# CasualGANPapers/Make-A-Scene

Measured on NVIDIA B200. Metric: VQ-IMG 256^2 images/sec (enc+VQ+dec fwd+bwd), higher is better.
Workload: dtype fp16 (3x3 convolutions) / tf32 (1x1) tcgen05 operands (11-bit significand), fp32 accumulate / storage; 3xTF32 for the attention contractions; fp32 FFMA for VQ argmin and edge layers

## Files before the change

include/mas_b200.h:

```cpp
#ifndef MAS_B200_H_
#define MAS_B200_H_

#include <stddef.h>
#include <stdint.h>

#ifdef __cplusplus
extern "C" {
#endif

#define MAS_OK 0
#define MAS_ERR_INVALID_ARG (-1)
#define MAS_ERR_UNSUPPORTED (-2)
#define MAS_ERR_LAUNCH (-3)
#define MAS_ERR_WORKSPACE (-4)

#define MAS_CONV_S1 0
#define MAS_CONV_S2 1
#define MAS_CONV_UP 2
#define MAS_CONV_ZS 3

#define MAS_IMPL_AUTO 0
#define MAS_IMPL_SIMT 1
#define MAS_IMPL_TC 2
#define MAS_IMPL_TC3 3

typedef struct mas_tensor4 {
  int64_t n, h, w, c;
  int64_t sn, sh, sw, sc;
} mas_tensor4;

int mas_version(void);
const char* mas_last_error(void);
int64_t mas_launch_count(void);
int64_t mas_tc_launch_count(void);

int mas_ffma_probe(float* scratch, int iters, double* flops_out_host, void* stream);

int mas_copy_strided(const float* x, mas_tensor4 xs, float* y, mas_tensor4 ys, void* stream);

int mas_nchw_to_nhwc_pad(const float* x_nchw, float* y_nhwc, int N, int C, int CP, int H, int W, void* stream);
int mas_scale_by(const float* x, const float* g, float* y, int64_t n, void* stream);

size_t mas_gn_ws_bytes(int N, int HW, int C, int G);
int mas_gn_stats(const float* x, int N, int HW, int C, int G, float eps, float* mean, float* rstd,
                 void* ws, size_t ws_bytes, void* stream);
int mas_gn_apply(const float* x, const float* mean, const float* rstd, const float* gamma,
                 const float* beta, float* y, int N, int HW, int C, int G, int silu, int round_tf32,
                 void* stream);
int mas_gn_backward(const float* dy, const float* x, const float* mean, const float* rstd,
                    const float* gamma, const float* beta, const float* dx_add, float* dx, float* dgamma,
                    float* dbeta, void* act_out, int act_f16, float* dx_amax, const float* add_amax, void* dx_f16,
                    float* dx_bound, int N, int HW, int C, int G, int silu, void* ws, size_t ws_bytes, void* stream);
int mas_add(const float* a, const float* b, float* out, int64_t n, void* stream);
int mas_silu_forward(const float* x, float* y, int64_t n, void* stream);
int mas_silu_backward(const float* dy, const float* x, float* dx, int64_t n, void* stream);

int mas_pack_conv3x3(const float* w_oihw, float* w_packed, int Cout, int Cin, int flip_transpose,
                     int round_tf32, void* stream);
int mas_conv3x3_fprop(const float* x, mas_tensor4 xs, const float* w_packed, const float* bias,
                      const float* residual, float* y, mas_tensor4 ys, int mode, int impl, void* stream);
int mas_conv3x3_tc_eligible(mas_tensor4 xs, mas_tensor4 ys, int mode);
int mas_pack_conv3x3_tc(const float* w_oihw, float* w_tc, int Cout, int Cin, int transpose, void* stream);
int mas_conv3x3_fprop_tc(const float* x, mas_tensor4 xs, const float* w_tc, const float* bias,
                         const float* residual, float* y, mas_tensor4 ys, int mode, const float* gn_table,
                         int gn_silu, float* stats_part, void* stream);
int mas_amax(const float* x, int64_t n, float* out, void* stream);
int mas_pack_conv3x3_tc16(const float* w_oihw, void* w_tc16, void* w_tc16_dgrad, int Cout, int Cin, int transpose,
                          void* stream);
int mas_conv3x3_fprop_tc16(const float* x, mas_tensor4 xs, const void* w_tc16, const float* bias,
                           const float* residual, float* y, mas_tensor4 ys, int mode, const float* gn_table,
                           int gn_silu, float* stats_part, const float* x_amax, void* stream);
int mas_conv3x3_tc16h_eligible(mas_tensor4 xs, mas_tensor4 ys);
int mas_conv3x3_fprop_tc16h(const void* x_f16, mas_tensor4 xs, const void* w_tc16, const float* bias,
                            const float* residual, float* y, mas_tensor4 ys, float* stats_part,
                            const float* x_amax, void* stream);
int mas_to_half(const float* x, void* y_f16, int64_t n, const float* amax, void* stream);
int mas_pack_conv3x3_tc_pair(const float* w_oihw, float* w_tc_fwd, float* w_tc_dgrad, int Cout, int Cin, void* stream);
int mas_gn_finalize_partials(const float* part, int tiles_per_image, int N, int C, int G, int64_t hw, float eps,
                             float* mean, float* rstd, void* stream);
int mas_gn_table(const float* mean, const float* rstd, const float* gamma, const float* beta, int N, int C, int G,
                 float* table, void* stream);
int mas_pack_gemm_tc(const float* w_nk, float* w_tc, int N, int K, int transpose, void* stream);
int mas_gemm_rows_packed(const float* A, int64_t lda, const float* w_tc, float* C, int64_t ldc, int64_t M, int N,
                         int K, float alpha, const float* bias, const float* residual, float* stats_part,
                         void* stream);
int mas_pack_gemm_tc16(const float* w_nk, void* w_tc16, int N, int K, int transpose, void* stream);
int mas_gemm_rows_f16(const void* x_f16, int64_t M, int K, const void* w_tc16, float* y, int64_t ldy, int N, const float* bias,
                      const float* residual, const float* x_amax, float alpha, void* stream);
size_t mas_wgrad_rows_f16_ws_bytes(int64_t M, int N, int K);
int mas_wgrad_rows_f16(const void* x_f16, const void* dy_f16, int64_t M, int N, int K, float* dw, float* dbias,
                       const float* x_amax, const float* dy_amax, void* ws, size_t ws_bytes, void* stream);
int mas_tc_probe(const float* A, const float* B, float* D, int a_src, int b_layout, uint64_t raw_desc,
                 uint32_t raw_idesc, int raw_off, void* stream);
int mas_tc_probe16(float* D, uint64_t raw_desc, uint32_t raw_idesc, int raw_off, void* stream);
size_t mas_conv3x3_wgrad_ws_bytes(mas_tensor4 xs, mas_tensor4 dys, int mode);
int mas_conv3x3_wgrad(const float* x, mas_tensor4 xs, const float* dy, mas_tensor4 dys, float* dw_oihw,
                      float* dbias, int mode, int impl, const float* gn_table, int gn_silu, void* ws,
                      size_t ws_bytes, void* stream);
int mas_conv3x3_wgrad_tc_eligible(mas_tensor4 xs, mas_tensor4 dys, int mode);
int mas_conv3x3_wgrad_tc16(const void* x, int x_is_f16, mas_tensor4 xs, const float* dy, mas_tensor4 dys, float* dw_oihw,
                           float* dbias, int mode, const float* gn_table, int gn_silu, const float* dy_amax, int cout_rows,
                           void* ws, size_t ws_bytes, void* stream);
size_t mas_conv1x1_wgrad_ws_bytes(int64_t M, int Cin, int Cout);
int mas_conv1x1_wgrad(const float* x, int64_t ldx, const float* dy, int64_t ldy, int64_t M, int Cin, int Cout,
                      float* dw, float* dbias, int impl, void* ws, size_t ws_bytes, void* stream);
int mas_edge_small_cin_fprop(const float* xs, mas_tensor4 xst, const float* w, const float* bias, float* y,
                             mas_tensor4 yst, int flip_transpose, void* stream);
int mas_edge_small_cout_fprop(const float* a, mas_tensor4 at, const float* w, const float* bias, float* ys,
                              mas_tensor4 yst, void* stream);
size_t mas_edge_wgrad_ws_bytes(int Cbig);
int mas_edge_small_cin_wgrad(const float* xs, mas_tensor4 xst, const float* dy, mas_tensor4 dyt, float* dw,
                             float* dbias, void* ws, size_t ws_bytes, void* stream);
int mas_edge_small_cout_wgrad(const float* a, mas_tensor4 at, const float* dys, mas_tensor4 dyt, float* dw,
                              float* dbias, void* ws, size_t ws_bytes, void* stream);
int mas_space_to_depth(const float* x, float* y, int N, int H, int W, int C, void* stream);
int mas_s2d_pack_weights(const float* w, float* w9, int Cout, int C, void* stream);
int mas_s2d_unpack_wgrad(const float* dw9, float* dw, int Cout, int C, void* stream);
int mas_sumpool2x2(const float* x, float* y, int N, int H, int W, int C, void* stream);

int mas_gemm(const float* A, const float* B, float* C, int M, int N, int K, int batch, int64_t lda,
             int64_t ldb, int64_t ldc, int64_t stride_a, int64_t stride_b, int64_t stride_c, int trans_a,
             int trans_b, float alpha, const float* bias, const float* residual, int impl, void* stream);
int mas_gemm_batched2(const float* A, const float* B, float* C, int M, int N, int K, int outer, int batch, int64_t lda,
                      int64_t ldb, int64_t ldc, int64_t outer_stride_a, int64_t outer_stride_b, int64_t outer_stride_c,
                      int64_t stride_a, int64_t stride_b, int64_t stride_c, int trans_a, int trans_b, float alpha, int impl,
                      int causal, void* stream);
size_t mas_colsum_ws_bytes(mas_tensor4 t);
int mas_colsum(const float* x, mas_tensor4 t, float* out, void* ws, size_t ws_bytes, void* stream);

int mas_softmax_forward(const float* s, float* p, int64_t rows, int cols, void* stream);
int mas_softmax_backward(const float* p, const float* dp, float* ds, int64_t rows, int cols, float scale,
                         void* stream);

size_t mas_attnblock_ws_bytes(int N, int HW, int C, int G);
int mas_attnblock_forward(const float* x, int N, int HW, int C, int G, const float* mean, const float* rstd,
                          const float* norm_w, const float* norm_b, const float* q_w, const float* q_b,
                          const float* k_w, const float* k_b, const float* v_w, const float* v_b,
                          const float* proj_w, const float* proj_b, float* hn, float* qkv, float* P, float* O,
                          float* out, float* stats_part, int impl, void* ws, size_t ws_bytes, void* stream);
int mas_attnblock_backward(const float* dout, const float* x, int N, int HW, int C, int G, const float* mean,
                           const float* rstd, const float* norm_w, const float* norm_b, const float* q_w,
                           const float* k_w, const float* v_w, const float* proj_w, const float* hn,
                           const float* qkv, const float* P, const float* O, float* dx, float* dnorm_w,
                           float* dnorm_b, float* dqkv_w, float* dqkv_b, float* dproj_w, float* dproj_b,
                           float* dx_amax , int impl, void* ws,
                           size_t ws_bytes, void* stream);

int mas_bn_stats(const float* x, int64_t R, int C, double* stats_out, void* stream);
int mas_bn_finalize(const double* stats, double count, int C, float eps, float momentum, float* mean,
                    float* invstd, float* running_mean, float* running_var, void* stream);
int mas_bn_invstd(const float* running_var, float eps, float* invstd, int C, void* stream);
int mas_bn_apply(const float* x, const float* mean, const float* invstd, const float* gamma,
                 const float* beta, float* y, int64_t R, int C, void* stream);
int mas_bn_backward_reduce(const float* dy, const float* x, const float* mean, const float* invstd,
                           int64_t R, int C, double* sums_out, void* stream);
int mas_bn_backward_apply(const float* dy, const float* x, const float* mean, const float* invstd,
                          const float* gamma, const double* sums_global, const double* sums_local,
                          double inv_count, float* dx, float* dgamma, float* dbeta, int64_t R, int C,
                          void* stream);

int mas_vq_select_path(int use_tensor_core_filter);
size_t mas_vq_ws_bytes(int64_t R, int K, int D);
int mas_vq_forward(const float* z, const float* E, int64_t R, int K, int D, float beta, int64_t* idx_out,
                   float* zq_out, float* loss_out, void* ws, size_t ws_bytes, void* stream);
int mas_vq_forward_given(const float* z, const float* E, const int64_t* idx_in, int64_t R, int K, int D, float beta,
                         float* zq_out, float* loss_out, void* ws, size_t ws_bytes, void* stream);
size_t mas_kmeans_ws_bytes(int K, int D);
int mas_kmeans_update(const float* x, const int64_t* idx, int64_t n, int K, int D, const float* centres_old,
                      float* centres_new, float* shift_out, void* ws, size_t ws_bytes, void* stream);
int mas_vq_backward(const float* g_zq, const float* g_loss, const float* z, const float* E,
                    const int64_t* idx, int64_t R, int K, int D, float beta, float* grad_z, float* grad_E,
                    void* stream);
int mas_vq_gather(const float* E, const int64_t* idx, int64_t R, int K, int D, float* out, void* stream);

int mas_layernorm_forward(const float* x, const float* gamma, const float* beta, const float* residual, float* y,
                          float* mean, float* rstd, int64_t R, int H, float eps, void* stream);
int mas_layernorm2_forward(const float* x, const float* gamma1, const float* beta1, const float* residual, float* y1,
                           const float* gamma2, const float* beta2, float* y2, int64_t R, int H, float eps1, float eps2,
                           void* stream);
size_t mas_layernorm_ws_bytes(int64_t R, int H);
int mas_layernorm_backward(const float* dy, const float* x, const float* mean, const float* rstd,
                           const float* gamma, float* dx, float* dgamma, float* dbeta, int64_t R, int H, void* ws,
                           size_t ws_bytes, void* stream);
int mas_gelu_forward(const float* x, float* y, int64_t n, void* stream);
int mas_gelu_backward(const float* dy, const float* x, float* dx, int64_t n, void* stream);
int mas_softmax_causal_forward(const float* s, float* p, int64_t mats, int rows, int cols, void* stream);
int mas_softmax_causal_backward(const float* p, const float* dp, float* ds, int64_t mats, int rows, int cols, float scale,
                                void* stream);
int mas_embed3_forward(const float* t0, const int64_t* id0, const float* t1, const int64_t* id1, const float* t2,
                       const int64_t* id2, float* out, int64_t R, int H, int seg, int total, int off, void* stream);
int mas_embed3_backward(const float* dout, const int64_t* id0, float* d0, const int64_t* id1, float* d1,
                        const int64_t* id2, float* d2, int64_t R, int H, int seg, int total, int off, void* stream);
int mas_attn_causal_forward(const float* qkv, const float* amax, float* P, float* ctx, int B, int S, int heads, int hd,
                            float scale, void* stream);
int mas_ce_forward(const float* logits, int64_t ld, const int64_t* target, float* loss_rows, float* lse, float* out,
                   int64_t R, int V, void* stream);
int mas_ce_backward(const float* logits, int64_t ld, const int64_t* target, const float* lse, const float* stat,
                    const float* dloss, float* dlogits, int64_t ldd, int64_t R, int V, void* stream);

int mas_linear_small(const float* x, int64_t ldx, const float* W, const float* bias, float* y, int64_t ldy, int R, int N,
                     int K, int act, void* stream);
int mas_kv_append(const float* qkv, int R, int T, int heads, int hd, float* kcache, float* vcache, int Tmax, int pos0,
                  void* stream);
int mas_attn_decode(const float* qkv, const float* kcache, const float* vcache, float* ctx, int R, int heads, int hd,
                    int Tmax, int len, void* stream);
int mas_attn_decode_append(const float* qkv, float* kcache, float* vcache, float* ctx, int R, int heads, int hd, int Tmax,
                           int pos, void* stream);
int mas_cfg_mix(const float* cond, const float* uncond, float* out, int64_t n, float scale, void* stream);
int mas_sample_topk(const float* logits, int64_t ld, int R, int V, float temperature, int top_k, const float* u,
                    int64_t* tokens, void* stream);

int mas_bce_logits(const float* logits, mas_tensor4 ls, const float* target, mas_tensor4 ts,
                   const float* pos_weight, float* loss_out, float* grad, mas_tensor4 gs, float grad_scale,
                   void* ws, size_t ws_bytes, void* stream);
size_t mas_bce_ws_bytes(mas_tensor4 ls);
size_t mas_bce_cl_ws_bytes(int N, int H, int W);
int mas_bce_cl_forward(const float* logits, const float* target_nchw, const float* pos_weight, int N, int C, int CP, int H,
                       int W, float* loss_out, void* ws, size_t ws_bytes, void* stream);
int mas_bce_cl_backward(const float* logits, const float* target_nchw, const float* pos_weight, const float* g, int N, int C,
                        int CP, int H, int W, float* grad, void* stream);

#ifdef __cplusplus
}
#endif
#endif
```

make-a-scene_b200/csrc/contract_tc.cu:

```cuda
#include <cuda.h>
#include <cudaTypedefs.h>
#include <cuda_fp16.h>
#include <stdlib.h>

#include "mas_common.cuh"
#include "tc_ptx.cuh"

namespace mas {
namespace tc {

constexpr int TILES_MAX = 4;
constexpr int NPROD = 256;
constexpr int NTHREADS = 320;
constexpr int STAGES_CONV = 3;

enum { MAP_S1 = 0, MAP_UP = 2, MAP_ZS = 3, MAP_ROWS = 4 };

struct Params {
  const float* x;
  const float* wpk;
  const float* bias;
  const float* res;
  float* y;
  int N, Hin, Win, Cin, Hout, Wout, Cout;
  int map;
  int64_t ldx, ldy;
  int tiles_x, tiles_y;
  int64_t total_tiles;
  float alpha;
  const float* gn_table;
  int gn_silu;
  float* stats_part;
  const float* x_amax;
  int Cstore;
};

template <int TAPS, int KC, int STAGES, int TILES, bool F16>
__global__ void __launch_bounds__(NTHREADS, (TILES == 2) ? 2 : 1) shift_gemm_tc(const Params p) {
  constexpr int EPC = F16 ? 8 : 4;
  constexpr int SLOTS = (TAPS == 9) ? 180 : 132;
  constexpr int ROWP = (TAPS == 9) ? 10 : 8;
  constexpr int LBO_A = SLOTS * 16;
  constexpr int SBO_A = ROWP * 16;
  constexpr int A_TILE = (KC / EPC) * LBO_A;
  constexpr int A_STAGE = TILES * A_TILE;
  constexpr int LBO_B = BN * 16;
  constexpr int B_TAP = (KC / EPC) * LBO_B;
  constexpr int B_STAGE = TAPS * B_TAP;
  constexpr int STAGE = A_STAGE + B_STAGE;
  constexpr int QUADS = KC / EPC;
  constexpr int ITEMS = TILES * SLOTS * QUADS;
  constexpr int LPI = F16 ? 2 : 1;
  constexpr int PER_THREAD = (ITEMS + NPROD - 1) / NPROD;
  static_assert((SLOTS % 8) == 4, "A plane pitch must be 64 mod 128 bytes for conflict-free producer stores");

  extern __shared__ __align__(1024) uint8_t smem[];
  uint64_t* bars = reinterpret_cast<uint64_t*>(smem + (size_t)STAGES * STAGE);
  uint32_t* tmem_slot = reinterpret_cast<uint32_t*>(bars + 2 * STAGES + 1);
  const uint32_t smem_base = smem_u32(smem);
  const uint32_t bar_base = smem_u32(bars);
  auto full_bar = [&](int s) { return bar_base + 8u * s; };
  auto empty_bar = [&](int s) { return bar_base + 8u * (STAGES + s); };
  const uint32_t accum_bar = bar_base + 8u * (2 * STAGES);

  const int tid = threadIdx.x, warp = tid >> 5, lane = tid & 31;
  const int64_t tile0 = (int64_t)blockIdx.x * TILES;
  const int n0 = blockIdx.y * BN;
  const int nchunks = p.Cin / KC;

  if (tid == 0) {
    for (int s = 0; s < STAGES; ++s) {
      mbar_init(full_bar(s), NPROD + 1);
      mbar_init(empty_bar(s), 1);
    }
    mbar_init(accum_bar, 1);
    fence_barrier_init();
  }
  if (warp == 8) tmem_alloc(smem_u32(tmem_slot), TILES * BN);
  tc_fence_before();
  __syncthreads();
  tc_fence_after();
  const uint32_t tmem_base = *tmem_slot;

  if (warp < 8) {
    const float* src[PER_THREAD];
    const float* tab[(TAPS == 9) ? PER_THREAD : 1];
    uint32_t dst[PER_THREAD];
#pragma unroll
    for (int i = 0; i < PER_THREAD; ++i) {
      const int item = tid + i * NPROD;
      src[i] = nullptr;
      if (TAPS == 9) tab[i] = nullptr;
      dst[i] = 0xFFFFFFFFu;
      if (item < ITEMS) {
        const int q = item % QUADS, rest = item / QUADS, slot = rest % SLOTS, tl = rest / SLOTS;
        dst[i] = (uint32_t)(tl * A_TILE + q * LBO_A + slot * 16);
        const int64_t tile = tile0 + tl;
        if (tile < p.total_tiles) {
          if (TAPS == 9) {
            const int tx_ = (int)(tile % p.tiles_x), ty_ = (int)((tile / p.tiles_x) % p.tiles_y);
            const int n = (int)(tile / ((int64_t)p.tiles_x * p.tiles_y));
            const int r = slot / 10, c = slot % 10;
            const int vy = ty_ * 16 - 1 + r, vx = tx_ * 8 - 1 + c;
            int iy = vy, ix = vx;
            bool ok;
            if (p.map == MAP_S1) {
              ok = (unsigned)vy < (unsigned)p.Hin && (unsigned)vx < (unsigned)p.Win;
            } else if (p.map == MAP_UP) {
              ok = (unsigned)vy < (unsigned)(2 * p.Hin) && (unsigned)vx < (unsigned)(2 * p.Win);
              iy = vy >> 1; ix = vx >> 1;
            } else {
              ok = vy >= 0 && vx >= 0 && (vy & 1) && (vx & 1) && (vy >> 1) < p.Hin && (vx >> 1) < p.Win;
              iy = vy >> 1; ix = vx >> 1;
            }
            if (ok) {
              src[i] = p.x + ((int64_t)(n * p.Hin + iy) * p.Win + ix) * p.ldx + q * EPC;
              if (p.gn_table) tab[i] = p.gn_table + ((size_t)n * p.Cin + q * EPC) * 2;
            }
          } else {
            const int64_t row = tile * BM + slot;
            if (slot >= BM) dst[i] = 0xFFFFFFFFu;
            else if (row < (int64_t)p.N * p.Hout * p.Wout) src[i] = p.x + row * p.ldx + q * EPC;
          }
        }
      }
    }
    int stage = 0;
    uint32_t phase = 0;
    float inv_scale = 1.f;
    const float in_scale = F16 ? operand_scale(p.x_amax, &inv_scale) : 1.f;
    float4 va[PER_THREAD][LPI], vb[PER_THREAD][LPI];
    auto gload = [&](int kc, float4 (*v)[LPI]) {
#pragma unroll
      for (int i = 0; i < PER_THREAD; ++i) {
#pragma unroll
        for (int h = 0; h < LPI; ++h) {
          v[i][h] = make_float4(0.f, 0.f, 0.f, 0.f);
          if (src[i]) v[i][h] = ldg_l2pf(reinterpret_cast<const float4*>(src[i] + (size_t)kc * KC) + h);
        }
      }
    };
    auto consume = [&](int kc, float4 (*v)[LPI]) {
      if (TAPS == 9) {
        if (p.gn_table) {
#pragma unroll
          for (int i = 0; i < PER_THREAD; ++i) {
            if (tab[i]) {
#pragma unroll
              for (int h = 0; h < LPI; ++h) {
                const float4* tp = reinterpret_cast<const float4*>(tab[i] + (size_t)kc * KC * 2) + 2 * h;
                const float4 t0 = __ldg(tp);
                const float4 t1 = __ldg(tp + 1);
                float a0 = fmaf(v[i][h].x, t0.x, t0.y), a1 = fmaf(v[i][h].y, t0.z, t0.w);
                float a2 = fmaf(v[i][h].z, t1.x, t1.y), a3 = fmaf(v[i][h].w, t1.z, t1.w);
                if (p.gn_silu) { a0 = silu_f(a0); a1 = silu_f(a1); a2 = silu_f(a2); a3 = silu_f(a3); }
                v[i][h] = make_float4(a0, a1, a2, a3);
              }
            }
          }
        }
      }
      mbar_wait(empty_bar(stage), phase ^ 1);
      uint8_t* a_st = smem + (size_t)stage * STAGE;
#pragma unroll
      for (int i = 0; i < PER_THREAD; ++i) {
        if (dst[i] != 0xFFFFFFFFu) {
          if (F16) {
            const float4 lo = v[i][0], hi = v[i][LPI - 1];
            *reinterpret_cast<uint4*>(a_st + dst[i]) =
                make_uint4(pack_h2(lo.x * in_scale, lo.y * in_scale), pack_h2(lo.z * in_scale, lo.w * in_scale),
                           pack_h2(hi.x * in_scale, hi.y * in_scale), pack_h2(hi.z * in_scale, hi.w * in_scale));
          } else {
            *reinterpret_cast<float4*>(a_st + dst[i]) = v[i][0];
          }
        }
      }
      fence_proxy_async();
      mbar_arrive(full_bar(stage));
      if (++stage == STAGES) { stage = 0; phase ^= 1; }
    };
    gload(0, va);
    if (nchunks > 1) gload(1, vb);
    for (int kc = 0; kc < nchunks; kc += 2) {
      consume(kc, va);
      if (kc + 2 < nchunks) gload(kc + 2, va);
      if (kc + 1 < nchunks) {
        consume(kc + 1, vb);
        if (kc + 3 < nchunks) gload(kc + 3, vb);
      }
    }
    const float alpha = p.alpha * inv_scale;

    mbar_wait(accum_bar, 0);
    tc_fence_after();
    const int lane_grp = warp & 3;
    const int chalf = warp >> 2;
    constexpr int EP_LD = 36;
    float* patch = reinterpret_cast<float*>(smem) + warp * (32 * EP_LD);
    const int sub_r = lane >> 3, sub_c = lane & 7;
#pragma unroll 1
    for (int tl = 0; tl < TILES; ++tl) {
      const int64_t tile = tile0 + tl;
      if (tile >= p.total_tiles) break;
      int64_t pix_base = 0;
      int tx_ = 0, ty_ = 0, n_img = 0;
      if (TAPS == 9) {
        tx_ = (int)(tile % p.tiles_x); ty_ = (int)((tile / p.tiles_x) % p.tiles_y);
        n_img = (int)(tile / ((int64_t)p.tiles_x * p.tiles_y));
      } else {
        pix_base = tile * BM;
      }
#pragma unroll 1
      for (int cc = 0; cc < 2; ++cc) {
        const int col = chalf * 64 + cc * 32;
        float v[32];
        tmem_ld32(tmem_base + ((uint32_t)(lane_grp * 32) << 16) + (uint32_t)(tl * BN + col), v);
        __syncwarp();
#pragma unroll
        for (int j = 0; j < 32; j += 4)
          *reinterpret_cast<float4*>(patch + lane * EP_LD + j) =
              make_float4(v[j] * alpha, v[j + 1] * alpha, v[j + 2] * alpha, v[j + 3] * alpha);
        __syncwarp();
        float4 bq = make_float4(0.f, 0.f, 0.f, 0.f);
        if (p.bias) bq = __ldg(reinterpret_cast<const float4*>(p.bias + n0 + col + sub_c * 4));
        float st_s = 0.f, st_q = 0.f;
#pragma unroll
        for (int i = 0; i < 8; ++i) {
          const int row = i * 4 + sub_r;
          const int m = lane_grp * 32 + row;
          int64_t pix;
          if (TAPS == 9) pix = ((int64_t)n_img * p.Hout + ty_ * 16 + (m >> 3)) * p.Wout + tx_ * 8 + (m & 7);
          else pix = pix_base + m;
          if (TAPS == 9 || pix < (int64_t)p.N * p.Hout * p.Wout) {
            float4 o = *reinterpret_cast<const float4*>(patch + row * EP_LD + sub_c * 4);
            o.x += bq.x; o.y += bq.y; o.z += bq.z; o.w += bq.w;
            const int64_t off = pix * p.ldy + n0 + col + sub_c * 4;
            if (n0 + col + sub_c * 4 >= p.Cstore) continue;
            if (p.res) {
              const float4 r4 = __ldg(reinterpret_cast<const float4*>(p.res + off));
              o.x += r4.x; o.y += r4.y; o.z += r4.z; o.w += r4.w;
            }
            *reinterpret_cast<float4*>(p.y + off) = o;
            st_s += (o.x + o.y) + (o.z + o.w);
            st_q = fmaf(o.x, o.x, fmaf(o.y, o.y, fmaf(o.z, o.z, fmaf(o.w, o.w, st_q))));
          }
        }
        if (p.stats_part) {
          st_s += __shfl_xor_sync(0xffffffffu, st_s, 8);
          st_q += __shfl_xor_sync(0xffffffffu, st_q, 8);
          st_s += __shfl_xor_sync(0xffffffffu, st_s, 16);
          st_q += __shfl_xor_sync(0xffffffffu, st_q, 16);
          if (lane < 8) {
            float* sp = p.stats_part + (((size_t)tile * 4 + lane_grp) * (p.Cout >> 2) + ((n0 + col) >> 2) + sub_c) * 2;
            sp[0] = st_s;
            sp[1] = st_q;
          }
        }
      }
    }
    tc_fence_before();
  } else if (warp == 8) {
    {
      constexpr uint32_t idesc = F16 ? make_idesc_f16(BN) : make_idesc(BN);
      int stage = 0;
      uint32_t phase = 0;
      for (int kc = 0; kc < nchunks; ++kc) {
        mbar_wait(full_bar(stage), phase);
        tc_fence_after();
        const uint32_t a_st = smem_base + (uint32_t)stage * STAGE;
        const uint64_t a_base = make_desc(a_st, LBO_A, SBO_A);
        const uint64_t b_base = make_desc(a_st + A_STAGE, LBO_B, 128);
        const uint32_t acc0 = (kc > 0) ? 1u : 0u;
        if (elect_one()) {
#pragma unroll
          for (int tl = 0; tl < TILES; ++tl) {
#pragma unroll
            for (int t = 0; t < TAPS; ++t) {
              const uint32_t tapoff = (TAPS == 9) ? (uint32_t)(((t / 3) * 10 + (t % 3)) * 16) : 0u;
#pragma unroll
              for (int k8 = 0; k8 < KC / (2 * EPC); ++k8) {
                const uint64_t ad = a_base + (uint64_t)((tl * A_TILE + tapoff + k8 * 2 * LBO_A) >> 4);
                const uint64_t bd = b_base + (uint64_t)((t * B_TAP + k8 * 2 * LBO_B) >> 4);
                if (F16) mma_f16_ss(tmem_base + (uint32_t)(tl * BN), ad, bd, idesc, (t > 0 || k8 > 0) ? 1u : acc0);
                else mma_tf32_ss(tmem_base + (uint32_t)(tl * BN), ad, bd, idesc, (t > 0 || k8 > 0) ? 1u : acc0);
              }
            }
          }
          mma_commit(empty_bar(stage));
          if (kc == nchunks - 1) mma_commit(accum_bar);
        }
        __syncwarp();
        if (++stage == STAGES) { stage = 0; phase ^= 1; }
      }
    }
  } else {
    if (lane == 0) {
      int stage = 0;
      uint32_t phase = 0;
      const float* wsrc = p.wpk + (size_t)blockIdx.y * nchunks * (B_STAGE / 4);
      for (int kc = 0; kc < nchunks; ++kc) {
        mbar_wait(empty_bar(stage), phase ^ 1);
        mbar_expect_tx(full_bar(stage), B_STAGE);
        bulk_g2s(smem_base + (uint32_t)stage * STAGE + A_STAGE, wsrc + (size_t)kc * (B_STAGE / 4), B_STAGE, full_bar(stage));
        if (++stage == STAGES) { stage = 0; phase ^= 1; }
      }
    }
    __syncwarp();
  }
  __syncthreads();
  if (warp == 8) {
    tc_fence_after();
    tmem_dealloc(tmem_base, TILES * BN);
  }
}

constexpr int P_STAGES = 4;
constexpr int P_NTHREADS = 14 * 32;
constexpr int P_EPI0 = 8;

__global__ void __launch_bounds__(P_NTHREADS, 1) shift_gemm_p16(const Params p) {
  constexpr int KC = 16, EPC = 8, TILES = 2, TAPS = 9;
  constexpr int SLOTS = 180, ROWP = 10;
  constexpr int LBO_A = SLOTS * 16, SBO_A = ROWP * 16;
  constexpr int A_TILE = (KC / EPC) * LBO_A, A_STAGE = TILES * A_TILE;
  constexpr int LBO_B = BN * 16, B_TAP = (KC / EPC) * LBO_B, B_STAGE = TAPS * B_TAP;
  constexpr int STAGE = A_STAGE + B_STAGE;
  constexpr int QUADS = KC / EPC;
  constexpr int ITEMS = TILES * SLOTS * QUADS;
  constexpr int PER_THREAD = (ITEMS + NPROD - 1) / NPROD;
  constexpr int EP_LD = 36;

  extern __shared__ __align__(1024) uint8_t smem[];
  float* patches = reinterpret_cast<float*>(smem + (size_t)P_STAGES * STAGE);
  uint64_t* bars = reinterpret_cast<uint64_t*>(patches + 4 * 32 * EP_LD);
  uint32_t* tmem_slot = reinterpret_cast<uint32_t*>(bars + 2 * P_STAGES + 4);
  const uint32_t smem_base = smem_u32(smem), bar_base = smem_u32(bars);
  auto full_bar = [&](int s) { return bar_base + 8u * s; };
  auto empty_bar = [&](int s) { return bar_base + 8u * (P_STAGES + s); };
  auto accf_bar = [&](int b) { return bar_base + 8u * (2 * P_STAGES + b); };
  auto acce_bar = [&](int b) { return bar_base + 8u * (2 * P_STAGES + 2 + b); };

  const int tid = threadIdx.x, warp = tid >> 5, lane = tid & 31;
  const int nchunks = p.Cin / KC;
  const int n_tiles = p.Cout / BN;
  const int64_t ngroups = (p.total_tiles + TILES - 1) / TILES;
  const int64_t nitems = ngroups * n_tiles;

  if (tid == 0) {
    for (int s = 0; s < P_STAGES; ++s) {
      mbar_init(full_bar(s), NPROD + 1);
      mbar_init(empty_bar(s), 1);
    }
    for (int b = 0; b < 2; ++b) {
      mbar_init(accf_bar(b), 1);
      mbar_init(acce_bar(b), 128);
    }
    fence_barrier_init();
  }
  if (warp == 12) tmem_alloc(smem_u32(tmem_slot), 512);
  tc_fence_before();
  __syncthreads();
  tc_fence_after();
  const uint32_t tmem_base = *tmem_slot;

  if (warp < 8) {
    float inv_scale = 1.f;
    const float in_scale = operand_scale(p.x_amax, &inv_scale);
    int stage = 0;
    uint32_t phase = 0;
    for (int64_t item = blockIdx.x; item < nitems; item += gridDim.x) {
      const int64_t tile0 = (item / n_tiles) * TILES;
      const float* src[PER_THREAD];
      const float* tab[PER_THREAD];
      uint32_t dst[PER_THREAD];
#pragma unroll
      for (int i = 0; i < PER_THREAD; ++i) {
        const int it = tid + i * NPROD;
        src[i] = nullptr;
        tab[i] = nullptr;
        dst[i] = 0xFFFFFFFFu;
        if (it < ITEMS) {
          const int q = it % QUADS, rest = it / QUADS, slot = rest % SLOTS, tl = rest / SLOTS;
          dst[i] = (uint32_t)(tl * A_TILE + q * LBO_A + slot * 16);
          const int64_t tile = tile0 + tl;
          if (tile < p.total_tiles) {
            const int tx_ = (int)(tile % p.tiles_x), ty_ = (int)((tile / p.tiles_x) % p.tiles_y);
            const int n = (int)(tile / ((int64_t)p.tiles_x * p.tiles_y));
            const int r = slot / 10, c = slot % 10;
            const int vy = ty_ * 16 - 1 + r, vx = tx_ * 8 - 1 + c;
            int iy = vy, ix = vx;
            bool ok;
            if (p.map == MAP_S1) {
              ok = (unsigned)vy < (unsigned)p.Hin && (unsigned)vx < (unsigned)p.Win;
            } else if (p.map == MAP_UP) {
              ok = (unsigned)vy < (unsigned)(2 * p.Hin) && (unsigned)vx < (unsigned)(2 * p.Win);
              iy = vy >> 1; ix = vx >> 1;
            } else {
              ok = vy >= 0 && vx >= 0 && (vy & 1) && (vx & 1) && (vy >> 1) < p.Hin && (vx >> 1) < p.Win;
              iy = vy >> 1; ix = vx >> 1;
            }
            if (ok) {
              src[i] = p.x + ((int64_t)(n * p.Hin + iy) * p.Win + ix) * p.ldx + q * EPC;
              if (p.gn_table) tab[i] = p.gn_table + ((size_t)n * p.Cin + q * EPC) * 2;
            }
          }
        }
      }
      float4 va[PER_THREAD][2], vb[PER_THREAD][2];
      auto gload = [&](int kc, float4 (*v)[2]) {
#pragma unroll
        for (int i = 0; i < PER_THREAD; ++i) {
#pragma unroll
          for (int h = 0; h < 2; ++h) {
            v[i][h] = make_float4(0.f, 0.f, 0.f, 0.f);
            if (src[i]) v[i][h] = ldg_l2pf(reinterpret_cast<const float4*>(src[i] + (size_t)kc * KC) + h);
          }
        }
      };
      auto consume = [&](int kc, float4 (*v)[2]) {
        if (p.gn_table) {
#pragma unroll
          for (int i = 0; i < PER_THREAD; ++i) {
            if (tab[i]) {
#pragma unroll
              for (int h = 0; h < 2; ++h) {
                const float4* tp = reinterpret_cast<const float4*>(tab[i] + (size_t)kc * KC * 2) + 2 * h;
                const float4 t0 = __ldg(tp);
                const float4 t1 = __ldg(tp + 1);
                float a0 = fmaf(v[i][h].x, t0.x, t0.y), a1 = fmaf(v[i][h].y, t0.z, t0.w);
                float a2 = fmaf(v[i][h].z, t1.x, t1.y), a3 = fmaf(v[i][h].w, t1.z, t1.w);
                if (p.gn_silu) { a0 = silu_f(a0); a1 = silu_f(a1); a2 = silu_f(a2); a3 = silu_f(a3); }
                v[i][h] = make_float4(a0, a1, a2, a3);
              }
            }
          }
        }
        mbar_wait(empty_bar(stage), phase ^ 1);
        uint8_t* a_st = smem + (size_t)stage * STAGE;
#pragma unroll
        for (int i = 0; i < PER_THREAD; ++i) {
          if (dst[i] != 0xFFFFFFFFu) {
            const float4 lo = v[i][0], hi = v[i][1];
            *reinterpret_cast<uint4*>(a_st + dst[i]) =
                make_uint4(pack_h2(lo.x * in_scale, lo.y * in_scale), pack_h2(lo.z * in_scale, lo.w * in_scale),
                           pack_h2(hi.x * in_scale, hi.y * in_scale), pack_h2(hi.z * in_scale, hi.w * in_scale));
          }
        }
        fence_proxy_async();
        mbar_arrive(full_bar(stage));
        if (++stage == P_STAGES) { stage = 0; phase ^= 1; }
      };
      gload(0, va);
      if (nchunks > 1) gload(1, vb);
      for (int kc = 0; kc < nchunks; kc += 2) {
        consume(kc, va);
        if (kc + 2 < nchunks) gload(kc + 2, va);
        if (kc + 1 < nchunks) {
          consume(kc + 1, vb);
          if (kc + 3 < nchunks) gload(kc + 3, vb);
        }
      }
    }
  } else if (warp < 12) {
    float inv_scale = 1.f;
    operand_scale(p.x_amax, &inv_scale);
    const float alpha = p.alpha * inv_scale;
    const int lane_grp = warp & 3;
    float* patch = patches + lane_grp * (32 * EP_LD);
    const int sub_r = lane >> 3, sub_c = lane & 7;
    int buf = 0;
    uint32_t ph[2] = {0u, 0u};
    for (int64_t item = blockIdx.x; item < nitems; item += gridDim.x) {
      const int64_t tile0 = (item / n_tiles) * TILES;
      const int n0 = (int)(item % n_tiles) * BN;
      mbar_wait(accf_bar(buf), ph[buf]);
      ph[buf] ^= 1u;
      tc_fence_after();
#pragma unroll 1
      for (int tl = 0; tl < TILES; ++tl) {
        const int64_t tile = tile0 + tl;
        const bool live = tile < p.total_tiles;
        const int tx_ = (int)(tile % p.tiles_x), ty_ = (int)((tile / p.tiles_x) % p.tiles_y);
        const int n_img = (int)(tile / ((int64_t)p.tiles_x * p.tiles_y));
#pragma unroll 1
        for (int cb = 0; cb < BN / 32; ++cb) {
          const int col = cb * 32;
          float v[32];
          tmem_ld32(tmem_base + ((uint32_t)(lane_grp * 32) << 16) + (uint32_t)(buf * TILES * BN + tl * BN + col), v);
          if (tl == TILES - 1 && cb == BN / 32 - 1) {
            tc_fence_before();
            mbar_arrive(acce_bar(buf));
          }
          if (!live) continue;
          __syncwarp();
#pragma unroll
          for (int j = 0; j < 32; j += 4)
            *reinterpret_cast<float4*>(patch + lane * EP_LD + j) =
                make_float4(v[j] * alpha, v[j + 1] * alpha, v[j + 2] * alpha, v[j + 3] * alpha);
          __syncwarp();
          float4 bq = make_float4(0.f, 0.f, 0.f, 0.f);
          if (p.bias) bq = __ldg(reinterpret_cast<const float4*>(p.bias + n0 + col + sub_c * 4));
          float st_s = 0.f, st_q = 0.f;
#pragma unroll
          for (int i = 0; i < 8; ++i) {
            const int row = i * 4 + sub_r;
            const int m = lane_grp * 32 + row;
            const int64_t pix = ((int64_t)n_img * p.Hout + ty_ * 16 + (m >> 3)) * p.Wout + tx_ * 8 + (m & 7);
            float4 o = *reinterpret_cast<const float4*>(patch + row * EP_LD + sub_c * 4);
            o.x += bq.x; o.y += bq.y; o.z += bq.z; o.w += bq.w;
            const int64_t off = pix * p.ldy + n0 + col + sub_c * 4;
            if (n0 + col + sub_c * 4 >= p.Cstore) continue;
            if (p.res) {
              const float4 r4 = __ldg(reinterpret_cast<const float4*>(p.res + off));
              o.x += r4.x; o.y += r4.y; o.z += r4.z; o.w += r4.w;
            }
            *reinterpret_cast<float4*>(p.y + off) = o;
            st_s += (o.x + o.y) + (o.z + o.w);
            st_q = fmaf(o.x, o.x, fmaf(o.y, o.y, fmaf(o.z, o.z, fmaf(o.w, o.w, st_q))));
          }
          if (p.stats_part) {
            st_s += __shfl_xor_sync(0xffffffffu, st_s, 8);
            st_q += __shfl_xor_sync(0xffffffffu, st_q, 8);
            st_s += __shfl_xor_sync(0xffffffffu, st_s, 16);
            st_q += __shfl_xor_sync(0xffffffffu, st_q, 16);
            if (lane < 8) {
              float* sp = p.stats_part + (((size_t)tile * 4 + lane_grp) * (p.Cout >> 2) + ((n0 + col) >> 2) + sub_c) * 2;
              sp[0] = st_s;
              sp[1] = st_q;
            }
          }
        }
      }
      buf ^= 1;
    }
  } else if (warp == 12) {
    {
      constexpr uint32_t idesc = make_idesc_f16(BN);
      int stage = 0, buf = 0;
      uint32_t phase = 0, eph[2] = {0u, 0u};
      for (int64_t item = blockIdx.x; item < nitems; item += gridDim.x) {
        mbar_wait(acce_bar(buf), eph[buf] ^ 1);
        eph[buf] ^= 1u;
        tc_fence_after();
        const uint32_t acc = tmem_base + (uint32_t)(buf * TILES * BN);
        for (int kc = 0; kc < nchunks; ++kc) {
          mbar_wait(full_bar(stage), phase);
          tc_fence_after();
          const uint32_t a_st = smem_base + (uint32_t)stage * STAGE;
          const uint64_t a_base = make_desc(a_st, LBO_A, SBO_A);
          const uint64_t b_base = make_desc(a_st + A_STAGE, LBO_B, 128);
          const uint32_t acc0 = (kc > 0) ? 1u : 0u;
          if (elect_one()) {
#pragma unroll
            for (int tl = 0; tl < TILES; ++tl) {
#pragma unroll
              for (int t = 0; t < TAPS; ++t) {
                const uint32_t tapoff = (uint32_t)(((t / 3) * 10 + (t % 3)) * 16);
                const uint64_t ad = a_base + (uint64_t)((tl * A_TILE + tapoff) >> 4);
                const uint64_t bd = b_base + (uint64_t)((t * B_TAP) >> 4);
                mma_f16_ss(acc + (uint32_t)(tl * BN), ad, bd, idesc, t > 0 ? 1u : acc0);
              }
            }
            mma_commit(empty_bar(stage));
            if (kc == nchunks - 1) mma_commit(accf_bar(buf));
          }
          __syncwarp();
          if (++stage == P_STAGES) { stage = 0; phase ^= 1; }
        }
        buf ^= 1;
      }
    }
  } else {
    if (lane == 0) {
      int stage = 0;
      uint32_t phase = 0;
      for (int64_t item = blockIdx.x; item < nitems; item += gridDim.x) {
        const float* wsrc = p.wpk + (size_t)(item % n_tiles) * nchunks * (B_STAGE / 4);
        for (int kc = 0; kc < nchunks; ++kc) {
          mbar_wait(empty_bar(stage), phase ^ 1);
          mbar_expect_tx(full_bar(stage), B_STAGE);
          bulk_g2s(smem_base + (uint32_t)stage * STAGE + A_STAGE, wsrc + (size_t)kc * (B_STAGE / 4), B_STAGE, full_bar(stage));
          if (++stage == P_STAGES) { stage = 0; phase ^= 1; }
        }
      }
    }
    __syncwarp();
  }
  tc_fence_before();
  __syncthreads();
  if (warp == 12) {
    tc_fence_after();
    tmem_dealloc(tmem_base, 512);
  }
}
constexpr size_t p16_smem_bytes() {
  return (size_t)P_STAGES * (2 * 2 * 180 * 16 + 9 * 2 * BN * 16) + 4 * 32 * 36 * 4 + (2 * P_STAGES + 4) * 8 + 16;
}

template <int TAPS, int KC, int STAGES, int TILES, bool F16>
constexpr size_t smem_bytes() {
  constexpr int SLOTS = (TAPS == 9) ? 180 : 132, EPC = F16 ? 8 : 4;
  return (size_t)STAGES * (TILES * (KC / EPC) * SLOTS * 16 + TAPS * (KC / EPC) * BN * 16) + (2 * STAGES + 1) * 8 + 16;
}

__global__ void pack_weights_tc(const float* __restrict__ w, float* __restrict__ out, int Cout, int Cin, int taps, int KC, int transpose) {
  const int N = transpose ? Cin : Cout, K = transpose ? Cout : Cin;
  const int64_t total = (int64_t)N * K * taps;
  const int nchunks = K / KC, quads = KC / 4;
  for (int64_t i = (int64_t)blockIdx.x * blockDim.x + threadIdx.x; i < total; i += (int64_t)gridDim.x * blockDim.x) {
    int64_t r = i;
    const int e = (int)(r % 4); r /= 4;
    const int nn = (int)(r % BN); r /= BN;
    const int q = (int)(r % quads); r /= quads;
    const int t = (int)(r % taps); r /= taps;
    const int kc = (int)(r % nchunks); r /= nchunks;
    const int nt = (int)r;
    const int n = nt * BN + nn, k = kc * KC + q * 4 + e;
    float v;
    if (!transpose) v = w[((size_t)n * Cin + k) * taps + t];
    else v = w[((size_t)k * Cin + n) * taps + (taps - 1 - t)];
    out[i] = round_tf32(v);
  }
}

__global__ void pack_weights_tc16(const float* __restrict__ w, __half* __restrict__ out_f, __half* __restrict__ out_d, int Cout, int Cin,
                                  int taps, int KC, int transpose, int both) {
  const int64_t total = (int64_t)Cout * Cin * taps;
  for (int64_t i = (int64_t)blockIdx.x * blockDim.x + threadIdx.x; i < total; i += (int64_t)gridDim.x * blockDim.x) {
    const int t = (int)(i % taps);
    const int ci = (int)((i / taps) % Cin), co = (int)(i / ((int64_t)taps * Cin));
    const __half v = __float2half_rn(w[i]);
    auto put = [&](__half* out, int n, int k, int tt, int K) {
      const int nchunks = K / KC, octs = KC / 8;
      const int64_t j = (((((int64_t)(n / BN) * nchunks + k / KC) * taps + tt) * octs + (k % KC) / 8) * BN + (n % BN)) * 8 + (k % 8);
      out[j] = v;
    };
    if (both) {
      put(out_f, co, ci, t, Cin);
      put(out_d, ci, co, taps - 1 - t, Cout);
    } else if (!transpose) {
      put(out_f, co, ci, t, Cin);
    } else {
      put(out_f, ci, co, taps - 1 - t, Cout);
    }
  }
}

__global__ void pack_weights_tc_pair(const float* __restrict__ w, float* __restrict__ out_f, float* __restrict__ out_d, int Cout, int Cin) {
  constexpr int taps = 9, KC = 8, quads = KC / 4;
  const int64_t total = (int64_t)Cout * Cin * taps;
  const int nchunks = Cin / KC, nchunks_d = Cout / KC;
  for (int64_t i = (int64_t)blockIdx.x * blockDim.x + threadIdx.x; i < total; i += (int64_t)gridDim.x * blockDim.x) {
    int64_t r = i;
    const int e = (int)(r % 4); r /= 4;
    const int nn = (int)(r % BN); r /= BN;
    const int q = (int)(r % quads); r /= quads;
    const int t = (int)(r % taps); r /= taps;
    const int kc = (int)(r % nchunks); r /= nchunks;
    const int nt = (int)r;
    const int n = nt * BN + nn, k = kc * KC + q * 4 + e;
    const float v = round_tf32(w[((size_t)n * Cin + k) * taps + t]);
    out_f[i] = v;
    const int td = taps - 1 - t;
    const int64_t j = ((((int64_t)(k / BN) * nchunks_d + n / KC) * taps + td) * quads + (n % KC) / 4) * BN * 4 + (int64_t)(k % BN) * 4 + (n % 4);
    out_d[j] = v;
  }
}


constexpr int WG_NT = 32;
constexpr int WG_STAGES = 3;
constexpr int WG_SLOTS = 100;
constexpr int WG_THREADS = 14 * 32;
constexpr int WG_DY_STAGE = 64 * 128 * 4;

struct WParams {
  const float* x;
  const float* dy;
  float* part;
  float* bpart;
  int N, Hin, Win, Cin, H, W, Cout, map;
  int units_x, units_y;
  int64_t total_units, units_per_split, rows, ldx, ldy;
  const float* gn_table;
  int gn_silu;
  const float* dy_amax;
  int Cout_real;
  int x_f16;
  int dy_f16;
};

template <int TAPS, bool PRO, bool F16>
__global__ void __launch_bounds__(WG_THREADS, 1) wgrad_tc(const WParams p, const __grid_constant__ CUtensorMap dy_map) {
  static_assert(!F16 || TAPS == 9, "the fp16-operand weight-gradient kernel is the 3x3 one");
  constexpr int NT = (TAPS == 9) ? WG_NT : 128, QUADS = NT / 4;
  constexpr int SLOTS = (TAPS == 9) ? WG_SLOTS : 64;
  constexpr int COPIES = (TAPS == 9) ? 3 : 1;
  constexpr int LBO_B = COPIES * NT * 16;
  constexpr int P16 = SLOTS * 16 + 32;
  constexpr int B_STAGE = F16 ? 12 * P16 : ((TAPS == 9) ? 20 : 16) * LBO_B;
  constexpr int A_COLS = F16 ? 32 : 64;
  constexpr int ITEMS = SLOTS * QUADS, PER_THREAD = (ITEMS + NPROD - 1) / NPROD;
  constexpr uint32_t ACC_COLS = TAPS * NT;
  constexpr int NMMA = COPIES * NT;
  constexpr uint32_t idesc = F16 ? (make_idesc_f16(NMMA) | (1u << 16))
                                 : ((1u << 4) | (2u << 7) | (2u << 10) | ((uint32_t)(NMMA >> 3) << 17) | ((uint32_t)(BM >> 4) << 24));

  extern __shared__ __align__(1024) uint8_t smem[];
  uint8_t* dy_smem = smem + (size_t)WG_STAGES * B_STAGE;
  uint64_t* bars = reinterpret_cast<uint64_t*>(dy_smem + (size_t)WG_STAGES * WG_DY_STAGE);
  uint32_t* tmem_slot = reinterpret_cast<uint32_t*>(bars + 4 * WG_STAGES + 1);
  const uint32_t smem_base = smem_u32(smem), bar_base = smem_u32(bars);
  auto fullB = [&](int s) { return bar_base + 8u * s; };
  auto fullA = [&](int s) { return bar_base + 8u * (WG_STAGES + s); };
  auto empty = [&](int s) { return bar_base + 8u * (2 * WG_STAGES + s); };
  auto fullD = [&](int s) { return bar_base + 8u * (3 * WG_STAGES + s); };
  const uint32_t accum_bar = bar_base + 8u * (4 * WG_STAGES);

  const int tid = threadIdx.x, warp = tid >> 5, lane = tid & 31;
  const int ci0 = blockIdx.x * NT, co0 = blockIdx.y * BM, split = blockIdx.z;
  const int64_t u0 = (int64_t)split * p.units_per_split;
  const int64_t u1 = min(p.total_units, u0 + p.units_per_split);

  if (tid == 0) {
    for (int s = 0; s < WG_STAGES; ++s) {
      mbar_init(fullB(s), NPROD);
      mbar_init(fullA(s), 128);
      mbar_init(empty(s), 1);
      mbar_init(fullD(s), 1);
    }
    mbar_init(accum_bar, 1);
    fence_barrier_init();
  }
  if (warp == 12) tmem_alloc(smem_u32(tmem_slot), 512);
  tc_fence_before();
  __syncthreads();
  tc_fence_after();
  const uint32_t tmem_base = *tmem_slot;

  if (warp < 8 && F16) {
    constexpr int OCTS = NT / 8, ITEMS16 = SLOTS * OCTS, PT16 = (ITEMS16 + NPROD - 1) / NPROD;
    int sl_r[PT16], sl_c[PT16], sl_o[PT16];
#pragma unroll
    for (int i = 0; i < PT16; ++i) {
      const int item = tid + i * NPROD, slot = item / OCTS;
      sl_o[i] = item % OCTS;
      sl_r[i] = slot / 10;
      sl_c[i] = item < ITEMS16 ? slot % 10 : -100;
    }
    int pux = (int)(u0 % p.units_x), puy = (int)((u0 / p.units_x) % p.units_y), pn = (int)(u0 / ((int64_t)p.units_x * p.units_y));
    int cux = 0, cuy = 0, cn = 0;
    auto gload16 = [&](float4 (*v)[2]) {
      const int ux = pux, uy = puy, n = pn;
      if (++pux == p.units_x) { pux = 0; if (++puy == p.units_y) { puy = 0; ++pn; } }
#pragma unroll
      for (int i = 0; i < PT16; ++i) {
        v[i][0] = make_float4(0.f, 0.f, 0.f, 0.f);
        v[i][1] = v[i][0];
        if (sl_c[i] >= 0) {
          const int vy = uy * 8 - 1 + sl_r[i], vx = ux * 8 - 1 + sl_c[i];
          int iy = vy, ix = vx;
          bool ok;
          if (p.map == MAP_S1) {
            ok = (unsigned)vy < (unsigned)p.Hin && (unsigned)vx < (unsigned)p.Win;
          } else {
            ok = (unsigned)vy < (unsigned)(2 * p.Hin) && (unsigned)vx < (unsigned)(2 * p.Win);
            iy = vy >> 1; ix = vx >> 1;
          }
          if (ok) {
            const int64_t e = ((int64_t)(n * p.Hin + iy) * p.Win + ix) * p.Cin + ci0 + sl_o[i] * 8;
            if (p.x_f16) {
              v[i][0] = __ldg(reinterpret_cast<const float4*>(reinterpret_cast<const __half*>(p.x) + e));
            } else {
              const float4* src = reinterpret_cast<const float4*>(p.x + e);
              v[i][0] = __ldg(src);
              v[i][1] = __ldg(src + 1);
            }
          }
        }
      }
    };
    int stage = 0;
    uint32_t phase = 0;
    float4 vn[PT16][2];
    if (u0 < u1) gload16(vn);
    for (int64_t u = u0; u < u1; ++u) {
      float4 v[PT16][2];
#pragma unroll
      for (int i = 0; i < PT16; ++i) { v[i][0] = vn[i][0]; v[i][1] = vn[i][1]; }
      if (PRO) {
        cux = (int)(u % p.units_x); cuy = (int)((u / p.units_x) % p.units_y); cn = (int)(u / ((int64_t)p.units_x * p.units_y));
      }
      if (u + 1 < u1) gload16(vn);
      if (PRO && p.gn_table) {
#pragma unroll
        for (int i = 0; i < PT16; ++i) {
          if (sl_c[i] >= 0) {
            const int vy = cuy * 8 - 1 + sl_r[i], vx = cux * 8 - 1 + sl_c[i];
            const bool ok = (p.map == MAP_S1) ? ((unsigned)vy < (unsigned)p.Hin && (unsigned)vx < (unsigned)p.Win)
                                              : ((unsigned)vy < (unsigned)(2 * p.Hin) && (unsigned)vx < (unsigned)(2 * p.Win));
            if (ok) {
#pragma unroll
              for (int h = 0; h < 2; ++h) {
                const float4* tp = reinterpret_cast<const float4*>(p.gn_table + ((size_t)cn * p.Cin + ci0 + sl_o[i] * 8 + h * 4) * 2);
                const float4 t0 = __ldg(tp), t1 = __ldg(tp + 1);
                float a0 = fmaf(v[i][h].x, t0.x, t0.y), a1 = fmaf(v[i][h].y, t0.z, t0.w);
                float a2 = fmaf(v[i][h].z, t1.x, t1.y), a3 = fmaf(v[i][h].w, t1.z, t1.w);
                if (p.gn_silu) { a0 = silu_f(a0); a1 = silu_f(a1); a2 = silu_f(a2); a3 = silu_f(a3); }
                v[i][h] = make_float4(a0, a1, a2, a3);
              }
            }
          }
        }
      }
      mbar_wait(empty(stage), phase ^ 1);
      uint8_t* b_st = smem + (size_t)stage * B_STAGE;
#pragma unroll
      for (int i = 0; i < PT16; ++i) {
        if (sl_c[i] >= 0) {
          const uint4 h = p.x_f16 ? make_uint4(__float_as_uint(v[i][0].x), __float_as_uint(v[i][0].y), __float_as_uint(v[i][0].z),
                                               __float_as_uint(v[i][0].w))
                                  : make_uint4(pack_h2(v[i][0].x, v[i][0].y), pack_h2(v[i][0].z, v[i][0].w), pack_h2(v[i][1].x, v[i][1].y),
                                               pack_h2(v[i][1].z, v[i][1].w));
          const int slot = sl_r[i] * 10 + sl_c[i];
#pragma unroll
          for (int dx = 0; dx < 3; ++dx)
            if (sl_c[i] >= dx) *reinterpret_cast<uint4*>(b_st + (dx * OCTS + sl_o[i]) * P16 + (slot - dx) * 16) = h;
        }
      }
      fence_proxy_async();
      mbar_arrive(fullB(stage));
      if (++stage == WG_STAGES) { stage = 0; phase ^= 1; }
    }
    if (warp < 4) {
      float inv = 1.f;
      operand_scale(p.dy_amax, &inv);
      mbar_wait(accum_bar, 0);
      tc_fence_after();
      const int co = co0 + warp * 32 + lane;
#pragma unroll 1
      for (int t = 0; t < TAPS; ++t) {
        float* o = p.part + (((size_t)split * TAPS + t) * p.Cout + co) * p.Cin + ci0;
        float v[32];
        tmem_ld32(tmem_base + ((uint32_t)(warp * 32) << 16) + (uint32_t)(t * NT), v);
#pragma unroll
        for (int q = 0; q < 8; ++q)
          *reinterpret_cast<float4*>(o + q * 4) = make_float4(v[4 * q] * inv, v[4 * q + 1] * inv, v[4 * q + 2] * inv, v[4 * q + 3] * inv);
      }
      tc_fence_before();
    }
  } else if (warp < 8) {
    int it_r[PER_THREAD], it_c[PER_THREAD], it_q[PER_THREAD];
#pragma unroll
    for (int i = 0; i < PER_THREAD; ++i) {
      const int item = tid + i * NPROD;
      const int q = (item % 8) + 8 * (item / (8 * SLOTS)), slot = (item / 8) % SLOTS;
      it_q[i] = q;
      if (TAPS == 9) { it_r[i] = slot / 10; it_c[i] = item < ITEMS ? slot % 10 : -100; }
      else { it_r[i] = slot; it_c[i] = item < ITEMS ? 0 : -100; }
    }
    int pux = (int)(u0 % p.units_x), puy = (int)((u0 / p.units_x) % p.units_y), pn = (int)(u0 / ((int64_t)p.units_x * p.units_y));
    auto gload = [&](int64_t u, float4* v) {
      if (TAPS == 9) {
        const int ux = pux, uy = puy, n = pn;
        if (++pux == p.units_x) { pux = 0; if (++puy == p.units_y) { puy = 0; ++pn; } }
#pragma unroll
        for (int i = 0; i < PER_THREAD; ++i) {
          v[i] = make_float4(0.f, 0.f, 0.f, 0.f);
          if (it_c[i] >= 0) {
            const int vy = uy * 8 - 1 + it_r[i], vx = ux * 8 - 1 + it_c[i];
            int iy = vy, ix = vx;
            bool ok;
            if (p.map == MAP_S1) {
              ok = (unsigned)vy < (unsigned)p.Hin && (unsigned)vx < (unsigned)p.Win;
            } else {
              ok = (unsigned)vy < (unsigned)(2 * p.Hin) && (unsigned)vx < (unsigned)(2 * p.Win);
              iy = vy >> 1; ix = vx >> 1;
            }
            if (ok) v[i] = __ldg(reinterpret_cast<const float4*>(p.x + ((int64_t)(n * p.Hin + iy) * p.Win + ix) * p.Cin + ci0 + it_q[i] * 4));
          }
        }
      } else {
#pragma unroll
        for (int i = 0; i < PER_THREAD; ++i) {
          v[i] = make_float4(0.f, 0.f, 0.f, 0.f);
          const int64_t row = u * 64 + it_r[i];
          if (it_c[i] >= 0 && row < p.rows) v[i] = __ldg(reinterpret_cast<const float4*>(p.x + row * p.ldx + ci0 + it_q[i] * 4));
        }
      }
    };
    int stage = 0;
    uint32_t phase = 0;
    float4 vn[PER_THREAD];
    if (u0 < u1) gload(u0, vn);
    for (int64_t u = u0; u < u1; ++u) {
      float4 v[PER_THREAD];
#pragma unroll
      for (int i = 0; i < PER_THREAD; ++i) v[i] = vn[i];
      if (u + 1 < u1) gload(u + 1, vn);
      if (TAPS == 9 && PRO) {
        if (p.gn_table) {
          const int ux = (int)(u % p.units_x), uy = (int)((u / p.units_x) % p.units_y);
          const int n = (int)(u / ((int64_t)p.units_x * p.units_y));
#pragma unroll
          for (int i = 0; i < PER_THREAD; ++i) {
            if (it_c[i] >= 0) {
              const int vy = uy * 8 - 1 + it_r[i], vx = ux * 8 - 1 + it_c[i];
              const bool ok = (p.map == MAP_S1) ? ((unsigned)vy < (unsigned)p.Hin && (unsigned)vx < (unsigned)p.Win)
                                                : ((unsigned)vy < (unsigned)(2 * p.Hin) && (unsigned)vx < (unsigned)(2 * p.Win));
              if (ok) {
                const float4* tp = reinterpret_cast<const float4*>(p.gn_table + ((size_t)n * p.Cin + ci0 + it_q[i] * 4) * 2);
                const float4 t0 = __ldg(tp), t1 = __ldg(tp + 1);
                float a0 = fmaf(v[i].x, t0.x, t0.y), a1 = fmaf(v[i].y, t0.z, t0.w);
                float a2 = fmaf(v[i].z, t1.x, t1.y), a3 = fmaf(v[i].w, t1.z, t1.w);
                if (p.gn_silu) { a0 = silu_f(a0); a1 = silu_f(a1); a2 = silu_f(a2); a3 = silu_f(a3); }
                v[i] = make_float4(a0, a1, a2, a3);
              }
            }
          }
        }
      }
      mbar_wait(empty(stage), phase ^ 1);
      float* b_st = reinterpret_cast<float*>(smem + (size_t)stage * B_STAGE);
#pragma unroll
      for (int i = 0; i < PER_THREAD; ++i) {
        if (it_c[i] >= 0) {
          const float e[4] = {v[i].x, v[i].y, v[i].z, v[i].w};
          if (F16) {
            const unsigned short h[4] = {to_h(e[0]), to_h(e[1]), to_h(e[2]), to_h(e[3])};
#pragma unroll
            for (int dx = 0; dx < COPIES; ++dx) {
              const int c = it_c[i] - dx;
              if ((unsigned)c < 8u) {
                unsigned short* d = reinterpret_cast<unsigned short*>(b_st) + it_r[i] * (LBO_B / 2) + dx * (NT * 8) + it_q[i] * 8 + c;
#pragma unroll
                for (int j = 0; j < 4; ++j) d[j * NT * 2] = h[j];
              }
            }
            continue;
          }
#pragma unroll
          for (int dx = 0; dx < COPIES; ++dx) {
            const int c = it_c[i] - dx;
            if (TAPS == 1 || (unsigned)c < 8u) {
              const int kk = (TAPS == 9) ? it_r[i] * 8 + c : it_r[i];
              float* d = b_st + (kk >> 2) * (LBO_B / 4) + dx * (NT * 4) + it_q[i] * 4 + (kk & 3);
#pragma unroll
              for (int j = 0; j < 4; ++j) d[j * NT] = e[j];
            }
          }
        }
      }
      fence_proxy_async();
      mbar_arrive(fullB(stage));
      if (++stage == WG_STAGES) { stage = 0; phase ^= 1; }
    }
    if (warp < 4) {
      float inv = 1.f;
      if (F16) operand_scale(p.dy_amax, &inv);
      mbar_wait(accum_bar, 0);
      tc_fence_after();
      const int co = co0 + warp * 32 + lane;
#pragma unroll 1
      for (int t = 0; t < TAPS; ++t) {
        float* o = p.part + (((size_t)split * TAPS + t) * p.Cout + co) * p.Cin + ci0;
        if (TAPS == 9) {
          float v[32];
          tmem_ld32(tmem_base + ((uint32_t)(warp * 32) << 16) + (uint32_t)(t * NT), v);
#pragma unroll
          for (int q = 0; q < 8; ++q)
            *reinterpret_cast<float4*>(o + q * 4) = make_float4(v[q] * inv, v[8 + q] * inv, v[16 + q] * inv, v[24 + q] * inv);
        } else {
#pragma unroll
          for (int qb = 0; qb < 32; qb += 8) {
            float v0[8], v1[8], v2[8], v3[8];
            const uint32_t tb = tmem_base + ((uint32_t)(warp * 32) << 16) + (uint32_t)qb;
            tmem_ld8(tb, v0);
            tmem_ld8(tb + 32, v1);
            tmem_ld8(tb + 64, v2);
            tmem_ld8(tb + 96, v3);
#pragma unroll
            for (int q = 0; q < 8; ++q) *reinterpret_cast<float4*>(o + (qb + q) * 4) = make_float4(v0[q], v1[q], v2[q], v3[q]);
          }
        }
      }
      tc_fence_before();
    }
  } else if (warp < 12) {
    const int lg = warp & 3;
    const int cl = lg * 32 + lane;
    float bsum = 0.f;
    const bool want_bias = p.bpart != nullptr && blockIdx.x == 0;
    int stage = 0;
    uint32_t phase = 0;
    float a_inv;
    const float a_scale = F16 ? operand_scale(p.dy_amax, &a_inv) : 1.f;
    for (int64_t u = u0; u < u1; ++u) {
      mbar_wait(fullD(stage), phase);
      const float* dys = reinterpret_cast<const float*>(dy_smem + (size_t)stage * WG_DY_STAGE) + cl;
      if (F16 && p.dy_f16) {
        const unsigned short* dh = reinterpret_cast<const unsigned short*>(dy_smem + (size_t)stage * WG_DY_STAGE) + cl;
        float w[32];
#pragma unroll
        for (int j = 0; j < 32; ++j) {
          const uint32_t lo = dh[(2 * j) * 128], hi = dh[(2 * j + 1) * 128];
          w[j] = __uint_as_float(lo | (hi << 16));
          if (want_bias) bsum += __half2float(__ushort_as_half((unsigned short)lo)) + __half2float(__ushort_as_half((unsigned short)hi));
        }
        tc_fence_after();
        tmem_st32(tmem_base + ((uint32_t)(lg * 32) << 16) + ACC_COLS + (uint32_t)(stage * A_COLS), w);
        tmem_st_wait();
        tc_fence_before();
        mbar_arrive(fullA(stage));
        if (++stage == WG_STAGES) { stage = 0; phase ^= 1; }
        continue;
      }
      float v[64];
      if (TAPS == 9) {
#pragma unroll
        for (int j = 0; j < 64; ++j) v[j] = dys[j * 128];
      } else {
#pragma unroll
        for (int j = 0; j < 64; ++j) v[j] = (u * 64 + j < p.rows) ? dys[j * 128] : 0.f;
      }
      if (want_bias) {
#pragma unroll
        for (int j = 0; j < 64; ++j) bsum += v[j];
      }
      tc_fence_after();
      const uint32_t ta = tmem_base + ((uint32_t)(lg * 32) << 16) + ACC_COLS + (uint32_t)(stage * A_COLS);
      if (F16) {
        float w[32];
#pragma unroll
        for (int j = 0; j < 32; ++j) w[j] = __uint_as_float(pack_h2(v[2 * j] * a_scale, v[2 * j + 1] * a_scale));
        tmem_st32(ta, w);
      } else {
        tmem_st32(ta, v);
        tmem_st32(ta + 32, v + 32);
      }
      tmem_st_wait();
      tc_fence_before();
      mbar_arrive(fullA(stage));
      if (++stage == WG_STAGES) { stage = 0; phase ^= 1; }
    }
    if (want_bias) p.bpart[(size_t)split * p.Cout + co0 + cl] = (F16 && p.dy_f16) ? bsum * a_inv : bsum;
  } else if (warp == 13) {
    if (lane == 0) {
      int stage = 0;
      uint32_t phase = 0;
      for (int64_t u = u0; u < u1; ++u) {
        const uint32_t dst = smem_u32(dy_smem) + (uint32_t)stage * WG_DY_STAGE;
        mbar_wait(empty(stage), phase ^ 1);
        mbar_expect_tx(fullD(stage), (F16 && p.dy_f16) ? WG_DY_STAGE / 2 : WG_DY_STAGE);
        if (TAPS == 9) {
          const int ux = (int)(u % p.units_x), uy = (int)((u / p.units_x) % p.units_y);
          const int n = (int)(u / ((int64_t)p.units_x * p.units_y));
          tma_load_4d(dst, &dy_map, co0, ux * 8, uy * 8, n, fullD(stage));
        } else {
          tma_load_2d(dst, &dy_map, co0, (int)(u * 64), fullD(stage));
        }
        if (++stage == WG_STAGES) { stage = 0; phase ^= 1; }
      }
    }
    __syncwarp();
  } else {
    {
      int stage = 0;
      uint32_t phase = 0;
      for (int64_t u = u0; u < u1; ++u) {
        mbar_wait(fullB(stage), phase);
        mbar_wait(fullA(stage), phase);
        tc_fence_after();
        const uint32_t b_st = smem_base + (uint32_t)stage * B_STAGE;
        const uint32_t a_t = tmem_base + ACC_COLS + (uint32_t)(stage * A_COLS);
        const uint64_t b_base = make_desc(b_st, LBO_B, 128);
        const uint64_t b16 = make_desc(b_st, 160, P16);
        const uint32_t acc0 = (u > u0) ? 1u : 0u;
        if (elect_one()) {
          if (F16) {
#pragma unroll
            for (int r = 0; r < 8; r += 2) {
#pragma unroll
              for (int dyy = 0; dyy < 3; ++dyy) {
                const uint64_t bd = b16 + (uint64_t)(((r + dyy) * 160) >> 4);
                mma_f16_ts(tmem_base + (uint32_t)(dyy * NMMA), a_t + (uint32_t)(r * 4), bd, idesc, r > 0 ? 1u : acc0);
              }
            }
          } else {
#pragma unroll
            for (int r = 0; r < 8; ++r) {
#pragma unroll
              for (int dyy = 0; dyy < ((TAPS == 9) ? 3 : 1); ++dyy) {
                const uint64_t bd = b_base + (uint64_t)(((r + dyy) * 2 * LBO_B) >> 4);
                mma_tf32_ts(tmem_base + (uint32_t)(dyy * NMMA), a_t + (uint32_t)(r * 8), bd, idesc, r > 0 ? 1u : acc0);
              }
            }
          }
          mma_commit(empty(stage));
          if (u + 1 == u1) mma_commit(accum_bar);
        }
        __syncwarp();
        if (++stage == WG_STAGES) { stage = 0; phase ^= 1; }
      }
      if (u0 >= u1 && elect_one()) mma_commit(accum_bar);
      __syncwarp();
    }
  }
  __syncthreads();
  if (warp == 12) {
    tc_fence_after();
    tmem_dealloc(tmem_base, 512);
  }
}

__global__ void __launch_bounds__(128, 1) mma_probe(const float* __restrict__ A, const float* __restrict__ B, float* __restrict__ D,
                                                    int a_src, int b_layout, unsigned long long raw_desc, unsigned raw_idesc,
                                                    int raw_off) {
  __shared__ __align__(1024) uint8_t sm[16384];
  __shared__ __align__(8) uint64_t bar;
  __shared__ uint32_t tslot;
  const int tid = threadIdx.x, warp = tid >> 5, lane = tid & 31;
  float* sa = reinterpret_cast<float*>(sm);
  float* sb = reinterpret_cast<float*>(sm + 8192);
  constexpr int PL = 36 * 16;
  if (tid == 0) { mbar_init(smem_u32(&bar), 1); fence_barrier_init(); }
  if (warp == 0) tmem_alloc(smem_u32(&tslot), 64);
  for (int i = tid; i < 128 * 8; i += 128) {
    int m = i / 8, k = i % 8;
    sa[((k / 4) * 2048 + m * 16 + (k % 4) * 4) / 4] = A[i];
  }
  const int raw = b_layout == 99;
  const int reveal = b_layout >= 10;
  if (reveal) {
    b_layout = raw ? 0 : b_layout - 10;
    for (int i = tid; i < 2048; i += 128) sb[i] = (float)i;
  } else {
    for (int i = tid; i < 32 * 8; i += 128) {
      int n = i / 8, k = i % 8;
      int off = (b_layout == 0) ? ((k / 4) * 512 + n * 16 + (k % 4) * 4) : ((n / 4) * PL + k * 16 + (n % 4) * 4);
      sb[off / 4] = B[i];
    }
  }
  fence_proxy_async();
  tc_fence_before();
  __syncthreads();
  tc_fence_after();
  const uint32_t tb = tslot;
  if (a_src == 1) {
    float v[32];
#pragma unroll
    for (int j = 0; j < 32; ++j) v[j] = j < 8 ? A[(warp * 32 + lane) * 8 + j] : 0.f;
    tmem_st32(tb + ((uint32_t)(warp * 32) << 16) + 32, v);
    tmem_st_wait();
    tc_fence_before();
  }
  __syncthreads();
  tc_fence_after();
  if (tid == 0) {
    uint32_t idesc = (1u << 4) | (2u << 7) | (2u << 10) | ((uint32_t)(32 >> 3) << 17) | ((uint32_t)(128 >> 4) << 24);
    if (b_layout != 0) idesc |= (1u << 16);
    uint64_t bd;
    if (b_layout == 0) bd = make_desc(smem_u32(sb), 512, 128);
    else if (b_layout == 1) bd = make_desc(smem_u32(sb), 160, PL);
    else bd = make_desc(smem_u32(sb), PL, 160);
    if (raw) {
      bd = (raw_desc & ~0x3FFFull) | (uint64_t)(((smem_u32(sb) + (uint32_t)raw_off) >> 4) & 0x3FFF);
      idesc = raw_idesc;
    }
    if (a_src == 0) mma_tf32_ss(tb, make_desc(smem_u32(sa), 2048, 128), bd, idesc, 0);
    else mma_tf32_ts(tb, tb + 32, bd, idesc, 0);
    mma_commit(smem_u32(&bar));
  }
  mbar_wait(smem_u32(&bar), 0);
  tc_fence_after();
  float v[32];
  tmem_ld32(tb + ((uint32_t)(warp * 32) << 16), v);
  for (int j = 0; j < 32; ++j) D[(warp * 32 + lane) * 32 + j] = v[j];
  tc_fence_before();
  __syncthreads();
  if (warp == 0) tmem_dealloc(tb, 64);
}

__global__ void __launch_bounds__(128, 1) mma_probe16(float* __restrict__ D, unsigned long long raw_desc, unsigned raw_idesc, int raw_off) {
  __shared__ __align__(1024) uint8_t sm[8192];
  __shared__ __align__(8) uint64_t bar;
  __shared__ uint32_t tslot;
  const int tid = threadIdx.x, warp = tid >> 5, lane = tid & 31;
  __half* sa = reinterpret_cast<__half*>(sm);
  __half* sb = reinterpret_cast<__half*>(sm + 4096);
  if (tid == 0) { mbar_init(smem_u32(&bar), 1); fence_barrier_init(); }
  if (warp == 0) tmem_alloc(smem_u32(&tslot), 64);
  for (int i = tid; i < 128 * 16; i += 128) {
    const int m = i / 16, k = i % 16;
    sa[(k / 8) * 1024 + m * 8 + (k % 8)] = __float2half((k == m % 16) ? 1.f : 0.f);
  }
  for (int i = tid; i < 2048; i += 128) sb[i] = __float2half((float)i);
  fence_proxy_async();
  tc_fence_before();
  __syncthreads();
  tc_fence_after();
  const uint32_t tb = tslot;
  if (tid == 0) {
    const uint64_t bd = (raw_desc & ~0x3FFFull) | (uint64_t)(((smem_u32(sb) + (uint32_t)raw_off) >> 4) & 0x3FFF);
    mma_f16_ss(tb, make_desc(smem_u32(sa), 2048, 128), bd, raw_idesc, 0);
    mma_commit(smem_u32(&bar));
  }
  mbar_wait(smem_u32(&bar), 0);
  tc_fence_after();
  float v[32];
  tmem_ld32(tb + ((uint32_t)(warp * 32) << 16), v);
  for (int j = 0; j < 32; ++j) D[(warp * 32 + lane) * 32 + j] = v[j];
  tc_fence_before();
  __syncthreads();
  if (warp == 0) tmem_dealloc(tb, 64);
}

}

void conv_wgrad_reduce_launch(const float* part, int splits, int ntap, int Cout, int Cin, float* dw, const float* bpart, float* dbias,
                              cudaStream_t st);

static bool dense_nhwc(const mas_tensor4& t) {
  return t.sc == 1 && t.sw == t.c && t.sh == t.w * t.c && t.sn == t.h * t.w * t.c;
}
static inline bool al16p(const void* p) { return (reinterpret_cast<uintptr_t>(p) & 15) == 0; }

template <typename K>
static int set_smem(K kernel, size_t bytes) {
  cudaError_t e = cudaFuncSetAttribute(kernel, cudaFuncAttributeMaxDynamicSharedMemorySize, (int)bytes);
  if (e != cudaSuccess) return fail(MAS_ERR_LAUNCH, "cudaFuncSetAttribute(smem=%zu): %s", bytes, cudaGetErrorString(e));
  return MAS_OK;
}

int conv3x3_fprop_tc_launch(const float* x, mas_tensor4 xs, const float* w_tc, const float* bias, const float* res, float* y,
                            mas_tensor4 ys, int mode, const float* gn_table, int gn_silu, float* stats_part, int f16,
                            const float* x_amax, cudaStream_t st) {
  const int Cin = (int)xs.c, Cstore = (int)ys.c, Cout = (int)cdiv(ys.c, tc::BN) * tc::BN;
  if (f16 && Cin % 16) return fail(MAS_ERR_UNSUPPORTED, "tc conv (fp16 operands): Cin=%d must be a multiple of 16", Cin);
  if (Cstore % 4) return fail(MAS_ERR_UNSUPPORTED, "tc conv: Cout=%d must be a multiple of 4", Cstore);
  if (Cstore != Cout && (res || stats_part)) return fail(MAS_ERR_UNSUPPORTED, "tc conv: residual / statistics epilogues need Cout %% 128 == 0");
  if (!(mode == MAS_CONV_S1 || mode == MAS_CONV_UP || mode == MAS_CONV_ZS)) return fail(MAS_ERR_UNSUPPORTED, "tc conv: mode %d", mode);
  if (!dense_nhwc(xs) || !dense_nhwc(ys) || Cin % 8 || ys.h % 16 || ys.w % 8 || !al16p(x) || !al16p(y) ||
      (res && !al16p(res)) || (bias && !al16p(bias)) || !al16p(w_tc))
    return fail(MAS_ERR_UNSUPPORTED, "tc conv: shape/layout not eligible (Cin=%d Cout=%d Hout=%lld Wout=%lld)", Cin, Cout,
                (long long)ys.h, (long long)ys.w);
  int64_t eh = (mode == MAS_CONV_S1) ? xs.h : 2 * xs.h, ew = (mode == MAS_CONV_S1) ? xs.w : 2 * xs.w;
  if (ys.h != eh || ys.w != ew || xs.n != ys.n) return fail(MAS_ERR_INVALID_ARG, "tc conv: output extent mismatch");
  tc::Params p;
  p.x = x; p.wpk = w_tc; p.bias = bias; p.res = res; p.y = y;
  p.N = (int)xs.n; p.Hin = (int)xs.h; p.Win = (int)xs.w; p.Cin = Cin; p.Hout = (int)ys.h; p.Wout = (int)ys.w; p.Cout = Cout;
  p.map = (mode == MAS_CONV_S1) ? tc::MAP_S1 : (mode == MAS_CONV_UP ? tc::MAP_UP : tc::MAP_ZS);
  p.ldx = Cin; p.ldy = Cstore; p.Cstore = Cstore;
  p.tiles_x = (int)(ys.w / 8); p.tiles_y = (int)(ys.h / 16);
  p.total_tiles = (int64_t)p.N * p.tiles_x * p.tiles_y;
  p.alpha = 1.0f;
  p.gn_table = gn_table; p.gn_silu = gn_silu; p.stats_part = stats_part;
  p.x_amax = f16 ? x_amax : nullptr;
  if (gn_table && !al16p(gn_table)) return fail(MAS_ERR_INVALID_ARG, "tc conv: gn_table must be 16-byte aligned");
  constexpr int T = 2, STG = 2;
  constexpr size_t smem = tc::smem_bytes<9, 8, STG, T, false>();
  static_assert(smem == tc::smem_bytes<9, 16, STG, T, true>(), "both operand formats stage the same bytes per K chunk");
  static std::atomic<uint64_t> configured{0};
  if (first_on_device(configured)) {
    if (int e = set_smem(tc::shift_gemm_tc<9, 8, STG, T, false>, smem)) return e;
    if (int e = set_smem(tc::shift_gemm_tc<9, 16, STG, T, true>, smem)) return e;
    mark_device(configured);
  }
  dim3 grid((unsigned)cdiv(p.total_tiles, T), (unsigned)(Cout / tc::BN));
  if (f16) {
    static const bool persist = [] { const char* e = getenv("MAS_CONV_PERSIST"); return e && e[0] == '1'; }();
    if (persist) {
      constexpr size_t psm = tc::p16_smem_bytes();
      static std::atomic<uint64_t> pconf{0};
      static int sm_count = 148;
      if (first_on_device(pconf)) {
        if (int e = set_smem(tc::shift_gemm_p16, psm)) return e;
        int dev = 0;
        cudaGetDevice(&dev);
        cudaDeviceGetAttribute(&sm_count, cudaDevAttrMultiProcessorCount, dev);
        mark_device(pconf);
      }
      const int64_t nitems = cdiv(p.total_tiles, 2) * (Cout / tc::BN);
      const unsigned g = (unsigned)(nitems < sm_count ? nitems : sm_count);
      tc::shift_gemm_p16<<<g, tc::P_NTHREADS, psm, st>>>(p);
      return launched_tc("shift_gemm_p16");
    }
    tc::shift_gemm_tc<9, 16, STG, T, true><<<grid, tc::NTHREADS, smem, st>>>(p);
    return launched_tc("shift_gemm_tc<9,f16>");
  }
  tc::shift_gemm_tc<9, 8, STG, T, false><<<grid, tc::NTHREADS, smem, st>>>(p);
  return launched_tc("shift_gemm_tc<9>");
}

int gemm_rows_tc_launch(const float* A, int64_t lda, const float* w_tc, float* C, int64_t ldc, int64_t M, int N, int K, float alpha,
                        const float* bias, const float* res, float* stats_part, cudaStream_t st) {
  if (K % 32 || N % tc::BN || lda % 4 || ldc % 4 || !al16p(A) || !al16p(C) || (res && !al16p(res)) || (bias && !al16p(bias)) ||
      !al16p(w_tc))
    return fail(MAS_ERR_UNSUPPORTED, "tc gemm: shape not eligible (M=%lld N=%d K=%d)", (long long)M, N, K);
  tc::Params p;
  p.x = A; p.wpk = w_tc; p.bias = bias; p.res = res; p.y = C;
  p.N = 1; p.Hin = 1; p.Win = 1; p.Cin = K; p.Hout = 1; p.Wout = (int)M; p.Cout = N;
  if (M > 0x7fffffff) return fail(MAS_ERR_UNSUPPORTED, "tc gemm: M too large");
  p.map = tc::MAP_ROWS;
  p.ldx = lda; p.ldy = ldc;
  p.tiles_x = 1; p.tiles_y = 1;
  p.total_tiles = cdiv(M, tc::BM);
  p.alpha = alpha;
  p.gn_table = nullptr; p.gn_silu = 0; p.stats_part = stats_part; p.x_amax = nullptr; p.Cstore = N;
  if (stats_part && (M % tc::BM || ldc != N)) return fail(MAS_ERR_UNSUPPORTED, "tc gemm: fused statistics need M %% 128 == 0 and a dense output");
  constexpr size_t smem = tc::smem_bytes<1, 32, 2, 2, false>();
  static std::atomic<uint64_t> configured{0};
  if (first_on_device(configured)) {
    if (int e = set_smem(tc::shift_gemm_tc<1, 32, 2, 2, false>, smem)) return e;
    mark_device(configured);
  }
  dim3 grid((unsigned)cdiv(p.total_tiles, 2), (unsigned)(N / tc::BN));
  tc::shift_gemm_tc<1, 32, 2, 2, false><<<grid, tc::NTHREADS, smem, st>>>(p);
  return launched_tc("shift_gemm_tc<1>");
}

int gemm_tc_launch(const float*, const float*, float*, int, int, int, int, int64_t, int64_t, int64_t, int64_t, int64_t, int64_t, int, int,
                   float, const float*, const float*, cudaStream_t) {
  return fail(MAS_ERR_UNSUPPORTED, "tc gemm with un-packed B operand: not available (use mas_gemm_rows_packed)");
}
static bool wgrad_tc_ok(const mas_tensor4& xs, const mas_tensor4& dys, int mode, bool pad_ok = false) {
  if (!(mode == MAS_CONV_S1 || mode == MAS_CONV_UP)) return false;
  if (!dense_nhwc(xs) || !dense_nhwc(dys) || xs.c % tc::WG_NT || dys.c % (pad_ok ? 4 : tc::BM) || dys.h % 8 || dys.w % 8) return false;
  int64_t eh = (mode == MAS_CONV_S1) ? xs.h : 2 * xs.h, ew = (mode == MAS_CONV_S1) ? xs.w : 2 * xs.w;
  return dys.h == eh && dys.w == ew && xs.n == dys.n;
}
static int wgrad_tc_splits(int64_t cps, int64_t units) {
  int64_t s = 148 / cps;
  if (s < 1) s = 1;
  if (s > units) s = units;
  const int64_t ups = cdiv(units, s);
  return (int)cdiv(units, ups);
}
size_t conv_wgrad_t16_ws(mas_tensor4 xs, mas_tensor4 dys);
bool conv_wgrad_t16_ok(mas_tensor4 xs, mas_tensor4 dys);
int conv_wgrad_t16_launch(const void* x16, mas_tensor4 xs, const void* dy16, mas_tensor4 dys, float* dw, float* dbias,
                          const float* dy_amax, void* ws, size_t ws_bytes, cudaStream_t st);
size_t conv_wgrad_tc_ws(mas_tensor4 xs, mas_tensor4 dys, int mode) {
  if (!wgrad_tc_ok(xs, dys, mode, true)) return 0;
  const int64_t coutk = cdiv(dys.c, tc::BM) * tc::BM;
  size_t splits = wgrad_tc_splits((coutk / tc::BM) * (xs.c / tc::WG_NT), dys.n * (dys.h / 8) * (dys.w / 8));
  const size_t a = splits * 9 * (size_t)coutk * xs.c * sizeof(float) + splits * (size_t)coutk * sizeof(float) + 256;
  const size_t b = mode == MAS_CONV_S1 ? conv_wgrad_t16_ws(xs, dys) : 0;
  return a > b ? a : b;
}
PFN_cuTensorMapEncodeTiled tensor_map_encoder() {
  static PFN_cuTensorMapEncodeTiled fn = nullptr;
  if (!fn) {
    void* ptr = nullptr;
    cudaDriverEntryPointQueryResult q;
    if (cudaGetDriverEntryPoint("cuTensorMapEncodeTiled", &ptr, cudaEnableDefault, &q) == cudaSuccess && q == cudaDriverEntryPointSuccess)
      fn = reinterpret_cast<PFN_cuTensorMapEncodeTiled>(ptr);
  }
  return fn;
}
static int make_dy_map(CUtensorMap* map, const tc::WParams& p, int taps) {
  PFN_cuTensorMapEncodeTiled enc = tensor_map_encoder();
  if (!enc) return fail(MAS_ERR_LAUNCH, "cuTensorMapEncodeTiled entry point not available");
  CUresult r;
  if (taps == 9) {
    const cuuint64_t eb = p.dy_f16 ? 2 : 4;
    cuuint64_t dims[4] = {(cuuint64_t)p.Cout_real, (cuuint64_t)p.W, (cuuint64_t)p.H, (cuuint64_t)p.N};
    cuuint64_t strides[3] = {(cuuint64_t)p.Cout_real * eb, (cuuint64_t)p.W * p.Cout_real * eb, (cuuint64_t)p.H * p.W * p.Cout_real * eb};
    cuuint32_t box[4] = {128, 8, 8, 1}, es[4] = {1, 1, 1, 1};
    r = enc(map, p.dy_f16 ? CU_TENSOR_MAP_DATA_TYPE_FLOAT16 : CU_TENSOR_MAP_DATA_TYPE_FLOAT32, 4, (void*)p.dy, dims, strides, box, es,
            CU_TENSOR_MAP_INTERLEAVE_NONE, CU_TENSOR_MAP_SWIZZLE_NONE, CU_TENSOR_MAP_L2_PROMOTION_L2_128B, CU_TENSOR_MAP_FLOAT_OOB_FILL_NONE);
  } else {
    cuuint64_t dims[2] = {(cuuint64_t)p.Cout_real, (cuuint64_t)p.rows};
    cuuint64_t strides[1] = {(cuuint64_t)p.ldy * 4};
    cuuint32_t box[2] = {128, 64}, es[2] = {1, 1};
    r = enc(map, CU_TENSOR_MAP_DATA_TYPE_FLOAT32, 2, (void*)p.dy, dims, strides, box, es, CU_TENSOR_MAP_INTERLEAVE_NONE,
            CU_TENSOR_MAP_SWIZZLE_NONE, CU_TENSOR_MAP_L2_PROMOTION_L2_128B, CU_TENSOR_MAP_FLOAT_OOB_FILL_NONE);
  }
  if (r != CUDA_SUCCESS) return fail(MAS_ERR_LAUNCH, "cuTensorMapEncodeTiled failed (%d)", (int)r);
  return MAS_OK;
}

template <int TAPS, bool PRO, bool F16>
static int wgrad_tc_run(tc::WParams& p, int splits, float* dw, float* dbias, void* ws, cudaStream_t st) {
  p.part = (float*)ws;
  p.bpart = dbias ? (float*)ws + (size_t)splits * TAPS * p.Cout * p.Cin : nullptr;
  p.units_per_split = cdiv(p.total_units, splits);
  constexpr int NT = (TAPS == 9) ? tc::WG_NT : 128;
  constexpr size_t bstage = F16 ? (size_t)12 * (tc::WG_SLOTS * 16 + 32) : (size_t)(TAPS == 9 ? 3 * 20 : 16) * NT * 16;
  constexpr size_t smem = (size_t)tc::WG_STAGES * (bstage + tc::WG_DY_STAGE) + (4 * tc::WG_STAGES + 1) * 8 + 16;
  static std::atomic<uint64_t> configured{0};
  if (first_on_device(configured)) {
    if (int e = set_smem(tc::wgrad_tc<TAPS, PRO, F16>, smem)) return e;
    mark_device(configured);
  }
  CUtensorMap dy_map;
  if (int e = make_dy_map(&dy_map, p, TAPS)) return e;
  dim3 grid((unsigned)(p.Cin / NT), (unsigned)(p.Cout / tc::BM), (unsigned)splits);
  tc::wgrad_tc<TAPS, PRO, F16><<<grid, tc::WG_THREADS, smem, st>>>(p, dy_map);
  if (int e = launched_tc("wgrad_tc")) return e;
  conv_wgrad_reduce_launch((const float*)ws, splits, TAPS, p.Cout, p.Cin, dw, p.bpart, dbias, st);
  return launched("conv_wgrad_reduce");
}
bool conv_wgrad_tc_eligible(mas_tensor4 xs, mas_tensor4 dys, int mode) { return wgrad_tc_ok(xs, dys, mode); }
int conv_wgrad_tc_launch(const float* x, mas_tensor4 xs, const float* dy, mas_tensor4 dys, float* dw, float* dbias, int mode,
                         const float* gn_table, int gn_silu, int f16, const float* dy_amax, int cout_rows, int x_f16, void* ws,
                         size_t ws_bytes, cudaStream_t st) {
  const int dy_f16 = (x_f16 >> 1) & 1;
  x_f16 &= 1;
  if (x_f16 && (!f16 || gn_table)) return fail(MAS_ERR_INVALID_ARG, "tc wgrad: an fp16 x needs the fp16-operand kernel and no prologue");
  if (dy_f16 && (!f16 || !dy_amax || dys.c % 8)) return fail(MAS_ERR_INVALID_ARG, "tc wgrad: an fp16 dy needs the fp16-operand kernel, its scale source and Cout %% 8 == 0");
  static const bool tma_off = [] { const char* e = getenv("MAS_WGRAD_TMA"); return e && e[0] == '0'; }();
  if (f16 && x_f16 && dy_f16 && mode == MAS_CONV_S1 && !gn_table && !tma_off && conv_wgrad_t16_ok(xs, dys) &&
      cout_rows == (int)(cdiv(dys.c, tc::BM) * tc::BM))
    return conv_wgrad_t16_launch(x, xs, dy, dys, dw, dbias, dy_amax, ws, ws_bytes, st);
  const bool pad_ok = cout_rows == (int)(cdiv(dys.c, tc::BM) * tc::BM);
  if (!wgrad_tc_ok(xs, dys, mode, pad_ok) || !al16p(x) || !al16p(dy)) return fail(MAS_ERR_UNSUPPORTED, "tc wgrad: shape/layout not eligible");
  if (ws_bytes < conv_wgrad_tc_ws(xs, dys, mode)) return fail(MAS_ERR_WORKSPACE, "tc wgrad: workspace too small");
  tc::WParams p;
  p.x = x; p.dy = dy;
  p.N = (int)xs.n; p.Hin = (int)xs.h; p.Win = (int)xs.w; p.Cin = (int)xs.c; p.H = (int)dys.h; p.W = (int)dys.w;
  p.Cout = (int)(cdiv(dys.c, tc::BM) * tc::BM); p.Cout_real = (int)dys.c;
  p.map = (mode == MAS_CONV_S1) ? tc::MAP_S1 : tc::MAP_UP;
  p.units_x = (int)(dys.w / 8); p.units_y = (int)(dys.h / 8);
  p.total_units = (int64_t)p.N * p.units_x * p.units_y;
  p.rows = 0; p.ldx = p.Cin; p.ldy = p.Cout_real;
  p.gn_table = gn_table; p.gn_silu = gn_silu; p.dy_amax = f16 ? dy_amax : nullptr; p.x_f16 = x_f16; p.dy_f16 = dy_f16;
  const int splits = wgrad_tc_splits((p.Cout / tc::BM) * (xs.c / tc::WG_NT), p.total_units);
  if (f16) return gn_table ? wgrad_tc_run<9, true, true>(p, splits, dw, dbias, ws, st) : wgrad_tc_run<9, false, true>(p, splits, dw, dbias, ws, st);
  return gn_table ? wgrad_tc_run<9, true, false>(p, splits, dw, dbias, ws, st) : wgrad_tc_run<9, false, false>(p, splits, dw, dbias, ws, st);
}
static bool wgrad1_tc_ok(const float* x, int64_t ldx, const float* dy, int64_t ldy, int Cin, int Cout) {
  return Cin % 128 == 0 && Cout % tc::BM == 0 && ldx % 4 == 0 && al16p(x) && dy != nullptr && ldy >= Cout && ldy % 4 == 0 && al16p(dy);
}
size_t conv1x1_wgrad_tc_ws(int64_t M, int Cin, int Cout) {
  if (Cin % 128 || Cout % tc::BM) return 0;
  size_t splits = wgrad_tc_splits((int64_t)(Cout / tc::BM) * (Cin / 128), cdiv(M, 64));
  return splits * (size_t)Cout * Cin * sizeof(float) + splits * (size_t)Cout * sizeof(float) + 256;
}
int conv1x1_wgrad_tc_launch(const float* x, int64_t ldx, const float* dy, int64_t ldy, int64_t M, int Cin, int Cout, float* dw,
                            float* dbias, void* ws, size_t ws_bytes, cudaStream_t st) {
  if (!wgrad1_tc_ok(x, ldx, dy, ldy, Cin, Cout)) return fail(MAS_ERR_UNSUPPORTED, "tc wgrad 1x1: shape not eligible");
  if (ws_bytes < conv1x1_wgrad_tc_ws(M, Cin, Cout)) return fail(MAS_ERR_WORKSPACE, "tc wgrad 1x1: workspace too small");
  tc::WParams p;
  p.x = x; p.dy = dy;
  p.N = 1; p.Hin = 1; p.Win = 1; p.Cin = Cin; p.H = 1; p.W = 1; p.Cout = Cout; p.Cout_real = Cout; p.map = tc::MAP_ROWS;
  p.units_x = 1; p.units_y = 1;
  p.total_units = cdiv(M, 64);
  p.rows = M; p.ldx = ldx; p.ldy = ldy;
  p.gn_table = nullptr; p.gn_silu = 0; p.dy_amax = nullptr; p.x_f16 = 0; p.dy_f16 = 0;
  const int splits = wgrad_tc_splits((int64_t)(Cout / tc::BM) * (Cin / 128), p.total_units);
  return wgrad_tc_run<1, false, false>(p, splits, dw, dbias, ws, st);
}

}

using namespace mas;

extern "C" {

int mas_pack_conv3x3_tc(const float* w_oihw, float* w_tc, int Cout, int Cin, int transpose, void* stream) {
  const int N = transpose ? Cin : Cout, K = transpose ? Cout : Cin;
  if (N % tc::BN || K % 8) return fail(MAS_ERR_UNSUPPORTED, "pack_conv3x3_tc: N=%d must be a multiple of 128 and K=%d of 8", N, K);
  int64_t total = (int64_t)9 * Cout * Cin;
  tc::pack_weights_tc<<<(int)(cdiv(total, 256) < 2368 ? cdiv(total, 256) : 2368), 256, 0, S(stream)>>>(w_oihw, w_tc, Cout, Cin, 9, 8, transpose);
  return launched("pack_weights_tc<9>");
}

int mas_pack_conv3x3_tc_pair(const float* w_oihw, float* w_tc_fwd, float* w_tc_dgrad, int Cout, int Cin, void* stream) {
  if (Cout % tc::BN || Cin % tc::BN) return fail(MAS_ERR_UNSUPPORTED, "pack_conv3x3_tc_pair: Cout=%d and Cin=%d must be multiples of 128", Cout, Cin);
  int64_t total = (int64_t)9 * Cout * Cin;
  tc::pack_weights_tc_pair<<<(int)(cdiv(total, 256) < 2368 ? cdiv(total, 256) : 2368), 256, 0, S(stream)>>>(w_oihw, w_tc_fwd, w_tc_dgrad, Cout, Cin);
  return launched("pack_weights_tc_pair");
}

int mas_pack_conv3x3_tc16(const float* w_oihw, void* w_tc16, void* w_tc16_dgrad, int Cout, int Cin, int transpose, void* stream) {
  const bool both = w_tc16_dgrad != nullptr;
  const int N = (transpose && !both) ? Cin : Cout, K = (transpose && !both) ? Cout : Cin;
  if (N % tc::BN || K % 16 || (both && (Cin % tc::BN || Cout % 16)))
    return fail(MAS_ERR_UNSUPPORTED, "pack_conv3x3_tc16: N must be a multiple of 128 and K of 16 (Cout=%d Cin=%d)", Cout, Cin);
  int64_t total = (int64_t)9 * Cout * Cin;
  tc::pack_weights_tc16<<<(int)(cdiv(total, 256) < 2368 ? cdiv(total, 256) : 2368), 256, 0, S(stream)>>>(
      w_oihw, (__half*)w_tc16, (__half*)w_tc16_dgrad, Cout, Cin, 9, 16, transpose, both ? 1 : 0);
  return launched("pack_weights_tc16<9>");
}

int mas_pack_gemm_tc16(const float* w_nk, void* w_tc16, int N, int K, int transpose, void* stream) {
  if (!w_nk || !w_tc16 || N <= 0 || K <= 0) return fail(MAS_ERR_INVALID_ARG, "pack_gemm_tc16: bad arguments");
  const int Nn = transpose ? K : N, Kk = transpose ? N : K;
  if (Nn % tc::BN || Kk % 64)
    return fail(MAS_ERR_UNSUPPORTED, "pack_gemm_tc16: output features (%d) must be a multiple of 128 and the contraction (%d) of 64", Nn, Kk);
  const int64_t total = (int64_t)N * K;
  tc::pack_weights_tc16<<<(int)(cdiv(total, 256) < 2368 ? cdiv(total, 256) : 2368), 256, 0, S(stream)>>>(w_nk, (__half*)w_tc16, nullptr, N, K, 1, 16,
                                                                                                     transpose, 0);
  return launched("pack_weights_tc16<1>");
}

int mas_pack_gemm_tc(const float* w_nk, float* w_tc, int N, int K, int transpose, void* stream) {
  const int Nn = transpose ? K : N, Kk = transpose ? N : K;
  if (Nn % tc::BN || Kk % 32) return fail(MAS_ERR_UNSUPPORTED, "pack_gemm_tc: N=%d must be a multiple of 128 and K=%d of 32", Nn, Kk);
  int64_t total = (int64_t)N * K;
  tc::pack_weights_tc<<<(int)(cdiv(total, 256) < 2368 ? cdiv(total, 256) : 2368), 256, 0, S(stream)>>>(w_nk, w_tc, N, K, 1, 32, transpose);
  return launched("pack_weights_tc<1>");
}

int mas_gemm_rows_packed(const float* A, int64_t lda, const float* w_tc, float* C, int64_t ldc, int64_t M, int N, int K, float alpha,
                         const float* bias, const float* residual, float* stats_part, void* stream) {
  MAS_REQUIRE(A && w_tc && C && M > 0, "gemm_rows_packed: bad arguments");
  return gemm_rows_tc_launch(A, lda, w_tc, C, ldc, M, N, K, alpha, bias, residual, stats_part, S(stream));
}

int mas_tc_probe(const float* A, const float* B, float* D, int a_src, int b_layout, uint64_t raw_desc, uint32_t raw_idesc,
                 int raw_off, void* stream) {
  tc::mma_probe<<<1, 128, 0, S(stream)>>>(A, B, D, a_src, b_layout, (unsigned long long)raw_desc, raw_idesc, raw_off);
  return launched_tc("mma_probe");
}

int mas_tc_probe16(float* D, uint64_t raw_desc, uint32_t raw_idesc, int raw_off, void* stream) {
  tc::mma_probe16<<<1, 128, 0, S(stream)>>>(D, (unsigned long long)raw_desc, raw_idesc, raw_off);
  return launched_tc("mma_probe16");
}

int mas_conv3x3_tc_eligible(mas_tensor4 xs, mas_tensor4 ys, int mode) {
  const int Cin = (int)xs.c, Cout = (int)ys.c;
  if (!(mode == MAS_CONV_S1 || mode == MAS_CONV_UP || mode == MAS_CONV_ZS)) return 0;
  if (!dense_nhwc(xs) || !dense_nhwc(ys) || Cin % 8 || Cout % tc::BN || ys.h % 16 || ys.w % 8) return 0;
  return 1;
}

int mas_conv3x3_fprop_tc(const float* x, mas_tensor4 xs, const float* w_tc, const float* bias, const float* residual, float* y,
                         mas_tensor4 ys, int mode, const float* gn_table, int gn_silu, float* stats_part, void* stream) {
  MAS_REQUIRE(x && w_tc && y, "conv3x3_fprop_tc: null pointer");
  return conv3x3_fprop_tc_launch(x, xs, w_tc, bias, residual, y, ys, mode, gn_table, gn_silu, stats_part, 0, nullptr, S(stream));
}

int mas_conv3x3_fprop_tc16(const float* x, mas_tensor4 xs, const void* w_tc16, const float* bias, const float* residual, float* y,
                           mas_tensor4 ys, int mode, const float* gn_table, int gn_silu, float* stats_part, const float* x_amax,
                           void* stream) {
  MAS_REQUIRE(x && w_tc16 && y, "conv3x3_fprop_tc16: null pointer");
  return conv3x3_fprop_tc_launch(x, xs, (const float*)w_tc16, bias, residual, y, ys, mode, gn_table, gn_silu, stats_part, 1, x_amax,
                                 S(stream));
}

}
```

make-a-scene_b200/mas_b200/_lib.py:

```python
from __future__ import annotations

import ctypes
import os

import torch

_HERE = os.path.dirname(os.path.abspath(__file__))
LIB_PATH = os.path.join(os.path.dirname(_HERE), "lib", "libmas_b200.so")

IMPL_AUTO, IMPL_SIMT, IMPL_TC, IMPL_TC3 = 0, 1, 2, 3
CONV_S1, CONV_S2, CONV_UP, CONV_ZS = 0, 1, 2, 3


class Tensor4(ctypes.Structure):
    _fields_ = [(k, ctypes.c_int64) for k in ("n", "h", "w", "c", "sn", "sh", "sw", "sc")]


_P, _I, _L, _F, _D, _Z, _T = (ctypes.c_void_p, ctypes.c_int, ctypes.c_int64, ctypes.c_float, ctypes.c_double,
                              ctypes.c_size_t, Tensor4)

_SPEC = {
    "mas_version": (_I, []),
    "mas_last_error": (ctypes.c_char_p, []),
    "mas_launch_count": (_L, []),
    "mas_tc_launch_count": (_L, []),
    "mas_ffma_probe": (_I, [_P, _I, _P, _P]),
    "mas_copy_strided": (_I, [_P, _T, _P, _T, _P]),
    "mas_nchw_to_nhwc_pad": (_I, [_P, _P, _I, _I, _I, _I, _I, _P]),
    "mas_scale_by": (_I, [_P, _P, _P, _L, _P]),
    "mas_gn_ws_bytes": (_Z, [_I, _I, _I, _I]),
    "mas_gn_stats": (_I, [_P, _I, _I, _I, _I, _F, _P, _P, _P, _Z, _P]),
    "mas_gn_apply": (_I, [_P, _P, _P, _P, _P, _P, _I, _I, _I, _I, _I, _I, _P]),
    "mas_gn_backward": (_I, [_P, _P, _P, _P, _P, _P, _P, _P, _P, _P, _P, _I, _P, _P, _P, _P, _I, _I, _I, _I, _I, _P, _Z, _P]),
    "mas_add": (_I, [_P, _P, _P, _L, _P]),
    "mas_silu_forward": (_I, [_P, _P, _L, _P]),
    "mas_silu_backward": (_I, [_P, _P, _P, _L, _P]),
    "mas_pack_conv3x3": (_I, [_P, _P, _I, _I, _I, _I, _P]),
    "mas_conv3x3_fprop": (_I, [_P, _T, _P, _P, _P, _P, _T, _I, _I, _P]),
    "mas_tc_probe": (_I, [_P, _P, _P, _I, _I, ctypes.c_uint64, ctypes.c_uint32, _I, _P]),
    "mas_tc_probe16": (_I, [_P, ctypes.c_uint64, ctypes.c_uint32, _I, _P]),
    "mas_conv3x3_tc_eligible": (_I, [_T, _T, _I]),
    "mas_pack_conv3x3_tc": (_I, [_P, _P, _I, _I, _I, _P]),
    "mas_pack_conv3x3_tc_pair": (_I, [_P, _P, _P, _I, _I, _P]),
    "mas_conv3x3_fprop_tc": (_I, [_P, _T, _P, _P, _P, _P, _T, _I, _P, _I, _P, _P]),
    "mas_amax": (_I, [_P, _L, _P, _P]),
    "mas_pack_conv3x3_tc16": (_I, [_P, _P, _P, _I, _I, _I, _P]),
    "mas_conv3x3_fprop_tc16": (_I, [_P, _T, _P, _P, _P, _P, _T, _I, _P, _I, _P, _P, _P]),
    "mas_conv3x3_tc16h_eligible": (_I, [_T, _T]),
    "mas_conv3x3_fprop_tc16h": (_I, [_P, _T, _P, _P, _P, _P, _T, _P, _P, _P]),
    "mas_to_half": (_I, [_P, _P, _L, _P, _P]),
    "mas_gn_finalize_partials": (_I, [_P, _I, _I, _I, _I, _L, _F, _P, _P, _P]),
    "mas_gn_table": (_I, [_P, _P, _P, _P, _I, _I, _I, _P, _P]),
    "mas_pack_gemm_tc": (_I, [_P, _P, _I, _I, _I, _P]),
    "mas_gemm_rows_packed": (_I, [_P, _L, _P, _P, _L, _L, _I, _I, _F, _P, _P, _P, _P]),
    "mas_conv3x3_wgrad_ws_bytes": (_Z, [_T, _T, _I]),
    "mas_conv3x3_wgrad": (_I, [_P, _T, _P, _T, _P, _P, _I, _I, _P, _I, _P, _Z, _P]),
    "mas_conv3x3_wgrad_tc_eligible": (_I, [_T, _T, _I]),
    "mas_conv3x3_wgrad_tc16": (_I, [_P, _I, _T, _P, _T, _P, _P, _I, _P, _I, _P, _I, _P, _Z, _P]),
    "mas_conv1x1_wgrad_ws_bytes": (_Z, [_L, _I, _I]),
    "mas_conv1x1_wgrad": (_I, [_P, _L, _P, _L, _L, _I, _I, _P, _P, _I, _P, _Z, _P]),
    "mas_edge_small_cin_fprop": (_I, [_P, _T, _P, _P, _P, _T, _I, _P]),
    "mas_edge_small_cout_fprop": (_I, [_P, _T, _P, _P, _P, _T, _P]),
    "mas_edge_wgrad_ws_bytes": (_Z, [_I]),
    "mas_edge_small_cin_wgrad": (_I, [_P, _T, _P, _T, _P, _P, _P, _Z, _P]),
    "mas_edge_small_cout_wgrad": (_I, [_P, _T, _P, _T, _P, _P, _P, _Z, _P]),
    "mas_space_to_depth": (_I, [_P, _P, _I, _I, _I, _I, _P]),
    "mas_s2d_pack_weights": (_I, [_P, _P, _I, _I, _P]),
    "mas_s2d_unpack_wgrad": (_I, [_P, _P, _I, _I, _P]),
    "mas_sumpool2x2": (_I, [_P, _P, _I, _I, _I, _I, _P]),
    "mas_gemm": (_I, [_P, _P, _P, _I, _I, _I, _I, _L, _L, _L, _L, _L, _L, _I, _I, _F, _P, _P, _I, _P]),
    "mas_colsum_ws_bytes": (_Z, [_T]),
    "mas_colsum": (_I, [_P, _T, _P, _P, _Z, _P]),
    "mas_attnblock_ws_bytes": (_Z, [_I, _I, _I, _I]),
    "mas_attnblock_forward": (_I, [_P, _I, _I, _I, _I] + [_P] * 18 + [_I, _P, _Z, _P]),
    "mas_attnblock_backward": (_I, [_P, _P, _I, _I, _I, _I] + [_P] * 20 + [_I, _P, _Z, _P]),
    "mas_softmax_forward": (_I, [_P, _P, _L, _I, _P]),
    "mas_softmax_backward": (_I, [_P, _P, _P, _L, _I, _F, _P]),
    "mas_bn_stats": (_I, [_P, _L, _I, _P, _P]),
    "mas_bn_finalize": (_I, [_P, _D, _I, _F, _F, _P, _P, _P, _P, _P]),
    "mas_bn_invstd": (_I, [_P, _F, _P, _I, _P]),
    "mas_bn_apply": (_I, [_P, _P, _P, _P, _P, _P, _L, _I, _P]),
    "mas_bn_backward_reduce": (_I, [_P, _P, _P, _P, _L, _I, _P, _P]),
    "mas_bn_backward_apply": (_I, [_P, _P, _P, _P, _P, _P, _P, _D, _P, _P, _P, _L, _I, _P]),
    "mas_vq_select_path": (_I, [_I]),
    "mas_vq_ws_bytes": (_Z, [_L, _I, _I]),
    "mas_vq_forward": (_I, [_P, _P, _L, _I, _I, _F, _P, _P, _P, _P, _Z, _P]),
    "mas_vq_forward_given": (_I, [_P, _P, _P, _L, _I, _I, _F, _P, _P, _P, _Z, _P]),
    "mas_kmeans_ws_bytes": (_Z, [_I, _I]),
    "mas_kmeans_update": (_I, [_P, _P, _L, _I, _I, _P, _P, _P, _P, _Z, _P]),
    "mas_vq_backward": (_I, [_P, _P, _P, _P, _P, _L, _I, _I, _F, _P, _P, _P]),
    "mas_vq_gather": (_I, [_P, _P, _L, _I, _I, _P, _P]),
    "mas_layernorm_forward": (_I, [_P, _P, _P, _P, _P, _P, _P, _L, _I, _F, _P]),
    "mas_layernorm_ws_bytes": (_Z, [_L, _I]),
    "mas_layernorm_backward": (_I, [_P, _P, _P, _P, _P, _P, _P, _P, _L, _I, _P, _Z, _P]),
    "mas_gelu_forward": (_I, [_P, _P, _L, _P]),
    "mas_gelu_backward": (_I, [_P, _P, _P, _L, _P]),
    "mas_softmax_causal_forward": (_I, [_P, _P, _L, _I, _I, _P]),
    "mas_embed3_forward": (_I, [_P, _P, _P, _P, _P, _P, _P, _L, _I, _I, _I, _I, _P]),
    "mas_embed3_backward": (_I, [_P, _P, _P, _P, _P, _P, _P, _L, _I, _I, _I, _I, _P]),
    "mas_linear_small": (_I, [_P, _L, _P, _P, _P, _L, _I, _I, _I, _I, _P]),
    "mas_kv_append": (_I, [_P, _I, _I, _I, _I, _P, _P, _I, _I, _P]),
    "mas_attn_decode": (_I, [_P, _P, _P, _P, _I, _I, _I, _I, _I, _P]),
    "mas_cfg_mix": (_I, [_P, _P, _P, _L, _F, _P]),
    "mas_attn_decode_append": (_I, [_P, _P, _P, _P, _I, _I, _I, _I, _I, _P]),
    "mas_layernorm2_forward": (_I, [_P, _P, _P, _P, _P, _P, _P, _P, _L, _I, _F, _F, _P]),
    "mas_sample_topk": (_I, [_P, _L, _I, _I, _F, _I, _P, _P, _P]),
    "mas_pack_gemm_tc16": (_I, [_P, _P, _I, _I, _I, _P]),
    "mas_gemm_rows_f16": (_I, [_P, _L, _I, _P, _P, _L, _I, _P, _P, _P, _F, _P]),
    "mas_wgrad_rows_f16_ws_bytes": (_Z, [_L, _I, _I]),
    "mas_wgrad_rows_f16": (_I, [_P, _P, _L, _I, _I, _P, _P, _P, _P, _P, _Z, _P]),
    "mas_attn_causal_forward": (_I, [_P, _P, _P, _P, _I, _I, _I, _I, _F, _P]),
    "mas_ce_forward": (_I, [_P, _L, _P, _P, _P, _P, _L, _I, _P]),
    "mas_ce_backward": (_I, [_P, _L, _P, _P, _P, _P, _P, _L, _L, _I, _P]),
    "mas_gemm_batched2": (_I, [_P, _P, _P, _I, _I, _I, _I, _I, _L, _L, _L, _L, _L, _L, _L, _L, _L, _I, _I, _F, _I, _I, _P]),
    "mas_softmax_causal_backward": (_I, [_P, _P, _P, _L, _I, _I, _F, _P]),
    "mas_bce_ws_bytes": (_Z, [_T]),
    "mas_bce_cl_ws_bytes": (_Z, [_I, _I, _I]),
    "mas_bce_cl_forward": (_I, [_P, _P, _P, _I, _I, _I, _I, _I, _P, _P, _Z, _P]),
    "mas_bce_cl_backward": (_I, [_P, _P, _P, _P, _I, _I, _I, _I, _I, _P, _P]),
    "mas_bce_logits": (_I, [_P, _T, _P, _T, _P, _P, _P, _T, _F, _P, _Z, _P]),
}

_lib = None


def exported_symbols():
    return sorted(_SPEC)


def load():
    global _lib
    if _lib is not None:
        return _lib
    if not os.path.exists(LIB_PATH):
        raise RuntimeError(
            f"libmas_b200.so not found at {LIB_PATH}: build it with `python -c 'import __graft_entry__ as g; g.build()'` "
            "(nvcc, sm_100a). There is no CPU/PyTorch fallback for this path.")
    lib = ctypes.CDLL(LIB_PATH)
    for name, (res, args) in _SPEC.items():
        fn = getattr(lib, name)
        fn.restype = res
        fn.argtypes = args
    _lib = lib
    return lib


def _ptr(t):
    if t is None:
        return None
    if isinstance(t, torch.Tensor):
        return ctypes.c_void_p(t.data_ptr())
    return t


def stream_ptr():
    return ctypes.c_void_p(torch.cuda.current_stream().cuda_stream)


_prof = None


def _device_of(args):
    for a in args:
        if isinstance(a, torch.Tensor) and a.is_cuda:
            return a.device
    return None


def call(name, *args):
    dev = _device_of(args)
    if dev is not None and dev.index != torch.cuda.current_device():
        with torch.cuda.device(dev):
            return call(name, *args)
    lib = load()
    fn = getattr(lib, name)
    conv = [_ptr(a) for a in args]
    conv.append(stream_ptr())
    if _prof is not None:
        e0, e1 = torch.cuda.Event(enable_timing=True), torch.cuda.Event(enable_timing=True)
        e0.record()
        rc = fn(*conv)
        e1.record()
        shp = ",".join("%dc%d" % (a.c, a.h) for a in args if isinstance(a, Tensor4))
        if not shp and name.startswith("mas_gn_"):
            ints = [a for a in args if isinstance(a, int) and not isinstance(a, bool)]
            shp = "x".join(str(v) for v in ints[:3])
        _prof.append((name + ("|" + shp if shp else ""), e0, e1))
    else:
        rc = fn(*conv)
    if rc != 0:
        raise RuntimeError(f"{name} failed ({rc}): {lib.mas_last_error().decode(errors='replace')}")


def profile_start():
    global _prof
    _prof = []


def profile_report(tag=None):
    global _prof
    torch.cuda.synchronize()
    agg = {}
    for name, e0, e1 in _prof or []:
        key = name if tag is None else tag(name)
        c, t = agg.get(key, (0, 0.0))
        agg[key] = (c + 1, t + e0.elapsed_time(e1))
    _prof = None
    return agg


def query(name, *args):
    return getattr(load(), name)(*[_ptr(a) for a in args])


def launch_count() -> int:
    return int(load().mas_launch_count())


def tc_launch_count() -> int:
    return int(load().mas_tc_launch_count())


def t4(x: torch.Tensor) -> Tensor4:
    n, c, h, w = x.shape
    sn, sc, sh, sw = x.stride()
    return Tensor4(n, h, w, c, sn, sh, sw, sc)


def rows4(m: int, c: int) -> Tensor4:
    return Tensor4(1, 1, m, c, m * c, m * c, c, 1)


_ws = {}


def workspace(nbytes: int, device) -> torch.Tensor:
    key = (device.type, device.index)
    buf = _ws.get(key)
    if buf is None or buf.numel() < nbytes:
        buf = torch.empty(max(int(nbytes), 1 << 20), dtype=torch.uint8, device=device)
        _ws[key] = buf
    return buf


def pin_workspaces():
    return list(_ws.values())
```

make-a-scene_b200/mas_b200/ops.py:

```python
from __future__ import annotations

import torch
import torch.distributed as dist

from . import _lib as L

GN_GROUPS = 32
GN_EPS = 1e-6

import os

_cfg = {"impl": L.IMPL_AUTO, "operands": os.environ.get("MAS_CONV_OPERANDS", "f16")}


def set_operand_format(fmt: str):
    if fmt not in ("f16", "tf32"):
        raise ValueError(fmt)
    _cfg["operands"] = fmt


def get_operand_format() -> str:
    return _cfg["operands"]


def amax(x):
    out = torch.empty(1, dtype=torch.float32, device=x.device)
    L.call("mas_amax", x, x.numel(), out)
    return out


def set_impl(impl: int):
    _cfg["impl"] = int(impl)


def get_impl() -> int:
    return _cfg["impl"]


def _need_cuda(x):
    if not x.is_cuda:
        raise RuntimeError("make-a-scene_b200 kernels run on CUDA (sm_100a) only; got a %s tensor — there is no CPU path"
                           % x.device.type)
    if x.dtype != torch.float32:
        raise RuntimeError("make-a-scene_b200 kernels take float32 tensors, got %s" % x.dtype)


def nhwc(x: torch.Tensor) -> torch.Tensor:
    _need_cuda(x)
    if x.dim() != 4:
        raise RuntimeError("expected a 4-D [N,C,H,W] tensor")
    if x.is_contiguous(memory_format=torch.channels_last) and x.stride(1) == 1:
        return x
    y = torch.empty_like(x, memory_format=torch.channels_last)
    L.call("mas_copy_strided", x, L.t4(x), y, L.t4(y))
    return y


def empty_nhwc(n, c, h, w, like):
    return torch.empty((n, c, h, w), dtype=torch.float32, device=like.device, memory_format=torch.channels_last)


def gn_stats(x):
    n, c, h, w = x.shape
    mean = torch.empty(n * GN_GROUPS, dtype=torch.float32, device=x.device)
    rstd = torch.empty_like(mean)
    nb = L.query("mas_gn_ws_bytes", n, h * w, c, GN_GROUPS)
    ws = L.workspace(nb, x.device)
    L.call("mas_gn_stats", x, n, h * w, c, GN_GROUPS, GN_EPS, mean, rstd, ws, ws.numel())
    return mean, rstd


def gn_apply(x, mean, rstd, gamma, beta, silu, rtf32=False):
    n, c, h, w = x.shape
    y = torch.empty_like(x)
    L.call("mas_gn_apply", x, mean, rstd, gamma, beta, y, n, h * w, c, GN_GROUPS, int(silu), int(rtf32))
    return y


def gn_backward(dy, x, mean, rstd, gamma, beta, silu, dx_add=None, want_act=False, act_f16=False, shadow=False, add_amax=None,
                shadow_only=False):
    n, c, h, w = x.shape
    shadow = shadow or shadow_only
    dx = None if shadow_only else torch.empty_like(x)
    dg = torch.empty_like(gamma)
    db = torch.empty_like(beta)
    act = torch.empty_like(x, dtype=torch.float16 if act_f16 else torch.float32) if want_act else None
    am = torch.empty(1, dtype=torch.float32, device=x.device) if (f16_operands() and not shadow_only) else None
    dx16 = bound = None
    if shadow:
        dx16 = torch.empty_like(x, dtype=torch.float16)
        bound = torch.empty(1, dtype=torch.float32, device=x.device)
        if dx_add is not None and add_amax is None:
            add_amax = amax_of(dx_add)
    nb = L.query("mas_gn_ws_bytes", n, h * w, c, GN_GROUPS)
    ws = L.workspace(nb, x.device)
    L.call("mas_gn_backward", dy, x, mean, rstd, gamma, beta, dx_add, dx, dg, db, act, int(act_f16 and want_act), am,
           add_amax if shadow else None, dx16, bound, n, h * w, c, GN_GROUPS, int(silu), ws, ws.numel())
    if shadow_only:
        dx = (dx16, bound)
    else:
        attach_amax(dx, am)
        if shadow:
            dx._mas_shadow = (dx16, bound, dx._version, dx.data_ptr())
    if want_act:
        return dx, dg, db, act
    return dx, dg, db


def shadow_of(t):
    st = getattr(t, "_mas_shadow", None)
    if st is not None and st[2] == t._version and st[3] == t.data_ptr() and st[0].device == t.device and st[0].shape == t.shape:
        return st[0], st[1]
    return None


def attach_amax(t, am):
    if am is not None:
        t._mas_amax = (am, t._version, t.data_ptr())
    return t


def amax_of(t):
    st = getattr(t, "_mas_amax", None)
    if st is not None and st[1] == t._version and st[2] == t.data_ptr() and st[0].device == t.device:
        return st[0]
    return amax(t)


def _conv_out_hw(h, w, mode):
    if mode == L.CONV_S1:
        return h, w
    if mode == L.CONV_S2:
        return h // 2, w // 2
    return 2 * h, 2 * w


def _tc_on():
    return _cfg["impl"] != L.IMPL_SIMT


def conv_tc_eligible(x, cout, mode):
    if not _tc_on() or not _is_dense_nhwc(x):
        return False
    n, _, h, w = x.shape
    ho, wo = _conv_out_hw(h, w, mode)
    ys = L.Tensor4(n, ho, wo, cout, ho * wo * cout, wo * cout, cout, 1)
    return bool(L.query("mas_conv3x3_tc_eligible", L.t4(x), ys, mode))


def gn_table(mean, rstd, gamma, beta, n, c):
    t = torch.empty((n, c, 2), dtype=torch.float32, device=mean.device)
    L.call("mas_gn_table", mean, rstd, gamma, beta, n, c, GN_GROUPS, t)
    return t


def _finalize_stats(part, tiles_per_image, n, c, hw):
    mean = torch.empty(n * GN_GROUPS, dtype=torch.float32, device=part.device)
    rstd = torch.empty_like(mean)
    L.call("mas_gn_finalize_partials", part, tiles_per_image, n, c, GN_GROUPS, hw, GN_EPS, mean, rstd)
    return mean, rstd


def conv3x3_raw(x, weight, bias, residual, mode, out_nchw=False, transpose=False, table=None, silu=True, want_stats=False,
                prepack=False, x_amax=None):
    n, _, h, w = x.shape
    cout = weight.shape[1] if transpose else weight.shape[0]
    cin = weight.shape[0] if transpose else weight.shape[1]
    ho, wo = _conv_out_hw(h, w, mode)
    if out_nchw:
        y = torch.empty((n, cout, ho, wo), dtype=torch.float32, device=x.device)
    else:
        y = empty_nhwc(n, cout, ho, wo, x)
    xs, ys = L.t4(x), L.t4(y)
    wc = weight.contiguous()
    stats = None
    if _tc_on() and not out_nchw and L.query("mas_conv3x3_tc_eligible", xs, ys, mode):
        f16 = _cfg["operands"] == "f16" and cin % 16 == 0
        wt = _packed_conv_weight(wc, weight, cout, cin, transpose, x.device, prepack, f16)
        part = None
        if want_stats and cout % (4 * GN_GROUPS) == 0:
            tiles = n * (ho // 16) * (wo // 8)
            part = torch.empty(tiles * cout * 2, dtype=torch.float32, device=x.device)
        if f16:
            xa = (x_amax if x_amax is not None else amax_of(x)) if table is None else None
            L.call("mas_conv3x3_fprop_tc16", x, xs, wt, bias, residual, y, ys, mode, table, int(silu), part, xa)
        else:
            L.call("mas_conv3x3_fprop_tc", x, xs, wt, bias, residual, y, ys, mode, table, int(silu), part)
        if part is not None:
            stats = _finalize_stats(part, (ho // 16) * (wo // 8), n, cout, ho * wo)
    else:
        if table is not None:
            raise RuntimeError("fused GroupNorm prologue requested for a shape that is not tensor-path eligible")
        if _cfg["impl"] == L.IMPL_TC:
            raise RuntimeError("IMPL_TC requested but the conv shape is not eligible for the tcgen05 kernel")
        wp = torch.empty(9 * cout * cin, dtype=torch.float32, device=x.device)
        L.call("mas_pack_conv3x3", wc, wp, weight.shape[0], weight.shape[1], int(transpose), 0)
        L.call("mas_conv3x3_fprop", x, xs, wp, bias, residual, y, ys, mode, L.IMPL_SIMT)
    if want_stats:
        return y, stats
    return y


def conv_tma_on():
    return f16_operands() and os.environ.get("MAS_CONV_TMA", "1") != "0"


def conv_h_eligible(n, cin, h, w, cout):
    return conv_tma_on() and cin % 64 == 0 and cout % 128 == 0 and h % 16 == 0 and w % 8 == 0


def to_half(x, x_amax=None):
    if not _is_dense_nhwc(x):
        raise RuntimeError("to_half expects a dense channels-last tensor")
    y = torch.empty_like(x, dtype=torch.float16)
    L.call("mas_to_half", x, y, x.numel(), x_amax)
    return y


def gn_apply_f16(x, mean, rstd, gamma, beta, silu):
    n, c, h, w = x.shape
    y = torch.empty_like(x, dtype=torch.float16)
    L.call("mas_gn_apply", x, mean, rstd, gamma, beta, y, n, h * w, c, GN_GROUPS, int(silu), 2)
    return y


def conv3x3_h_raw(x16, weight, bias, residual, transpose=False, want_stats=False, prepack=False, x_amax=None):
    n, _, h, w = x16.shape
    cout = weight.shape[1] if transpose else weight.shape[0]
    cin = weight.shape[0] if transpose else weight.shape[1]
    y = empty_nhwc(n, cout, h, w, x16)
    wt = _packed_conv_weight(weight.contiguous(), weight, cout, cin, transpose, x16.device, prepack, True)
    part = None
    if want_stats and cout % (4 * GN_GROUPS) == 0:
        part = torch.empty(n * (h // 16) * (w // 8) * cout * 2, dtype=torch.float32, device=x16.device)
    L.call("mas_conv3x3_fprop_tc16h", x16, L.t4(x16), wt, bias, residual, y, L.t4(y), part, x_amax)
    if want_stats:
        return y, (_finalize_stats(part, (h // 16) * (w // 8), n, cout, h * w) if part is not None else None)
    return y


_packs = {}


def _pack_entry(weight):
    k = id(weight)
    ent = _packs.get(k)
    if ent is not None and ent[0]() is weight and ent[1] == weight._version and ent[2] == weight.data_ptr():
        return ent[3]
    import weakref
    d = {}
    _packs[k] = (weakref.ref(weight, lambda _r, k=k: _packs.pop(k, None)), weight._version, weight.data_ptr(), d)
    return d


def _packed_conv_weight(wc, weight, cout, cin, transpose, dev, prepack=False, f16=False):
    ent = _pack_entry(weight)
    key = ("d" if transpose else "f", f16)
    hit = ent.get(key)
    if hit is not None and hit.device == dev:
        return hit
    dt = torch.float16 if f16 else torch.float32
    wt = torch.empty(9 * cout * cin, dtype=dt, device=dev)
    pair_ok = cout % 128 == 0 and cin % 128 == 0
    if prepack and not transpose and pair_ok:
        wd = torch.empty(9 * cout * cin, dtype=dt, device=dev)
        if f16:
            L.call("mas_pack_conv3x3_tc16", wc, wt, wd, weight.shape[0], weight.shape[1], 0)
        else:
            L.call("mas_pack_conv3x3_tc_pair", wc, wt, wd, weight.shape[0], weight.shape[1])
        ent[("d", f16)] = wd
    elif f16:
        L.call("mas_pack_conv3x3_tc16", wc, wt, None, weight.shape[0], weight.shape[1], int(transpose))
    else:
        L.call("mas_pack_conv3x3_tc", wc, wt, weight.shape[0], weight.shape[1], int(transpose))
    ent[key] = wt
    return wt


def conv3x3_wgrad_raw(x, dy, cout, cin, mode, want_bias=True, table=None, silu=True, dy_amax=None):
    dw = torch.empty((cout, cin, 3, 3), dtype=torch.float32, device=x.device)
    db = torch.empty(cout, dtype=torch.float32, device=x.device) if want_bias else None
    nb = L.query("mas_conv3x3_wgrad_ws_bytes", L.t4(x), L.t4(dy), mode)
    ws = L.workspace(nb, x.device)
    padded = cout != dy.shape[1]
    if (_tc_on() and _cfg["operands"] == "f16" and wgrad_f16_on() and _is_dense_nhwc(x) and _is_dense_nhwc(dy)
            and (padded or L.query("mas_conv3x3_wgrad_tc_eligible", L.t4(x), L.t4(dy), mode))):
        flags = int(x.dtype == torch.float16) | (2 if dy.dtype == torch.float16 else 0)
        if dy.dtype == torch.float16 and dy_amax is None:
            raise RuntimeError("an fp16 output-gradient shadow needs the device scalar its scale was derived from")
        L.call("mas_conv3x3_wgrad_tc16", x, flags, L.t4(x), dy, L.t4(dy), dw, db, mode, table, int(silu),
               dy_amax if dy_amax is not None else amax_of(dy), cout, ws, ws.numel())
        return dw, db
    if x.dtype == torch.float16 or dy.dtype == torch.float16:
        raise RuntimeError("fp16 operands can only feed the fp16-operand tensor-core weight gradient")
    if padded:
        raise RuntimeError("padded weight gradient needs the fp16 tensor-core kernel")
    L.call("mas_conv3x3_wgrad", x, L.t4(x), dy, L.t4(dy), dw, db, mode, _cfg["impl"], table, int(silu), ws, ws.numel())
    return dw, db


def wgrad_f16_eligible(x, dout, c1w):
    if not (f16_operands() and wgrad_f16_on() and _is_dense_nhwc(x) and _is_dense_nhwc(dout)):
        return False
    n, cin, h, w = x.shape
    cout = c1w.shape[0]
    return cin % 32 == 0 and cout % 128 == 0 and h % 8 == 0 and w % 8 == 0


def wgrad_f16_on():
    return os.environ.get("MAS_WGRAD_F16", "1") != "0"


def f16_operands():
    return _tc_on() and _cfg["operands"] == "f16"


def conv3x3_dgrad_raw(dy, weight, mode, dy_amax=None):
    if mode == L.CONV_S1:
        return conv3x3_raw(dy, weight, None, None, L.CONV_S1, transpose=True, x_amax=dy_amax)
    if mode == L.CONV_S2:
        return conv3x3_raw(dy, weight, None, None, L.CONV_ZS, transpose=True, x_amax=dy_amax)
    du = conv3x3_raw(dy, weight, None, None, L.CONV_S1, transpose=True, x_amax=dy_amax)
    n, cin, h2, w2 = du.shape
    dx = empty_nhwc(n, cin, h2 // 2, w2 // 2, du)
    L.call("mas_sumpool2x2", du, dx, n, h2 // 2, w2 // 2, cin)
    return dx


def gemm(A, B, C, M, N, K, batch=1, lda=None, ldb=None, ldc=None, sa=0, sb=0, sc=0, ta=False, tb=False, alpha=1.0,
         bias=None, residual=None, impl=None):
    def p(v):
        if isinstance(v, tuple):
            import ctypes
            t, off = v
            return ctypes.c_void_p(t.data_ptr() + 4 * off)
        return v
    L.call("mas_gemm", p(A), p(B), p(C), M, N, K, batch, lda, ldb, ldc, sa, sb, sc, int(ta), int(tb), float(alpha), p(bias),
           p(residual), _cfg["impl"] if impl is None else impl)


def gemm_w(A, lda, weight, C, ldc, M, transpose=False, alpha=1.0, bias=None, residual=None, stats_part=None):
    nout, kin = weight.shape[0], weight.shape[1]
    N, K = (kin, nout) if transpose else (nout, kin)
    w2 = weight.contiguous()
    if _tc_on() and N % 128 == 0 and K % 32 == 0 and lda % 4 == 0 and ldc % 4 == 0:
        import ctypes

        def p(v):
            return ctypes.c_void_p(v[0].data_ptr() + 4 * v[1]) if isinstance(v, tuple) else v
        dev = (A[0] if isinstance(A, tuple) else A).device
        wt = torch.empty(N * K, dtype=torch.float32, device=dev)
        L.call("mas_pack_gemm_tc", w2, wt, nout, kin, int(transpose))
        L.call("mas_gemm_rows_packed", p(A), lda, wt, p(C), ldc, M, N, K, float(alpha), bias, p(residual), stats_part)
        return True
    else:
        gemm(A, w2, C, M, N, K, lda=lda, ldb=kin, ldc=ldc, tb=not transpose, alpha=alpha, bias=bias, residual=residual)
        return False


def conv1x1_raw(x, weight, bias, residual=None):
    n, cin, h, w = x.shape
    cout = weight.shape[0]
    y = empty_nhwc(n, cout, h, w, x)
    gemm_w(x, cin, weight, y, cout, n * h * w, bias=bias, residual=residual)
    return y


def conv1x1_dgrad_raw(dy, weight, residual=None):
    n, cout, h, w = dy.shape
    cin = weight.shape[1]
    dx = empty_nhwc(n, cin, h, w, dy)
    gemm_w(dy, cout, weight, dx, cin, n * h * w, transpose=True, residual=residual)
    return dx


def conv1x1_wgrad_raw(x_rows, dy_rows, M, cin, cout, want_bias=True, ldx=None, ldy=None, dy_off=0):
    import ctypes
    dev = x_rows.device
    dy_ptr = ctypes.c_void_p(dy_rows.data_ptr() + 4 * dy_off)
    dw = torch.empty((cout, cin, 1, 1), dtype=torch.float32, device=dev)
    db = torch.empty(cout, dtype=torch.float32, device=dev) if want_bias else None
    nb = L.query("mas_conv1x1_wgrad_ws_bytes", M, cin, cout)
    ws = L.workspace(nb, dev)
    L.call("mas_conv1x1_wgrad", x_rows, ldx or cin, dy_ptr, ldy or cout, M, cin, cout, dw, db, _cfg["impl"], ws, ws.numel())
    return dw, db


def attach_stats(t, mean, rstd):
    if mean is not None:
        t._mas_gn = (mean, rstd, t._version)
    return t


def take_stats(t):
    st = getattr(t, "_mas_gn", None)
    if st is not None and st[2] == t._version and st[0].device == t.device:
        return st[0], st[1]
    return None, None


class GroupNormFn(torch.autograd.Function):

    @staticmethod
    def forward(ctx, x, weight, bias, silu):
        x = nhwc(x)
        mean, rstd = gn_stats(x)
        y = gn_apply(x, mean, rstd, weight, bias, silu)
        ctx.save_for_backward(x, weight, bias, mean, rstd)
        ctx.silu = silu
        return y

    @staticmethod
    def backward(ctx, dy):
        x, weight, bias, mean, rstd = ctx.saved_tensors
        dx, dg, db = gn_backward(nhwc(dy), x, mean, rstd, weight, bias, ctx.silu)
        return dx, dg, db, None


class SiLUFn(torch.autograd.Function):
    @staticmethod
    def forward(ctx, x):
        _need_cuda(x)
        x = x.contiguous() if not (x.is_contiguous() or x.is_contiguous(memory_format=torch.channels_last)) else x
        y = torch.empty_like(x)
        L.call("mas_silu_forward", x, y, x.numel())
        ctx.save_for_backward(x)
        return y

    @staticmethod
    def backward(ctx, dy):
        (x,) = ctx.saved_tensors
        if dy.stride() != x.stride():
            d2 = torch.empty_like(x)
            if x.dim() == 4:
                L.call("mas_copy_strided", dy, L.t4(dy), d2, L.t4(d2))
            else:
                d2.copy_(dy)
            dy = d2
        dx = torch.empty_like(x)
        L.call("mas_silu_backward", dy, x, dx, x.numel())
        return dx


def _is_dense_nhwc(t):
    return t.dim() == 4 and t.stride(1) == 1 and t.is_contiguous(memory_format=torch.channels_last)


class Conv3x3Fn(torch.autograd.Function):

    @staticmethod
    def forward(ctx, x, weight, bias, residual, mode, out_nchw):
        _need_cuda(x)
        cout, cin = weight.shape[0], weight.shape[1]
        n, _, h, w = x.shape
        edge = 0
        tc_pad_in = (mode == L.CONV_S1 and f16_operands() and residual is None and cout % 128 == 0 and h % 16 == 0 and w % 8 == 0
                     and (cin % 16 != 0) and (cin > 64 or cin <= 4))
        if mode == L.CONV_S1 and residual is None and cin == 3 and cout > 4 and not tc_pad_in:
            edge = 1
            y = empty_nhwc(n, cout, h, w, x)
            L.call("mas_edge_small_cin_fprop", x, L.t4(x), weight.contiguous(), bias, y, L.t4(y), 0)
        elif mode == L.CONV_S1 and residual is None and cout == 3 and cin > 4 and cin % 4 == 0 and cin <= 1024:
            edge = 2
            x = nhwc(x)
            y = (torch.empty((n, cout, h, w), dtype=torch.float32, device=x.device) if out_nchw else empty_nhwc(n, cout, h, w, x))
            L.call("mas_edge_small_cout_fprop", x, L.t4(x), weight.contiguous(), bias, y, L.t4(y))
        elif tc_pad_in:
            edge = 4
            cp = _round_up(cin, 32)
            x = pad_nhwc(x, cp)
            wp = torch.zeros((cout, cp, 3, 3), dtype=torch.float32, device=x.device)
            wp[:, :cin].copy_(weight.detach())
            y = conv3x3_raw(x, wp, bias, None, L.CONV_S1)
        elif (mode == L.CONV_S1 and f16_operands() and residual is None and cout % 128 != 0 and cout > 128 and cin % 16 == 0
              and h % 16 == 0 and w % 8 == 0):
            edge = 5
            x = nhwc(x)
            cpo, ck = _round_up(cout, 4), _round_up(cout, 128)
            wk = torch.zeros((ck, cin, 3, 3), dtype=torch.float32, device=x.device)
            wk[:cout].copy_(weight.detach())
            bk = torch.zeros(ck, dtype=torch.float32, device=x.device)
            if bias is not None:
                bk[:cout].copy_(bias.detach())
            wt = torch.empty(9 * ck * cin, dtype=torch.float16, device=x.device)
            L.call("mas_pack_conv3x3_tc16", wk, wt, None, ck, cin, 0)
            full = torch.empty((n, h, w, cpo), dtype=torch.float32, device=x.device).permute(0, 3, 1, 2)
            L.call("mas_conv3x3_fprop_tc16", x, L.t4(x), wt, bk, None, full, L.t4(full), L.CONV_S1, None, 0, None, amax_of(x))
            y = full[:, :cout]
        elif (mode == L.CONV_S2 and _tc_on() and residual is None and not out_nchw and _is_dense_nhwc(x) and cin % 8 == 0
              and cout % 128 == 0 and h % 32 == 0 and w % 16 == 0):
            edge = 3
            x4 = empty_nhwc(n, 4 * cin, h // 2, w // 2, x)
            L.call("mas_space_to_depth", x, x4, n, h, w, cin)
            w9 = torch.empty((cout, 4 * cin, 3, 3), dtype=torch.float32, device=x.device)
            L.call("mas_s2d_pack_weights", weight.contiguous(), w9, cout, cin)
            y = conv3x3_raw(x4, w9, bias, None, L.CONV_S1)
            x = x4
        else:
            y = conv3x3_raw(x, weight, bias, residual, mode, out_nchw, prepack=ctx.needs_input_grad[0])
        ctx.save_for_backward(x, weight)
        ctx.mode, ctx.has_bias, ctx.has_res, ctx.edge = mode, bias is not None, residual is not None, edge
        return y



    @staticmethod
    def backward(ctx, dy):
        x, weight = ctx.saved_tensors
        cout, cin = weight.shape[0], weight.shape[1]
        dx = dw = db = dres = None
        want_w = ctx.needs_input_grad[1] or (ctx.has_bias and ctx.needs_input_grad[2])
        if ctx.edge == 1:
            if ctx.needs_input_grad[0]:
                dx = conv3x3_dgrad_raw(dy, weight, ctx.mode)
            if want_w:
                dyd = nhwc(dy)
                dw = torch.empty_like(weight)
                db = torch.empty(cout, dtype=torch.float32, device=x.device)
                ws = L.workspace(L.query("mas_edge_wgrad_ws_bytes", cout), x.device)
                L.call("mas_edge_small_cin_wgrad", x, L.t4(x), dyd, L.t4(dyd), dw, db, ws, ws.numel())
        elif ctx.edge == 2:
            n, _, h, w = x.shape
            if ctx.needs_input_grad[0]:
                dx = empty_nhwc(n, cin, h, w, x)
                L.call("mas_edge_small_cin_fprop", dy, L.t4(dy), weight.contiguous(), None, dx, L.t4(dx), 1)
            if want_w:
                dw = torch.empty_like(weight)
                db = torch.empty(cout, dtype=torch.float32, device=x.device)
                ws = L.workspace(L.query("mas_edge_wgrad_ws_bytes", cin), x.device)
                L.call("mas_edge_small_cout_wgrad", x, L.t4(x), dy, L.t4(dy), dw, db, ws, ws.numel())
        elif ctx.edge == 4:
            cp = x.shape[1]
            dy = nhwc(dy)
            am = amax_of(dy)
            if want_w:
                dwp, db = conv3x3_wgrad_raw(x, dy, cout, cp, L.CONV_S1, ctx.has_bias, dy_amax=am)
                dw = dwp[:, :cin].contiguous()
            if ctx.needs_input_grad[0]:
                wp = torch.zeros((cout, cp, 3, 3), dtype=torch.float32, device=x.device)
                wp[:, :cin].copy_(weight.detach())
                dx = conv3x3_dgrad_raw(dy, wp, L.CONV_S1, am)[:, :cin]
        elif ctx.edge == 5:
            cpo, ck = _round_up(cout, 4), _round_up(cout, 128)
            full = getattr(dy, "_mas_pad_base", None)
            if full is None or full.shape[1] != cpo or full.data_ptr() != dy.data_ptr() or not _is_dense_nhwc(full):
                full = pad_nhwc(dy.contiguous() if not dy.is_contiguous() and _cl_pitch(dy) is None else dy, cpo)
            am = amax_of(full)
            if ctx.needs_input_grad[0]:
                w160 = torch.zeros((cpo, cin, 3, 3), dtype=torch.float32, device=x.device)
                w160[:cout].copy_(weight.detach())
                dx = conv3x3_raw(full, w160, None, None, L.CONV_S1, transpose=True, x_amax=am)
            if want_w:
                dwk, dbk = conv3x3_wgrad_raw(x, full, ck, cin, L.CONV_S1, True, dy_amax=am)
                dw, db = dwk[:cout].contiguous(), dbk[:cout].contiguous()
        elif ctx.edge == 3:
            if ctx.needs_input_grad[0]:
                dx = conv3x3_dgrad_raw(nhwc(dy), weight, ctx.mode)
            if want_w:
                dw9, db = conv3x3_wgrad_raw(x, nhwc(dy), cout, 4 * cin, L.CONV_S1, ctx.has_bias)
                dw = torch.empty_like(weight)
                L.call("mas_s2d_unpack_wgrad", dw9, dw, cout, cin)
        else:
            dy = nhwc(dy)
            am = amax_of(dy) if f16_operands() else None
            if ctx.needs_input_grad[0]:
                dx = conv3x3_dgrad_raw(dy, weight, ctx.mode, am)
            if want_w:
                dw, db = conv3x3_wgrad_raw(x, dy, cout, cin, ctx.mode, ctx.has_bias, dy_amax=am)
        if not ctx.has_bias:
            db = None
        if ctx.has_res and ctx.needs_input_grad[3]:
            dres = dy
        return dx, dw, db, dres, None, None


class Conv1x1Fn(torch.autograd.Function):

    @staticmethod
    def forward(ctx, x, weight, bias):
        x = nhwc(x)
        y = conv1x1_raw(x, weight, bias)
        ctx.save_for_backward(x, weight)
        ctx.has_bias = bias is not None
        return y

    @staticmethod
    def backward(ctx, dy):
        x, weight = ctx.saved_tensors
        dy = nhwc(dy)
        n, cin, h, w = x.shape
        cout = weight.shape[0]
        dx = conv1x1_dgrad_raw(dy, weight) if ctx.needs_input_grad[0] else None
        dw, db = conv1x1_wgrad_raw(x, dy, n * h * w, cin, cout, ctx.has_bias)
        return dx, dw, db


class ResnetBlockFn(torch.autograd.Function):

    @staticmethod
    def forward(ctx, x, mean_in, rstd_in, n1w, n1b, c1w, c1b, n2w, n2b, c2w, c2b, sw, sb, dx_shadow=False):
        x = nhwc(x)
        n, cin, h, w = x.shape
        cout = c1w.shape[0]
        if mean_in is None:
            mean_in, rstd_in = gn_stats(x)
        m1, r1 = mean_in, rstd_in
        fused = conv_tc_eligible(x, cout, L.CONV_S1) and cin % 8 == 0 and cout % (4 * GN_GROUPS) == 0
        hmode = (fused and conv_h_eligible(n, cin, h, w, cout) and conv_h_eligible(n, cout, h, w, cout)
                 and wgrad_f16_on() and cin % 32 == 0)
        sc = x if sw is None else conv1x1_raw(x, sw, sb)
        if hmode:
            a1 = gn_apply_f16(x, m1, r1, n1w, n1b, True)
            h1, st2 = conv3x3_h_raw(a1, c1w, c1b, None, want_stats=True, prepack=ctx.needs_input_grad[0])
            m2, r2 = st2
            a2 = gn_apply_f16(h1, m2, r2, n2w, n2b, True)
            out, st_out = conv3x3_h_raw(a2, c2w, c2b, sc, want_stats=True, prepack=any(ctx.needs_input_grad))
            if not any(ctx.needs_input_grad):
                a1 = a2 = None
        elif fused:
            t1 = gn_table(m1, r1, n1w, n1b, n, cin)
            h1, st2 = conv3x3_raw(x, c1w, c1b, None, L.CONV_S1, table=t1, want_stats=True, prepack=ctx.needs_input_grad[0])
            m2, r2 = st2
            t2 = gn_table(m2, r2, n2w, n2b, n, cout)
            out, st_out = conv3x3_raw(h1, c2w, c2b, sc, L.CONV_S1, table=t2, want_stats=True, prepack=any(ctx.needs_input_grad))
            a1 = a2 = None
        else:
            a1 = gn_apply(x, m1, r1, n1w, n1b, True)
            h1 = conv3x3_raw(a1, c1w, c1b, None, L.CONV_S1, prepack=ctx.needs_input_grad[0])
            m2, r2 = gn_stats(h1)
            a2 = gn_apply(h1, m2, r2, n2w, n2b, True)
            out = conv3x3_raw(a2, c2w, c2b, sc, L.CONV_S1, prepack=any(ctx.needs_input_grad))
            st_out = None
        ctx.save_for_backward(x, h1, a1, a2, m1, r1, m2, r2, n1w, n1b, c1w, n2w, n2b, c2w, sw)
        ctx.has_sc, ctx.fused = sw is not None, fused and not hmode
        ctx.hmode, ctx.dx_shadow = hmode, bool(dx_shadow) and hmode and sw is None
        if st_out is None:
            mo = ro = None
        else:
            mo, ro = st_out
            ctx.mark_non_differentiable(mo, ro)
        ctx.set_materialize_grads(False)
        return out, mo, ro

    @staticmethod
    def backward(ctx, dout, _gm, _gr):
        if dout is None:
            return (None,) * 14
        x, h1, a1, a2, m1, r1, m2, r2, n1w, n1b, c1w, n2w, n2b, c2w, sw = ctx.saved_tensors
        dout = nhwc(dout)
        cout, cin = c1w.shape[0], c1w.shape[1]
        n, _, h, w = x.shape
        am_out = amax_of(dout) if f16_operands() else None
        hmode = ctx.hmode and conv_tma_on()
        sh_out = shadow_of(dout) if hmode else None
        if hmode and sh_out is None and am_out is not None:
            sh_out = (to_half(dout, am_out), am_out)
        if sh_out is not None:
            d_a2 = conv3x3_h_raw(sh_out[0], c2w, None, None, transpose=True, x_amax=sh_out[1])
        else:
            d_a2 = conv3x3_dgrad_raw(dout, c2w, L.CONV_S1, am_out)
        a16 = ctx.fused and wgrad_f16_eligible(x, dout, c1w)
        sh_h1 = None
        if ctx.fused:
            d_h1, dn2w, dn2b, a2 = gn_backward(d_a2, h1, m2, r2, n2w, n2b, True, want_act=True, act_f16=a16)
        elif hmode:
            sh_h1, dn2w, dn2b = gn_backward(d_a2, h1, m2, r2, n2w, n2b, True, shadow_only=True)
        else:
            d_h1, dn2w, dn2b = gn_backward(d_a2, h1, m2, r2, n2w, n2b, True)
        del d_a2
        if sh_out is not None and a2.dtype == torch.float16:
            dc2w, dc2b = conv3x3_wgrad_raw(a2, sh_out[0], cout, cout, L.CONV_S1, dy_amax=sh_out[1])
        else:
            dc2w, dc2b = conv3x3_wgrad_raw(a2, dout, cout, cout, L.CONV_S1, dy_amax=am_out)
        del a2, sh_out
        if sh_h1 is not None:
            d_h1, am_h1 = sh_h1
            d_a1 = conv3x3_h_raw(d_h1, c1w, None, None, transpose=True, x_amax=am_h1)
        else:
            am_h1 = amax_of(d_h1) if f16_operands() else None
            d_a1 = conv3x3_dgrad_raw(d_h1, c1w, L.CONV_S1, am_h1)
        del sh_h1
        if ctx.has_sc:
            r_ = gn_backward(d_a1, x, m1, r1, n1w, n1b, True, want_act=ctx.fused, act_f16=a16)
            dxm, dn1w, dn1b = r_[0], r_[1], r_[2]
            if ctx.fused:
                a1 = r_[3]
            dx = conv1x1_dgrad_raw(dout, sw, residual=dxm)
            dsw, dsb = conv1x1_wgrad_raw(x, dout, n * h * w, cin, cout)
        else:
            r_ = gn_backward(d_a1, x, m1, r1, n1w, n1b, True, dx_add=dout, want_act=ctx.fused, act_f16=a16,
                             shadow=ctx.dx_shadow and hmode, add_amax=am_out)
            dx, dn1w, dn1b = r_[0], r_[1], r_[2]
            if ctx.fused:
                a1 = r_[3]
            dsw = dsb = None
        del d_a1
        dc1w, dc1b = conv3x3_wgrad_raw(a1, d_h1, cout, cin, L.CONV_S1, dy_amax=am_h1)
        del a1, d_h1
        return dx, None, None, dn1w, dn1b, dc1w, dc1b, dn2w, dn2b, dc2w, dc2b, dsw, dsb, None


class AttnBlockFn(torch.autograd.Function):

    @staticmethod
    def forward(ctx, x, mean_in, rstd_in, nw, nb, qw, qb, kw, kb, vw, vb, pw, pb):
        x = nhwc(x)
        n, c, h, w = x.shape
        hw, M = h * w, n * h * w
        if mean_in is None:
            mean_in, rstd_in = gn_stats(x)
        mean, rstd = mean_in, rstd_in
        dev = x.device
        hn = empty_nhwc(n, c, h, w, x)
        qkv = torch.empty((M, 3 * c), dtype=torch.float32, device=dev)
        P = torch.empty((n, hw, hw), dtype=torch.float32, device=dev)
        O = empty_nhwc(n, c, h, w, x)
        out = empty_nhwc(n, c, h, w, x)
        part = None
        if _tc_on() and hw % 128 == 0 and c % 128 == 0:
            part = torch.empty((M // 128) * c * 2, dtype=torch.float32, device=dev)
        ws = L.workspace(L.query("mas_attnblock_ws_bytes", n, hw, c, GN_GROUPS), dev)
        L.call("mas_attnblock_forward", x, n, hw, c, GN_GROUPS, mean, rstd, nw, nb, qw.contiguous(), qb, kw.contiguous(), kb,
               vw.contiguous(), vb, pw.contiguous(), pb, hn, qkv, P, O, out, part, _cfg["impl"], ws, ws.numel())
        ctx.save_for_backward(x, mean, rstd, hn, qkv, P, O, nw, nb, qw, kw, vw, pw)
        ctx.set_materialize_grads(False)
        if part is not None:
            mo, ro = _finalize_stats(part, hw // 128, n, c, hw)
            ctx.mark_non_differentiable(mo, ro)
            return out, mo, ro
        return out, None, None

    @staticmethod
    def backward(ctx, dout, _gm, _gr):
        if dout is None:
            return (None,) * 13
        x, mean, rstd, hn, qkv, P, O, nw, nb, qw, kw, vw, pw = ctx.saved_tensors
        dout = nhwc(dout)
        n, c, h, w = x.shape
        hw = h * w
        dev = x.device
        dx = torch.empty_like(x)
        dnw, dnb = torch.empty_like(nw), torch.empty_like(nb)
        dqkv_w = torch.empty((3 * c,) + tuple(qw.shape[1:]), dtype=torch.float32, device=dev)
        dqkv_b = torch.empty(3 * c, dtype=torch.float32, device=dev)
        dpw = torch.empty_like(pw, memory_format=torch.contiguous_format)
        dpb = torch.empty(c, dtype=torch.float32, device=dev)
        ws = L.workspace(L.query("mas_attnblock_ws_bytes", n, hw, c, GN_GROUPS), dev)
        am = torch.empty(1, dtype=torch.float32, device=dev) if f16_operands() else None
        L.call("mas_attnblock_backward", dout, x, n, hw, c, GN_GROUPS, mean, rstd, nw, nb, qw.contiguous(), kw.contiguous(),
               vw.contiguous(), pw.contiguous(), hn, qkv, P, O, dx, dnw, dnb, dqkv_w, dqkv_b, dpw, dpb, am, _cfg["impl"], ws,
               ws.numel())
        attach_amax(dx, am)
        return (dx, None, None, dnw, dnb, dqkv_w[:c], dqkv_b[:c], dqkv_w[c:2 * c], dqkv_b[c:2 * c], dqkv_w[2 * c:], dqkv_b[2 * c:],
                dpw, dpb)


class BatchNormFn(torch.autograd.Function):

    @staticmethod
    def forward(ctx, x, weight, bias, running_mean, running_var, momentum, eps, sync):
        x = nhwc(x)
        n, c, h, w = x.shape
        R = n * h * w
        buf = torch.empty(2 * c + 1, dtype=torch.float64, device=x.device)
        L.call("mas_bn_stats", x, R, c, buf)
        world = 1
        if sync and dist.is_available() and dist.is_initialized() and dist.get_world_size() > 1:
            world = dist.get_world_size()
            dist.all_reduce(buf)
        mean = torch.empty(c, dtype=torch.float32, device=x.device)
        invstd = torch.empty_like(mean)
        L.call("mas_bn_finalize", buf, 0.0, c, float(eps), float(momentum), mean, invstd, running_mean, running_var)
        y = torch.empty_like(x)
        L.call("mas_bn_apply", x, mean, invstd, weight, bias, y, R, c)
        ctx.save_for_backward(x, weight, mean, invstd)
        ctx.world = world
        return y

    @staticmethod
    def backward(ctx, dy):
        x, weight, mean, invstd = ctx.saved_tensors
        dy = nhwc(dy)
        n, c, h, w = x.shape
        R = n * h * w
        local = torch.empty(2 * c + 1, dtype=torch.float64, device=x.device)
        L.call("mas_bn_backward_reduce", dy, x, mean, invstd, R, c, local)
        glob = local
        if ctx.world > 1:
            glob = local.clone()
            dist.all_reduce(glob)
        dx = torch.empty_like(x)
        dg = torch.empty_like(weight)
        db = torch.empty_like(weight)
        L.call("mas_bn_backward_apply", dy, x, mean, invstd, weight, glob, local, 0.0, dx, dg, db, R, c)
        return dx, dg, db, None, None, None, None, None


def batchnorm_eval(x, weight, bias, running_mean, running_var, eps):
    x = nhwc(x)
    n, c, h, w = x.shape
    invstd = torch.empty_like(running_var)
    L.call("mas_bn_invstd", running_var, float(eps), invstd, c)
    y = torch.empty_like(x)
    L.call("mas_bn_apply", x, running_mean, invstd, weight, bias, y, n * h * w, c)
    return y


class VQFn(torch.autograd.Function):

    @staticmethod
    def forward(ctx, z, E, beta):
        z = nhwc(z)
        n, d, h, w = z.shape
        R, K = n * h * w, E.shape[0]
        E = E.contiguous()
        idx = torch.empty(R, dtype=torch.int64, device=z.device)
        zq = torch.empty_like(z)
        loss = torch.empty((), dtype=torch.float32, device=z.device)
        nb = L.query("mas_vq_ws_bytes", R, K, d)
        ws = L.workspace(nb, z.device)
        L.call("mas_vq_forward", z, E, R, K, d, float(beta), idx, zq, loss, ws, ws.numel())
        ctx.save_for_backward(z, E, idx)
        ctx.beta = float(beta)
        ctx.mark_non_differentiable(idx)
        return zq, loss, idx

    @staticmethod
    def backward(ctx, g_zq, g_loss, _g_idx):
        z, E, idx = ctx.saved_tensors
        n, d, h, w = z.shape
        R, K = n * h * w, E.shape[0]
        g_zq = nhwc(g_zq) if g_zq is not None else None
        if g_loss is not None:
            g_loss = g_loss.contiguous()
        grad_z = torch.empty_like(z) if ctx.needs_input_grad[0] else None
        grad_E = torch.zeros_like(E) if ctx.needs_input_grad[1] else None
        L.call("mas_vq_backward", g_zq, g_loss, z, E, idx, R, K, d, ctx.beta, grad_z, grad_E)
        return grad_z, grad_E, None


def vq_select_path(tensor_core_filter: bool):
    rc = L.load().mas_vq_select_path(1 if tensor_core_filter else 0)
    if rc != 0:
        raise RuntimeError("mas_vq_select_path failed")


class VQGivenFn(torch.autograd.Function):

    @staticmethod
    def forward(ctx, z, E, beta, idx):
        z = nhwc(z)
        n, d, h, w = z.shape
        R, K = n * h * w, E.shape[0]
        E = E.contiguous()
        idx = idx.contiguous().view(-1)
        if idx.numel() != R or idx.dtype != torch.int64:
            raise RuntimeError("VQGivenFn: need %d int64 indices" % R)
        zq = torch.empty_like(z)
        loss = torch.empty((), dtype=torch.float32, device=z.device)
        ws = L.workspace(L.query("mas_vq_ws_bytes", R, K, d), z.device)
        L.call("mas_vq_forward_given", z, E, idx, R, K, d, float(beta), zq, loss, ws, ws.numel())
        ctx.save_for_backward(z, E, idx)
        ctx.beta = float(beta)
        return zq, loss

    @staticmethod
    def backward(ctx, g_zq, g_loss):
        z, E, idx = ctx.saved_tensors
        n, d, h, w = z.shape
        R, K = n * h * w, E.shape[0]
        g_zq = nhwc(g_zq) if g_zq is not None else None
        if g_loss is not None:
            g_loss = g_loss.contiguous()
        grad_z = torch.empty_like(z) if ctx.needs_input_grad[0] else None
        grad_E = torch.zeros_like(E) if ctx.needs_input_grad[1] else None
        L.call("mas_vq_backward", g_zq, g_loss, z, E, idx, R, K, d, ctx.beta, grad_z, grad_E)
        return grad_z, grad_E, None, None


def vq_gather(E, idx):
    R, (K, D) = idx.numel(), E.shape
    out = torch.empty((R, D), dtype=torch.float32, device=E.device)
    L.call("mas_vq_gather", E.contiguous(), idx.contiguous().view(-1), R, K, D, out)
    return out


def _round_up(v, m):
    return (v + m - 1) // m * m


def pad_nhwc(x, cp):
    _need_cuda(x)
    n, c, h, w = x.shape
    base = torch.empty((n, h, w, cp), dtype=torch.float32, device=x.device)
    if x.is_contiguous() and c * 33 * 4 <= 48 * 1024:
        L.call("mas_nchw_to_nhwc_pad", x, base, n, c, cp, h, w)
    else:
        if cp > c:
            base[..., c:].zero_()
        view = base.permute(0, 3, 1, 2)[:, :c]
        L.call("mas_copy_strided", x, L.t4(x), view, L.t4(view))
    return base.permute(0, 3, 1, 2)


def _cl_pitch(t):
    if t.dim() != 4 or t.stride(1) != 1:
        return None
    n, c, h, w = t.shape
    pitch = t.stride(3)
    if pitch < c or t.stride(2) != w * pitch or (n > 1 and t.stride(0) != h * w * pitch):
        return None
    return pitch


class BCELogitsFn(torch.autograd.Function):

    @staticmethod
    def forward(ctx, logits, target, pos_weight):
        _need_cuda(logits)
        n, c, h, w = logits.shape
        loss = torch.empty((), dtype=torch.float32, device=logits.device)
        cp = _cl_pitch(logits)
        if cp is not None and target.is_contiguous() and w % 32 == 0 and c * 33 * 4 <= 48 * 1024:
            ws = L.workspace(L.query("mas_bce_cl_ws_bytes", n, h, w), logits.device)
            L.call("mas_bce_cl_forward", logits, target, pos_weight, n, c, cp, h, w, loss, ws, ws.numel())
            ctx.save_for_backward(logits, target, pos_weight)
            ctx.cp = cp
            return loss
        grad = torch.empty_like(logits)
        nb = L.query("mas_bce_ws_bytes", L.t4(logits))
        ws = L.workspace(nb, logits.device)
        L.call("mas_bce_logits", logits, L.t4(logits), target, L.t4(target), pos_weight, loss, grad, L.t4(grad),
               1.0 / logits.numel(), ws, ws.numel())
        ctx.save_for_backward(grad)
        ctx.cp = None
        return loss

    @staticmethod
    def backward(ctx, g):
        g = g.contiguous()
        if ctx.cp is None:
            (grad,) = ctx.saved_tensors
            out = torch.empty_like(grad)
            src = grad if grad.is_contiguous() or grad.is_contiguous(memory_format=torch.channels_last) else grad.contiguous()
            out = torch.empty_like(src)
            L.call("mas_scale_by", src, g, out, src.numel())
            return out, None, None
        logits, target, pw = ctx.saved_tensors
        n, c, h, w = logits.shape
        base = torch.empty((n, h, w, ctx.cp), dtype=torch.float32, device=logits.device)
        L.call("mas_bce_cl_backward", logits, target, pw, g, n, c, ctx.cp, h, w, base)
        full = base.permute(0, 3, 1, 2)
        grad = full[:, :c]
        grad._mas_pad_base = full
        return grad, None, None


class LayerNormFn(torch.autograd.Function):

    @staticmethod
    def forward(ctx, x, weight, bias, residual, eps):
        _need_cuda(x)
        x = x.contiguous()
        H = x.shape[-1]
        R = x.numel() // H
        y = torch.empty_like(x)
        mean = torch.empty(R, dtype=torch.float32, device=x.device)
        rstd = torch.empty_like(mean)
        res = residual.contiguous() if residual is not None else None
        L.call("mas_layernorm_forward", x, weight, bias, res, y, mean, rstd, R, H, float(eps))
        ctx.save_for_backward(x, weight, mean, rstd)
        ctx.has_res = residual is not None
        return y

    @staticmethod
    def backward(ctx, dy):
        x, weight, mean, rstd = ctx.saved_tensors
        dy = dy.contiguous()
        H = x.shape[-1]
        R = x.numel() // H
        dx = torch.empty_like(x)
        dg = torch.empty_like(weight)
        db = torch.empty_like(weight)
        ws = L.workspace(L.query("mas_layernorm_ws_bytes", R, H), x.device)
        L.call("mas_layernorm_backward", dy, x, mean, rstd, weight, dx, dg, db, R, H, ws, ws.numel())
        return dx, dg, db, (dy if ctx.has_res else None), None


class GeluFn(torch.autograd.Function):
    @staticmethod
    def forward(ctx, x):
        _need_cuda(x)
        x = x.contiguous()
        y = torch.empty_like(x)
        L.call("mas_gelu_forward", x, y, x.numel())
        ctx.save_for_backward(x)
        return y

    @staticmethod
    def backward(ctx, dy):
        (x,) = ctx.saved_tensors
        dx = torch.empty_like(x)
        L.call("mas_gelu_backward", dy.contiguous(), x, dx, x.numel())
        return dx


def linear_f16_on(nout, kin):
    return f16_operands() and nout % 128 == 0 and kin % 128 == 0 and os.environ.get("MAS_LINEAR_F16", "1") != "0"


def _packed_linear_weight(weight, transpose, dev):
    ent = _pack_entry(weight)
    key = ("lin16", bool(transpose))
    hit = ent.get(key)
    if hit is not None and hit.device == dev:
        return hit
    n, k = weight.shape
    wt = torch.empty(n * k, dtype=torch.float16, device=dev)
    L.call("mas_pack_gemm_tc16", weight.contiguous(), wt, n, k, int(transpose))
    ent[key] = wt
    return wt


def rows_to_half(x2d):
    am = amax(x2d)
    x16 = torch.empty(x2d.shape, dtype=torch.float16, device=x2d.device)
    L.call("mas_to_half", x2d, x16, x2d.numel(), am)
    return x16, am


def gemm_rows_f16(x16, am, weight, transpose=False, bias=None):
    M, kc = x16.shape
    nout = weight.shape[1] if transpose else weight.shape[0]
    y = torch.empty((M, nout), dtype=torch.float32, device=x16.device)
    L.call("mas_gemm_rows_f16", x16, M, kc, _packed_linear_weight(weight, transpose, x16.device), y, nout, nout, bias, None, am, 1.0)
    return y


def wgrad_rows_f16(x16, am_x, dy16, am_dy, want_bias=True):
    M, K = x16.shape
    N = dy16.shape[1]
    dw = torch.empty((N, K), dtype=torch.float32, device=x16.device)
    db = torch.empty(N, dtype=torch.float32, device=x16.device) if want_bias else None
    ws = L.workspace(L.query("mas_wgrad_rows_f16_ws_bytes", M, N, K), x16.device)
    L.call("mas_wgrad_rows_f16", x16, dy16, M, N, K, dw, db, am_x, am_dy, ws, ws.numel())
    return dw, db


class LinearFn(torch.autograd.Function):

    @staticmethod
    def forward(ctx, x, weight, bias):
        _need_cuda(x)
        x = x.contiguous()
        K, N = x.shape[-1], weight.shape[0]
        R = x.numel() // K
        ctx.f16 = linear_f16_on(N, K)
        ctx.has_bias = bias is not None
        ctx.xshape = x.shape
        if ctx.f16:
            x16, am = rows_to_half(x.view(R, K))
            y = gemm_rows_f16(x16, am, weight, False, bias).view(x.shape[:-1] + (N,))
            ctx.save_for_backward(x16, am, weight)
            return y
        y = torch.empty(x.shape[:-1] + (N,), dtype=torch.float32, device=x.device)
        gemm_w(x, K, weight, y, N, R, bias=bias)
        ctx.save_for_backward(x, weight)
        return y

    @staticmethod
    def backward(ctx, dy):
        dy = dy.contiguous()
        if ctx.f16:
            x16, am_x, weight = ctx.saved_tensors
            N, K = weight.shape
            R = x16.shape[0]
            dy16, am_dy = rows_to_half(dy.view(R, N))
            dx = gemm_rows_f16(dy16, am_dy, weight, True).view(ctx.xshape) if ctx.needs_input_grad[0] else None
            dw, db = wgrad_rows_f16(x16, am_x, dy16, am_dy, ctx.has_bias)
            return dx, dw, db
        x, weight = ctx.saved_tensors
        K, N = x.shape[-1], weight.shape[0]
        R = x.numel() // K
        dx = None
        if ctx.needs_input_grad[0]:
            dx = torch.empty_like(x)
            gemm_w(dy, N, weight, dx, K, R, transpose=True)
        dw, db = conv1x1_wgrad_raw(x, dy, R, K, N, ctx.has_bias)
        return dx, dw.view(N, K), db


def _attn_impl(S_, hd):
    if _tc_on() and S_ % 64 == 0 and hd % 64 == 0:
        return L.IMPL_TC3
    return None


def gemm2(A, B, C, M, N, K, outer, batch, lda, ldb, ldc, osa, osb, osc, sa, sb, sc, ta=False, tb=False, alpha=1.0, impl=None, causal=0):
    import ctypes

    def at(v, o):
        t, off = v if isinstance(v, tuple) else (v, 0)
        return ctypes.c_void_p(t.data_ptr() + 4 * (off + o))
    step = max(1, 65535 // batch)
    for o0 in range(0, outer, step):
        n = min(step, outer - o0)
        L.call("mas_gemm_batched2", at(A, o0 * osa), at(B, o0 * osb), at(C, o0 * osc), M, N, K, n, batch, lda, ldb, ldc, osa, osb, osc,
               sa, sb, sc, int(ta), int(tb), float(alpha), _cfg["impl"] if impl is None else impl, int(causal))


def attn_causal_fused_on(S_, hd):
    return _tc_on() and hd == 64 and S_ % 128 == 0 and S_ >= 128 and os.environ.get("MAS_ATTN_FUSED", "1") != "0"


class CausalAttentionFn(torch.autograd.Function):

    @staticmethod
    def forward(ctx, qkv, heads):
        _need_cuda(qkv)
        qkv = qkv.contiguous()
        B, S_, H3 = qkv.shape
        H = H3 // 3
        hd = H // heads
        alpha = 1.0 / float(hd) ** 0.5
        impl = _attn_impl(S_, hd)
        P = torch.empty((B, heads, S_, S_), dtype=torch.float32, device=qkv.device)
        ctxv = torch.empty((B, S_, H), dtype=torch.float32, device=qkv.device)
        SS = S_ * S_
        if attn_causal_fused_on(S_, hd):
            L.call("mas_attn_causal_forward", qkv, amax(qkv), P, ctxv, B, S_, heads, hd, alpha)
        else:
            gemm2(qkv, (qkv, H), P, S_, S_, hd, B, heads, H3, H3, S_, S_ * H3, S_ * H3, heads * SS, hd, hd, SS, tb=True, alpha=alpha,
                  impl=impl, causal=3)
            L.call("mas_softmax_causal_forward", P, P, B * heads, S_, S_)
            gemm2(P, (qkv, 2 * H), ctxv, S_, hd, S_, B, heads, S_, H3, H, heads * SS, S_ * H3, S_ * H, SS, hd, hd, impl=impl, causal=1)
        ctx.save_for_backward(qkv, P)
        ctx.heads = heads
        return ctxv

    @staticmethod
    def backward(ctx, dctx):
        qkv, P = ctx.saved_tensors
        dctx = dctx.contiguous()
        heads = ctx.heads
        B, S_, H3 = qkv.shape
        H = H3 // 3
        hd = H // heads
        alpha = 1.0 / float(hd) ** 0.5
        impl = _attn_impl(S_, hd)
        dqkv = torch.empty_like(qkv)
        dP = torch.empty_like(P)
        SS = S_ * S_
        oq, op_, oc = S_ * H3, heads * SS, S_ * H
        gemm2(P, dctx, (dqkv, 2 * H), S_, hd, S_, B, heads, S_, H, H3, op_, oc, oq, SS, hd, hd, ta=True, impl=impl, causal=2)
        gemm2(dctx, (qkv, 2 * H), dP, S_, S_, hd, B, heads, H, H3, S_, oc, oq, op_, hd, hd, SS, tb=True, impl=impl, causal=3)
        L.call("mas_softmax_causal_backward", P, dP, dP, B * heads, S_, S_, alpha)
        gemm2(dP, (qkv, H), dqkv, S_, hd, S_, B, heads, S_, H3, H3, op_, oq, oq, SS, hd, hd, impl=impl, causal=1)
        gemm2(dP, qkv, (dqkv, H), S_, hd, S_, B, heads, S_, H3, H3, op_, oq, oq, SS, hd, hd, ta=True, impl=impl, causal=2)
        return dqkv, None


class CrossEntropyFn(torch.autograd.Function):

    @staticmethod
    def forward(ctx, logits, target):
        _need_cuda(logits)
        V = logits.shape[-1]
        lg = logits.reshape(-1, V)
        if lg.stride(-1) != 1:
            lg = lg.contiguous()
        tg = target.reshape(-1).to(torch.int64).contiguous()
        R = lg.shape[0]
        if tg.numel() != R:
            raise ValueError("cross_entropy: %d logit rows vs %d targets" % (R, tg.numel()))
        rows = torch.empty(R, dtype=torch.float32, device=lg.device)
        lse = torch.empty(R, dtype=torch.float32, device=lg.device)
        out = torch.empty(2, dtype=torch.float32, device=lg.device)
        L.call("mas_ce_forward", lg, lg.stride(0), tg, rows, lse, out, R, V)
        ctx.save_for_backward(lg, tg, lse, out)
        ctx.shape = logits.shape
        return out[0]

    @staticmethod
    def backward(ctx, dloss):
        lg, tg, lse, out = ctx.saved_tensors
        R, V = lg.shape
        d = torch.empty((R, V), dtype=torch.float32, device=lg.device)
        L.call("mas_ce_backward", lg, lg.stride(0), tg, lse, out, dloss.contiguous().to(torch.float32), d, V, R, V)
        return d.view(ctx.shape), None


def cross_entropy(logits, target):
    return CrossEntropyFn.apply(logits, target)


def sample_topk(logits, temperature, top_k, u):
    _need_cuda(logits)
    logits = logits.contiguous()
    R, V = logits.shape
    tok = torch.empty(R, dtype=torch.int64, device=logits.device)
    L.call("mas_sample_topk", logits, V, R, V, float(temperature), int(top_k) if top_k else 0, u.contiguous(), tok)
    return tok


def linear_small(x, weight, bias, act=0):
    _need_cuda(x)
    x = x.contiguous()
    R, K = x.shape
    N = weight.shape[0]
    y = torch.empty((R, N), dtype=torch.float32, device=x.device)
    L.call("mas_linear_small", x, K, weight.contiguous(), bias, y, N, R, N, K, int(act))
    return y


def kv_append(qkv, kcache, vcache, pos0):
    R, heads, Tmax, hd = kcache.shape
    T = qkv.shape[1]
    L.call("mas_kv_append", qkv.contiguous(), R, T, heads, hd, kcache, vcache, Tmax, int(pos0))


def attn_decode(qkv, kcache, vcache, length):
    R, heads, Tmax, hd = kcache.shape
    ctx = torch.empty((R, heads * hd), dtype=torch.float32, device=qkv.device)
    L.call("mas_attn_decode", qkv.contiguous(), kcache, vcache, ctx, R, heads, hd, Tmax, int(length))
    return ctx


def attn_decode_append(qkv, kcache, vcache, pos):
    R, heads, Tmax, hd = kcache.shape
    ctx = torch.empty((R, heads * hd), dtype=torch.float32, device=qkv.device)
    L.call("mas_attn_decode_append", qkv.contiguous(), kcache, vcache, ctx, R, heads, hd, Tmax, int(pos))
    return ctx


def layernorm2(x, ln1, residual, ln2):
    _need_cuda(x)
    x = x.contiguous()
    R, H = x.shape
    y1, y2 = torch.empty_like(x), torch.empty_like(x)
    L.call("mas_layernorm2_forward", x, ln1.weight, ln1.bias, None if residual is None else residual.contiguous(), y1, ln2.weight,
           ln2.bias, y2, R, H, float(ln1.eps), float(ln2.eps))
    return y1, y2


def cfg_mix(cond, uncond, scale):
    out = torch.empty_like(cond)
    L.call("mas_cfg_mix", cond.contiguous(), uncond.contiguous(), out, cond.numel(), float(scale))
    return out


class EmbedFn(torch.autograd.Function):

    @staticmethod
    def forward(ctx, segs, total, H, *tables):
        dev = tables[0].device
        B = segs[0][0].shape[0]
        out = torch.empty((B, total, H), dtype=torch.float32, device=dev)
        for i, (ids, pa, pb, off) in enumerate(segs):
            t0, t1, t2 = tables[3 * i:3 * i + 3]
            Lg = ids.shape[1]
            L.call("mas_embed3_forward", t0, ids.contiguous(), t1, pa, t2 if pb is not None else None, pb, out, B * Lg, H, Lg, total, off)
        ctx.segs, ctx.total, ctx.H = segs, total, H
        ctx.shapes = [t.shape for t in tables]
        return out

    @staticmethod
    def backward(ctx, dout):
        dout = dout.contiguous()
        grads = []
        for i, (ids, pa, pb, off) in enumerate(ctx.segs):
            d0 = torch.zeros(ctx.shapes[3 * i], dtype=torch.float32, device=dout.device)
            d1 = torch.zeros(ctx.shapes[3 * i + 1], dtype=torch.float32, device=dout.device)
            d2 = torch.zeros(ctx.shapes[3 * i + 2], dtype=torch.float32, device=dout.device) if pb is not None else None
            Lg = ids.shape[1]
            L.call("mas_embed3_backward", dout, ids.contiguous(), d0, pa, d1, pb, d2, ids.shape[0] * Lg, ctx.H, Lg, ctx.total, off)
            grads += [d0, d1, d2]
        return (None, None, None) + tuple(grads)
```

Before: 388.6.

## Skip structurally-zero taps in space-to-depth and zero-stuffed 3x3 convolutions

Adds an S2D conv mode so the fprop and wgrad kernels skip MMA issues for taps that are structurally zero after space-to-depth weight packing, writing zeros for dead wgrad taps. It also adds a phase-decomposed fp16 kernel for zero-stuffed (transposed/dgrad) convolutions that issues only the taps live for each output parity. The goal is to cut tensor-core work that only multiplies padded zeros. The cost is more template variants, extra branching in the MMA issue loop, and environment switches to fall back to the dense path.

```diff
diff --git a/include/mas_b200.h b/include/mas_b200.h
--- a/include/mas_b200.h
+++ b/include/mas_b200.h
@@ -18,6 +18,7 @@
 #define MAS_CONV_S2 1
 #define MAS_CONV_UP 2
 #define MAS_CONV_ZS 3
+#define MAS_CONV_S2D 4
 
 #define MAS_IMPL_AUTO 0
 #define MAS_IMPL_SIMT 1
diff --git a/make-a-scene_b200/csrc/contract_tc.cu b/make-a-scene_b200/csrc/contract_tc.cu
--- a/make-a-scene_b200/csrc/contract_tc.cu
+++ b/make-a-scene_b200/csrc/contract_tc.cu
@@ -33,23 +33,31 @@
   float* stats_part;
   const float* x_amax;
   int Cstore;
+  int s2d_c;
 };
 
-template <int TAPS, int KC, int STAGES, int TILES, bool F16>
+__device__ __forceinline__ uint32_t s2d_live_taps(int py, int px) {
+  const uint32_t cols = px ? 0x2u : 0x6u;
+  return (cols << 3) | (py ? 0u : cols << 6);
+}
+
+template <int TAPS, int KC, int STAGES, int TILES, bool F16, bool PH = false>
 __global__ void __launch_bounds__(NTHREADS, (TILES == 2) ? 2 : 1) shift_gemm_tc(const Params p) {
+  static_assert(!PH || (TAPS == 9 && TILES == 2 && F16), "the phase-decomposed data gradient is an fp16 3x3 kernel with two phases per CTA");
+  constexpr int STILES = PH ? 1 : TILES;
   constexpr int EPC = F16 ? 8 : 4;
   constexpr int SLOTS = (TAPS == 9) ? 180 : 132;
   constexpr int ROWP = (TAPS == 9) ? 10 : 8;
   constexpr int LBO_A = SLOTS * 16;
   constexpr int SBO_A = ROWP * 16;
   constexpr int A_TILE = (KC / EPC) * LBO_A;
-  constexpr int A_STAGE = TILES * A_TILE;
+  constexpr int A_STAGE = STILES * A_TILE;
   constexpr int LBO_B = BN * 16;
   constexpr int B_TAP = (KC / EPC) * LBO_B;
   constexpr int B_STAGE = TAPS * B_TAP;
   constexpr int STAGE = A_STAGE + B_STAGE;
   constexpr int QUADS = KC / EPC;
-  constexpr int ITEMS = TILES * SLOTS * QUADS;
+  constexpr int ITEMS = STILES * SLOTS * QUADS;
   constexpr int LPI = F16 ? 2 : 1;
   constexpr int PER_THREAD = (ITEMS + NPROD - 1) / NPROD;
   static_assert((SLOTS % 8) == 4, "A plane pitch must be 64 mod 128 bytes for conflict-free producer stores");
@@ -64,7 +72,8 @@
   const uint32_t accum_bar = bar_base + 8u * (2 * STAGES);
 
   const int tid = threadIdx.x, warp = tid >> 5, lane = tid & 31;
-  const int64_t tile0 = (int64_t)blockIdx.x * TILES;
+  const int64_t tile0 = PH ? (int64_t)(blockIdx.x >> 1) : (int64_t)blockIdx.x * TILES;
+  const int pp = PH ? (int)(blockIdx.x & 1) : 0;
   const int n0 = blockIdx.y * BN;
   const int nchunks = p.Cin / KC;
 
@@ -200,8 +209,9 @@
     const int sub_r = lane >> 3, sub_c = lane & 7;
 #pragma unroll 1
     for (int tl = 0; tl < TILES; ++tl) {
-      const int64_t tile = tile0 + tl;
+      const int64_t tile = PH ? tile0 : tile0 + tl;
       if (tile >= p.total_tiles) break;
+      const int py = PH ? tl : 0, px = PH ? (pp ? 1 - tl : tl) : 0;
       int64_t pix_base = 0;
       int tx_ = 0, ty_ = 0, n_img = 0;
       if (TAPS == 9) {
@@ -229,7 +239,8 @@
           const int row = i * 4 + sub_r;
           const int m = lane_grp * 32 + row;
           int64_t pix;
-          if (TAPS == 9) pix = ((int64_t)n_img * p.Hout + ty_ * 16 + (m >> 3)) * p.Wout + tx_ * 8 + (m & 7);
+          if (PH) pix = ((int64_t)n_img * p.Hout + 2 * (ty_ * 16 + (m >> 3)) + py) * p.Wout + 2 * (tx_ * 8 + (m & 7)) + px;
+          else if (TAPS == 9) pix = ((int64_t)n_img * p.Hout + ty_ * 16 + (m >> 3)) * p.Wout + tx_ * 8 + (m & 7);
           else pix = pix_base + m;
           if (TAPS == 9 || pix < (int64_t)p.N * p.Hout * p.Wout) {
             float4 o = *reinterpret_cast<const float4*>(patch + row * EP_LD + sub_c * 4);
@@ -271,18 +282,44 @@
         const uint64_t a_base = make_desc(a_st, LBO_A, SBO_A);
         const uint64_t b_base = make_desc(a_st + A_STAGE, LBO_B, 128);
         const uint32_t acc0 = (kc > 0) ? 1u : 0u;
-        if (elect_one()) {
+        uint32_t live = 0x1FFu;
+        int t_first = 0;
+        if (TAPS == 9 && p.s2d_c) {
+          const int sub = kc * KC / p.s2d_c;
+          live = s2d_live_taps(sub >> 1, sub & 1);
+          t_first = 4;
+        }
+        if (PH) {
+          if (elect_one()) {
+#pragma unroll
+            for (int tl = 0; tl < TILES; ++tl) {
+              const int py = tl, px = pp ? 1 - tl : tl;
+#pragma unroll
+              for (int t = 0; t < 9; ++t) {
+                const int ty = t / 3, tx = t % 3;
+                if ((ty & 1) != py || (tx & 1) != px) continue;
+                const uint32_t tapoff = (uint32_t)((((ty + py) >> 1) * 10 + ((tx + px) >> 1)) * 16);
+                const uint64_t ad = a_base + (uint64_t)(tapoff >> 4);
+                const uint64_t bd = b_base + (uint64_t)((t * B_TAP) >> 4);
+                mma_f16_ss(tmem_base + (uint32_t)(tl * BN), ad, bd, idesc, (t > py * 3 + px) ? 1u : acc0);
+              }
+            }
+            mma_commit(empty_bar(stage));
+            if (kc == nchunks - 1) mma_commit(accum_bar);
+          }
+        } else if (elect_one()) {
 #pragma unroll
           for (int tl = 0; tl < TILES; ++tl) {
 #pragma unroll
             for (int t = 0; t < TAPS; ++t) {
+              if (!((live >> t) & 1u)) continue;
               const uint32_t tapoff = (TAPS == 9) ? (uint32_t)(((t / 3) * 10 + (t % 3)) * 16) : 0u;
 #pragma unroll
               for (int k8 = 0; k8 < KC / (2 * EPC); ++k8) {
                 const uint64_t ad = a_base + (uint64_t)((tl * A_TILE + tapoff + k8 * 2 * LBO_A) >> 4);
                 const uint64_t bd = b_base + (uint64_t)((t * B_TAP + k8 * 2 * LBO_B) >> 4);
-                if (F16) mma_f16_ss(tmem_base + (uint32_t)(tl * BN), ad, bd, idesc, (t > 0 || k8 > 0) ? 1u : acc0);
-                else mma_tf32_ss(tmem_base + (uint32_t)(tl * BN), ad, bd, idesc, (t > 0 || k8 > 0) ? 1u : acc0);
+                if (F16) mma_f16_ss(tmem_base + (uint32_t)(tl * BN), ad, bd, idesc, (t > t_first || k8 > 0) ? 1u : acc0);
+                else mma_tf32_ss(tmem_base + (uint32_t)(tl * BN), ad, bd, idesc, (t > t_first || k8 > 0) ? 1u : acc0);
               }
             }
           }
@@ -550,15 +587,23 @@
           const uint64_t a_base = make_desc(a_st, LBO_A, SBO_A);
           const uint64_t b_base = make_desc(a_st + A_STAGE, LBO_B, 128);
           const uint32_t acc0 = (kc > 0) ? 1u : 0u;
+          uint32_t live = 0x1FFu;
+          int t_first = 0;
+          if (p.s2d_c) {
+            const int sub = kc * KC / p.s2d_c;
+            live = s2d_live_taps(sub >> 1, sub & 1);
+            t_first = 4;
+          }
           if (elect_one()) {
 #pragma unroll
             for (int tl = 0; tl < TILES; ++tl) {
 #pragma unroll
               for (int t = 0; t < TAPS; ++t) {
+                if (!((live >> t) & 1u)) continue;
                 const uint32_t tapoff = (uint32_t)(((t / 3) * 10 + (t % 3)) * 16);
                 const uint64_t ad = a_base + (uint64_t)((tl * A_TILE + tapoff) >> 4);
                 const uint64_t bd = b_base + (uint64_t)((t * B_TAP) >> 4);
-                mma_f16_ss(acc + (uint32_t)(tl * BN), ad, bd, idesc, t > 0 ? 1u : acc0);
+                mma_f16_ss(acc + (uint32_t)(tl * BN), ad, bd, idesc, t > t_first ? 1u : acc0);
               }
             }
             mma_commit(empty_bar(stage));
@@ -597,10 +642,10 @@
   return (size_t)P_STAGES * (2 * 2 * 180 * 16 + 9 * 2 * BN * 16) + 4 * 32 * 36 * 4 + (2 * P_STAGES + 4) * 8 + 16;
 }
 
-template <int TAPS, int KC, int STAGES, int TILES, bool F16>
+template <int TAPS, int KC, int STAGES, int TILES, bool F16, bool PH = false>
 constexpr size_t smem_bytes() {
   constexpr int SLOTS = (TAPS == 9) ? 180 : 132, EPC = F16 ? 8 : 4;
-  return (size_t)STAGES * (TILES * (KC / EPC) * SLOTS * 16 + TAPS * (KC / EPC) * BN * 16) + (2 * STAGES + 1) * 8 + 16;
+  return (size_t)STAGES * ((PH ? 1 : TILES) * (KC / EPC) * SLOTS * 16 + TAPS * (KC / EPC) * BN * 16) + (2 * STAGES + 1) * 8 + 16;
 }
 
 __global__ void pack_weights_tc(const float* __restrict__ w, float* __restrict__ out, int Cout, int Cin, int taps, int KC, int transpose) {
@@ -688,6 +733,8 @@
   int Cout_real;
   int x_f16;
   int dy_f16;
+  int s2d_c;
+  int s2d_n64;
 };
 
 template <int TAPS, bool PRO, bool F16>
@@ -705,6 +752,8 @@
   constexpr int NMMA = COPIES * NT;
   constexpr uint32_t idesc = F16 ? (make_idesc_f16(NMMA) | (1u << 16))
                                  : ((1u << 4) | (2u << 7) | (2u << 10) | ((uint32_t)(NMMA >> 3) << 17) | ((uint32_t)(BM >> 4) << 24));
+  constexpr uint32_t idesc_n2 = make_idesc_f16(2 * NT) | (1u << 16), idesc_n1 = make_idesc_f16(NT) | (1u << 16);
+  constexpr int OCTS16 = NT / 8;
 
   extern __shared__ __align__(1024) uint8_t smem[];
   uint8_t* dy_smem = smem + (size_t)WG_STAGES * B_STAGE;
@@ -721,6 +770,10 @@
   const int ci0 = blockIdx.x * NT, co0 = blockIdx.y * BM, split = blockIdx.z;
   const int64_t u0 = (int64_t)split * p.units_per_split;
   const int64_t u1 = min(p.total_units, u0 + p.units_per_split);
+  const int s2d_sub = p.s2d_c ? ci0 / p.s2d_c : 0;
+  const int s2d_py = s2d_sub >> 1, s2d_px = s2d_sub & 1;
+  const uint32_t tap_live = (F16 && p.s2d_c) ? s2d_live_taps(s2d_py, s2d_px) : 0x1FFu;
+  const uint32_t dx_live = (F16 && p.s2d_c) ? (s2d_px ? 0x2u : 0x6u) : 0x7u;
 
   if (tid == 0) {
     for (int s = 0; s < WG_STAGES; ++s) {
@@ -747,6 +800,7 @@
       sl_o[i] = item % OCTS;
       sl_r[i] = slot / 10;
       sl_c[i] = item < ITEMS16 ? slot % 10 : -100;
+      if (p.s2d_c && (sl_r[i] == 0 || sl_c[i] == 0 || (s2d_py && sl_r[i] == 9) || (s2d_px && sl_c[i] == 9))) sl_c[i] = -100;
     }
     int pux = (int)(u0 % p.units_x), puy = (int)((u0 / p.units_x) % p.units_y), pn = (int)(u0 / ((int64_t)p.units_x * p.units_y));
     int cux = 0, cuy = 0, cn = 0;
@@ -825,7 +879,7 @@
           const int slot = sl_r[i] * 10 + sl_c[i];
 #pragma unroll
           for (int dx = 0; dx < 3; ++dx)
-            if (sl_c[i] >= dx) *reinterpret_cast<uint4*>(b_st + (dx * OCTS + sl_o[i]) * P16 + (slot - dx) * 16) = h;
+            if (sl_c[i] >= dx && (dx_live >> dx) & 1) *reinterpret_cast<uint4*>(b_st + (dx * OCTS + sl_o[i]) * P16 + (slot - dx) * 16) = h;
         }
       }
       fence_proxy_async();
@@ -841,6 +895,11 @@
 #pragma unroll 1
       for (int t = 0; t < TAPS; ++t) {
         float* o = p.part + (((size_t)split * TAPS + t) * p.Cout + co) * p.Cin + ci0;
+        if (!((tap_live >> t) & 1u)) {
+#pragma unroll
+          for (int q = 0; q < 8; ++q) *reinterpret_cast<float4*>(o + q * 4) = make_float4(0.f, 0.f, 0.f, 0.f);
+          continue;
+        }
         float v[32];
         tmem_ld32(tmem_base + ((uint32_t)(warp * 32) << 16) + (uint32_t)(t * NT), v);
 #pragma unroll
@@ -1077,7 +1136,19 @@
         const uint64_t b16 = make_desc(b_st, 160, P16);
         const uint32_t acc0 = (u > u0) ? 1u : 0u;
         if (elect_one()) {
-          if (F16) {
+          if (F16 && p.s2d_c) {
+#pragma unroll
+            for (int r = 0; r < 8; r += 2) {
+#pragma unroll
+              for (int dyy = 1; dyy < 3; ++dyy) {
+                if (dyy == 2 && s2d_py) continue;
+                const uint64_t bd = b16 + (uint64_t)(((r + dyy) * 160 + OCTS16 * P16) >> 4);
+                const uint32_t d = tmem_base + (uint32_t)(dyy * NMMA + NT);
+                if (s2d_px && !p.s2d_n64) mma_f16_ts(d, a_t + (uint32_t)(r * 4), bd, idesc_n1, r > 0 ? 1u : acc0);
+                else mma_f16_ts(d, a_t + (uint32_t)(r * 4), bd, idesc_n2, r > 0 ? 1u : acc0);
+              }
+            }
+          } else if (F16) {
 #pragma unroll
             for (int r = 0; r < 8; r += 2) {
 #pragma unroll
@@ -1232,6 +1303,11 @@
   return MAS_OK;
 }
 
+static bool s2d_dense() {
+  const char* e = getenv("MAS_S2D_DENSE");
+  return e && e[0] == '1';
+}
+
 int conv3x3_fprop_tc_launch(const float* x, mas_tensor4 xs, const float* w_tc, const float* bias, const float* res, float* y,
                             mas_tensor4 ys, int mode, const float* gn_table, int gn_silu, float* stats_part, int f16,
                             const float* x_amax, cudaStream_t st) {
@@ -1239,7 +1315,13 @@
   if (f16 && Cin % 16) return fail(MAS_ERR_UNSUPPORTED, "tc conv (fp16 operands): Cin=%d must be a multiple of 16", Cin);
   if (Cstore % 4) return fail(MAS_ERR_UNSUPPORTED, "tc conv: Cout=%d must be a multiple of 4", Cstore);
   if (Cstore != Cout && (res || stats_part)) return fail(MAS_ERR_UNSUPPORTED, "tc conv: residual / statistics epilogues need Cout %% 128 == 0");
-  if (!(mode == MAS_CONV_S1 || mode == MAS_CONV_UP || mode == MAS_CONV_ZS)) return fail(MAS_ERR_UNSUPPORTED, "tc conv: mode %d", mode);
+  if (!(mode == MAS_CONV_S1 || mode == MAS_CONV_UP || mode == MAS_CONV_ZS || mode == MAS_CONV_S2D))
+    return fail(MAS_ERR_UNSUPPORTED, "tc conv: mode %d", mode);
+  const bool s2d = mode == MAS_CONV_S2D;
+  if (s2d) {
+    if (Cin % 64) return fail(MAS_ERR_UNSUPPORTED, "tc conv (space-to-depth): Cin=%d must be 4 x a multiple of 16", Cin);
+    mode = MAS_CONV_S1;
+  }
   if (!dense_nhwc(xs) || !dense_nhwc(ys) || Cin % 8 || ys.h % 16 || ys.w % 8 || !al16p(x) || !al16p(y) ||
       (res && !al16p(res)) || (bias && !al16p(bias)) || !al16p(w_tc))
     return fail(MAS_ERR_UNSUPPORTED, "tc conv: shape/layout not eligible (Cin=%d Cout=%d Hout=%lld Wout=%lld)", Cin, Cout,
@@ -1256,15 +1338,26 @@
   p.alpha = 1.0f;
   p.gn_table = gn_table; p.gn_silu = gn_silu; p.stats_part = stats_part;
   p.x_amax = f16 ? x_amax : nullptr;
+  p.s2d_c = s2d ? Cin / 4 : 0;
   if (gn_table && !al16p(gn_table)) return fail(MAS_ERR_INVALID_ARG, "tc conv: gn_table must be 16-byte aligned");
   constexpr int T = 2, STG = 2;
   constexpr size_t smem = tc::smem_bytes<9, 8, STG, T, false>();
   static_assert(smem == tc::smem_bytes<9, 16, STG, T, true>(), "both operand formats stage the same bytes per K chunk");
+  constexpr size_t smem_ph = tc::smem_bytes<9, 16, STG, T, true, true>();
   static std::atomic<uint64_t> configured{0};
   if (first_on_device(configured)) {
     if (int e = set_smem(tc::shift_gemm_tc<9, 8, STG, T, false>, smem)) return e;
     if (int e = set_smem(tc::shift_gemm_tc<9, 16, STG, T, true>, smem)) return e;
+    if (int e = set_smem(tc::shift_gemm_tc<9, 16, STG, T, true, true>, smem_ph)) return e;
     mark_device(configured);
+  }
+  if (f16 && mode == MAS_CONV_ZS && !res && !stats_part && !gn_table && xs.h % 16 == 0 && xs.w % 8 == 0 && !s2d_dense()) {
+    p.map = tc::MAP_S1;
+    p.tiles_x = (int)(xs.w / 8); p.tiles_y = (int)(xs.h / 16);
+    p.total_tiles = (int64_t)p.N * p.tiles_x * p.tiles_y;
+    dim3 gph((unsigned)(2 * p.total_tiles), (unsigned)(Cout / tc::BN));
+    tc::shift_gemm_tc<9, 16, STG, T, true, true><<<gph, tc::NTHREADS, smem_ph, st>>>(p);
+    return launched_tc("shift_gemm_tc<9,f16,phases>");
   }
   dim3 grid((unsigned)cdiv(p.total_tiles, T), (unsigned)(Cout / tc::BN));
   if (f16) {
@@ -1306,7 +1399,7 @@
   p.tiles_x = 1; p.tiles_y = 1;
   p.total_tiles = cdiv(M, tc::BM);
   p.alpha = alpha;
-  p.gn_table = nullptr; p.gn_silu = 0; p.stats_part = stats_part; p.x_amax = nullptr; p.Cstore = N;
+  p.gn_table = nullptr; p.gn_silu = 0; p.stats_part = stats_part; p.x_amax = nullptr; p.Cstore = N; p.s2d_c = 0;
   if (stats_part && (M % tc::BM || ldc != N)) return fail(MAS_ERR_UNSUPPORTED, "tc gemm: fused statistics need M %% 128 == 0 and a dense output");
   constexpr size_t smem = tc::smem_bytes<1, 32, 2, 2, false>();
   static std::atomic<uint64_t> configured{0};
@@ -1405,12 +1498,14 @@
 int conv_wgrad_tc_launch(const float* x, mas_tensor4 xs, const float* dy, mas_tensor4 dys, float* dw, float* dbias, int mode,
                          const float* gn_table, int gn_silu, int f16, const float* dy_amax, int cout_rows, int x_f16, void* ws,
                          size_t ws_bytes, cudaStream_t st) {
-  const int dy_f16 = (x_f16 >> 1) & 1;
+  const int dy_f16 = (x_f16 >> 1) & 1, s2d = (x_f16 >> 2) & 1;
   x_f16 &= 1;
+  if (s2d && (!f16 || gn_table || mode != MAS_CONV_S1 || xs.c % (4 * tc::WG_NT)))
+    return fail(MAS_ERR_INVALID_ARG, "tc wgrad: a space-to-depth x needs the fp16-operand kernel, mode S1, no prologue and Cin %% 128 == 0");
   if (x_f16 && (!f16 || gn_table)) return fail(MAS_ERR_INVALID_ARG, "tc wgrad: an fp16 x needs the fp16-operand kernel and no prologue");
   if (dy_f16 && (!f16 || !dy_amax || dys.c % 8)) return fail(MAS_ERR_INVALID_ARG, "tc wgrad: an fp16 dy needs the fp16-operand kernel, its scale source and Cout %% 8 == 0");
   static const bool tma_off = [] { const char* e = getenv("MAS_WGRAD_TMA"); return e && e[0] == '0'; }();
-  if (f16 && x_f16 && dy_f16 && mode == MAS_CONV_S1 && !gn_table && !tma_off && conv_wgrad_t16_ok(xs, dys) &&
+  if (f16 && x_f16 && dy_f16 && mode == MAS_CONV_S1 && !gn_table && !s2d && !tma_off && conv_wgrad_t16_ok(xs, dys) &&
       cout_rows == (int)(cdiv(dys.c, tc::BM) * tc::BM))
     return conv_wgrad_t16_launch(x, xs, dy, dys, dw, dbias, dy_amax, ws, ws_bytes, st);
   const bool pad_ok = cout_rows == (int)(cdiv(dys.c, tc::BM) * tc::BM);
@@ -1425,6 +1520,8 @@
   p.total_units = (int64_t)p.N * p.units_x * p.units_y;
   p.rows = 0; p.ldx = p.Cin; p.ldy = p.Cout_real;
   p.gn_table = gn_table; p.gn_silu = gn_silu; p.dy_amax = f16 ? dy_amax : nullptr; p.x_f16 = x_f16; p.dy_f16 = dy_f16;
+  p.s2d_c = s2d ? p.Cin / 4 : 0;
+  { const char* e = getenv("MAS_S2D_WGRAD_N64"); p.s2d_n64 = e && e[0] == '1'; }
   const int splits = wgrad_tc_splits((p.Cout / tc::BM) * (xs.c / tc::WG_NT), p.total_units);
   if (f16) return gn_table ? wgrad_tc_run<9, true, true>(p, splits, dw, dbias, ws, st) : wgrad_tc_run<9, false, true>(p, splits, dw, dbias, ws, st);
   return gn_table ? wgrad_tc_run<9, true, false>(p, splits, dw, dbias, ws, st) : wgrad_tc_run<9, false, false>(p, splits, dw, dbias, ws, st);
@@ -1447,7 +1544,7 @@
   p.units_x = 1; p.units_y = 1;
   p.total_units = cdiv(M, 64);
   p.rows = M; p.ldx = ldx; p.ldy = ldy;
-  p.gn_table = nullptr; p.gn_silu = 0; p.dy_amax = nullptr; p.x_f16 = 0; p.dy_f16 = 0;
+  p.gn_table = nullptr; p.gn_silu = 0; p.dy_amax = nullptr; p.x_f16 = 0; p.dy_f16 = 0; p.s2d_c = 0; p.s2d_n64 = 0;
   const int splits = wgrad_tc_splits((int64_t)(Cout / tc::BM) * (Cin / 128), p.total_units);
   return wgrad_tc_run<1, false, false>(p, splits, dw, dbias, ws, st);
 }
diff --git a/make-a-scene_b200/mas_b200/_lib.py b/make-a-scene_b200/mas_b200/_lib.py
--- a/make-a-scene_b200/mas_b200/_lib.py
+++ b/make-a-scene_b200/mas_b200/_lib.py
@@ -9,7 +9,7 @@
 LIB_PATH = os.path.join(os.path.dirname(_HERE), "lib", "libmas_b200.so")
 
 IMPL_AUTO, IMPL_SIMT, IMPL_TC, IMPL_TC3 = 0, 1, 2, 3
-CONV_S1, CONV_S2, CONV_UP, CONV_ZS = 0, 1, 2, 3
+CONV_S1, CONV_S2, CONV_UP, CONV_ZS, CONV_S2D = 0, 1, 2, 3, 4
 
 
 class Tensor4(ctypes.Structure):
diff --git a/make-a-scene_b200/mas_b200/ops.py b/make-a-scene_b200/mas_b200/ops.py
--- a/make-a-scene_b200/mas_b200/ops.py
+++ b/make-a-scene_b200/mas_b200/ops.py
@@ -162,7 +162,7 @@
 
 
 def conv3x3_raw(x, weight, bias, residual, mode, out_nchw=False, transpose=False, table=None, silu=True, want_stats=False,
-                prepack=False, x_amax=None):
+                prepack=False, x_amax=None, s2d=False):
     n, _, h, w = x.shape
     cout = weight.shape[1] if transpose else weight.shape[0]
     cin = weight.shape[0] if transpose else weight.shape[1]
@@ -176,6 +176,7 @@
     stats = None
     if _tc_on() and not out_nchw and L.query("mas_conv3x3_tc_eligible", xs, ys, mode):
         f16 = _cfg["operands"] == "f16" and cin % 16 == 0
+        kmode = L.CONV_S2D if s2d and cin % 64 == 0 else mode
         wt = _packed_conv_weight(wc, weight, cout, cin, transpose, x.device, prepack, f16)
         part = None
         if want_stats and cout % (4 * GN_GROUPS) == 0:
@@ -183,9 +184,9 @@
             part = torch.empty(tiles * cout * 2, dtype=torch.float32, device=x.device)
         if f16:
             xa = (x_amax if x_amax is not None else amax_of(x)) if table is None else None
-            L.call("mas_conv3x3_fprop_tc16", x, xs, wt, bias, residual, y, ys, mode, table, int(silu), part, xa)
+            L.call("mas_conv3x3_fprop_tc16", x, xs, wt, bias, residual, y, ys, kmode, table, int(silu), part, xa)
         else:
-            L.call("mas_conv3x3_fprop_tc", x, xs, wt, bias, residual, y, ys, mode, table, int(silu), part)
+            L.call("mas_conv3x3_fprop_tc", x, xs, wt, bias, residual, y, ys, kmode, table, int(silu), part)
         if part is not None:
             stats = _finalize_stats(part, (ho // 16) * (wo // 8), n, cout, ho * wo)
     else:
@@ -277,7 +278,7 @@
     return wt
 
 
-def conv3x3_wgrad_raw(x, dy, cout, cin, mode, want_bias=True, table=None, silu=True, dy_amax=None):
+def conv3x3_wgrad_raw(x, dy, cout, cin, mode, want_bias=True, table=None, silu=True, dy_amax=None, s2d=False):
     dw = torch.empty((cout, cin, 3, 3), dtype=torch.float32, device=x.device)
     db = torch.empty(cout, dtype=torch.float32, device=x.device) if want_bias else None
     nb = L.query("mas_conv3x3_wgrad_ws_bytes", L.t4(x), L.t4(dy), mode)
@@ -286,6 +287,8 @@
     if (_tc_on() and _cfg["operands"] == "f16" and wgrad_f16_on() and _is_dense_nhwc(x) and _is_dense_nhwc(dy)
             and (padded or L.query("mas_conv3x3_wgrad_tc_eligible", L.t4(x), L.t4(dy), mode))):
         flags = int(x.dtype == torch.float16) | (2 if dy.dtype == torch.float16 else 0)
+        if s2d and table is None and cin % 128 == 0:
+            flags |= 4
         if dy.dtype == torch.float16 and dy_amax is None:
             raise RuntimeError("an fp16 output-gradient shadow needs the device scalar its scale was derived from")
         L.call("mas_conv3x3_wgrad_tc16", x, flags, L.t4(x), dy, L.t4(dy), dw, db, mode, table, int(silu),
@@ -309,6 +312,10 @@
 
 def wgrad_f16_on():
     return os.environ.get("MAS_WGRAD_F16", "1") != "0"
+
+
+def s2d_exact_on():
+    return os.environ.get("MAS_S2D_DENSE", "0") != "1"
 
 
 def f16_operands():
@@ -494,7 +501,7 @@
             L.call("mas_space_to_depth", x, x4, n, h, w, cin)
             w9 = torch.empty((cout, 4 * cin, 3, 3), dtype=torch.float32, device=x.device)
             L.call("mas_s2d_pack_weights", weight.contiguous(), w9, cout, cin)
-            y = conv3x3_raw(x4, w9, bias, None, L.CONV_S1)
+            y = conv3x3_raw(x4, w9, bias, None, L.CONV_S1, s2d=s2d_exact_on())
             x = x4
         else:
             y = conv3x3_raw(x, weight, bias, residual, mode, out_nchw, prepack=ctx.needs_input_grad[0])
@@ -557,7 +564,7 @@
             if ctx.needs_input_grad[0]:
                 dx = conv3x3_dgrad_raw(nhwc(dy), weight, ctx.mode)
             if want_w:
-                dw9, db = conv3x3_wgrad_raw(x, nhwc(dy), cout, 4 * cin, L.CONV_S1, ctx.has_bias)
+                dw9, db = conv3x3_wgrad_raw(x, nhwc(dy), cout, 4 * cin, L.CONV_S1, ctx.has_bias, s2d=s2d_exact_on())
                 dw = torch.empty_like(weight)
                 L.call("mas_s2d_unpack_wgrad", dw9, dw, cout, cin)
         else:
```

Result: no change. 391.0, median of 6 (+0.6%).
